# rasd3/TODA

Hardware: NVIDIA B200
Metric: frames/s voxelize+VoxelResBackBone8x fwd+bwd (higher is better)
Workload: dtype bf16

## Files before the change

include/toda_b200.h:

```cpp
#ifndef TODA_B200_H
#define TODA_B200_H

#include <stddef.h>
#include <stdint.h>

#ifdef __cplusplus
extern "C" {
#endif

#define TODA_OK 0
#define TODA_ERR_INVALID (-1)
#define TODA_ERR_CUDA (-2)
#define TODA_ERR_WORKSPACE (-3)
#define TODA_ERR_UNSUPPORTED (-4)

#define TODA_ORDER_FIRST_APPEARANCE 0
#define TODA_ORDER_CANONICAL 1

const char *toda_last_error(void);
int toda_version(void);
long long toda_launch_count(void);
int toda_device_info(int *sm_count_host, int *cc_major_host, int *cc_minor_host);

size_t toda_index_bytes(int batch, int D, int H, int W);
int toda_index_insert(void *index, int batch, int D, int H, int W, const int32_t *coords, int n, void *stream);
int toda_index_insert_strided(void *index_out, int batch, int oD, int oH, int oW, const int32_t *in_coords, int n_in,
                              const int *ksize_host, const int *stride_host, const int *pad_host, void *stream);
int toda_index_build(void *index, int batch, int D, int H, int W, int32_t *out_coords, int cap, int32_t *n_out,
                     void *stream);
int toda_index_rows(const void *index, int batch, int D, int H, int W, const int32_t *coords, int n, int32_t *rows,
                    void *stream);
int toda_index_release(void *index, int batch, int D, int H, int W, const int32_t *coords, int n, void *stream);

#define TODA_SELECT_RANGE_XY 0
#define TODA_SELECT_RECT_XY 1
#define TODA_SELECT_SECTOR 2
#define TODA_SELECT_BOXES 3
size_t toda_points_select_workspace_bytes(int n);
int toda_points_select(const float *points, int n, int stride, int x_col, const int32_t *frame_offsets, int batch, int mode,
                       const double *params_host, int invert, int add_batch_col, float *out, int32_t *out_offsets,
                       void *workspace, size_t workspace_bytes, void *stream);

#define TODA_WORLD_FLIP_X 0
#define TODA_WORLD_FLIP_Y 1
#define TODA_WORLD_ROTATE 2
#define TODA_WORLD_SCALE 3
int toda_points_world_transform(const float *points, int n, int stride, int x_col, const int32_t *frame_offsets, int batch,
                                int n_steps, const int *kinds_host, const float *params_host, float *out, void *stream);

size_t toda_voxelize_workspace_bytes(int64_t n_points, int batch, const int *grid_host, int max_points,
                                     int max_voxels);
int toda_voxelize_hard(const float *points, int64_t n_points, int point_stride, int xyz_col, int feat_col,
                       int num_features, const int32_t *frame_offsets, int batch, const float *range_host,
                       const float *vsize_host, const int *grid_host, int max_points, int max_voxels, int order,
                       float *voxels, int32_t *coords, int32_t *num_points, int32_t *voxel_counts, void *workspace,
                       size_t workspace_bytes, void *stream);

int toda_mean_vfe_fwd(const float *voxels, const void *num_points, int num_is_float, int n_voxels, int max_points,
                      int num_features, float *voxel_features, void *stream);
int toda_mean_vfe_bwd(const float *d_voxel_features, const void *num_points, int num_is_float, int n_voxels,
                      int max_points, int num_features, float *d_voxels, void *stream);

int toda_rulebook_subm(const void *index, int batch, int D, int H, int W, const int32_t *coords, int n,
                       const int *ksize_host, int32_t *nbr, void *stream);
int toda_rulebook_sparse(const void *index_in, int iD, int iH, int iW, const void *index_out, int oD, int oH, int oW,
                         int batch, const int32_t *in_coords, int n_in, const int32_t *out_coords, int n_out,
                         const int *ksize_host, const int *stride_host, const int *pad_host, int32_t *nbr_fwd,
                         int32_t *nbr_bwd, void *stream);

size_t toda_parity_order_workspace_bytes(int n);
int toda_parity_order(const int32_t *coords, int n, const int *stride_host, const int *pad_host, int32_t *order,
                      int32_t *pos_of_row, void *workspace, size_t workspace_bytes, void *stream);

#define TODA_CONV_FP32 0
#define TODA_CONV_BF16 1
#define TODA_CONV_BF16X3 2
int toda_weight_repack(const float *w_param, int kvol, int cin, int cout, int transpose, int mirror_k, float *w_out,
                       void *stream);
size_t toda_spconv_fwd_workspace_bytes(int n_in, int cin, int cout, int kvol, int precision);
int toda_table_tile_masks(const int32_t *nbr, int n_out, int kvol, uint32_t *masks, void *stream);
int toda_spconv_uses_tensor_cores(int cin, int cout, int kvol, int precision);
int toda_spconv_wgrad_uses_tensor_cores(int cin, int cout, int kvol, int precision);
int toda_spconv_fwd(const float *x, const void *x_bf16, int n_in, int cin, const int32_t *nbr, int n_out, int kvol,
                    const float *w, int cout, const float *bias, float *y, const int32_t *out_rows,
                    const uint32_t *tile_masks, double *bn_sums, int precision, void *workspace, size_t workspace_bytes,
                    void *stream);
int toda_tile_plan_capacity(int channels);
int toda_table_tile_plan(const int32_t *nbr, int n_out, int kvol, int ngroups, int cap, uint16_t *lidx, int32_t *rows,
                         int32_t *cnt, void *stream);
int toda_spconv_fwd_plan(const float *x, const void *x_bf16, int n_in, int cin, const int32_t *nbr, int n_out, int kvol,
                         const float *w, int cout, const float *bias, const float *addend, float *y,
                         const int32_t *out_rows, const uint32_t *tile_masks, const uint16_t *plan_lidx,
                         const int32_t *plan_rows, const int32_t *plan_cnt, int plan_groups, int plan_cap, double *bn_sums,
                         const void *w_bf16, int precision, void *workspace, size_t workspace_bytes, void *stream);
int toda_weight_kmajor_bf16(const float *w, int kvol, int cin, int cout, void *w_bf16, void *stream);
size_t toda_spconv_wgrad_workspace_bytes(int n_in, int n_out, int kvol, int cin, int cout, int precision);
int toda_spconv_wgrad(const float *x, const void *x_bf16, int n_in, int cin, const int32_t *nbr, int n_out, int kvol,
                      const float *dy, const void *dy_bf16, int cout, float *dw_param, void *workspace,
                      size_t workspace_bytes, int precision, void *stream);

size_t toda_bn_workspace_bytes(int channels);
int toda_bn_local_sums(const float *y, const double *epilogue_sums, int n, int channels, double *sums, double *count,
                       void *workspace, size_t workspace_bytes, void *stream);
int toda_bn_eval_coeffs(const float *gamma, const float *beta, const float *running_mean, const float *running_var,
                        float eps, int channels, float *scale, float *shift, void *stream);
int toda_bn_apply(const float *y, int n, int channels, const float *scale, const float *shift, const float *residual,
                  int relu, float *a, void *a_bf16, void *stream);
int toda_bn_apply_sums(const float *y, int n, int channels, const double *sums, const double *count, const float *gamma,
                       const float *beta, float eps, float momentum, float *running_mean, float *running_var, float *scale,
                       float *shift, float *save_mean, float *save_rstd, const float *residual, int relu, float *a,
                       void *a_bf16, void *stream);
int toda_bn_bwd_reduce(const float *da, const float *a, const float *y, int n, int channels, const float *save_mean,
                       const float *save_rstd, int relu, double *red, float *dgamma, float *dbeta, void *workspace,
                       size_t workspace_bytes, void *stream);
int toda_bn_bwd_finish(const float *da, const float *a, const float *y, int n, int channels, const float *gamma,
                       const float *save_mean, const float *save_rstd, int relu, int training, const double *red,
                       const double *count, float *dy, void *dy_bf16, float *dresidual, void *stream);
int toda_bn_bwd(const float *da, const float *a, const float *y, int n, int channels, const float *gamma,
                const float *save_mean, const float *save_rstd, int relu, int training, float *dy, void *dy_bf16,
                float *dresidual, float *dgamma, float *dbeta, void *workspace, size_t workspace_bytes, void *stream);
int toda_col_sum(const float *dy, int n, int channels, float *out, void *workspace, size_t workspace_bytes,
                 void *stream);

typedef struct {
    const float *x; const void *x_bf16; int n_in, cin; const int32_t *nbr; int n_out, kvol;
    const float *w; const void *w_bf16 ; int cout; const float *bias ;
    const uint32_t *tile_masks ;
    const uint16_t *plan_lidx ; const int32_t *plan_rows; const int32_t *plan_cnt; int plan_groups, plan_cap;
    int precision; void *conv_ws; size_t conv_ws_bytes;
    const float *gamma; const float *beta; float eps, momentum; float *running_mean; float *running_var; int training;
    const float *residual ; int relu;
    float *y; double *sums; float *stats; float *a; void *a_bf16 ;
    void *bn_ws; size_t bn_ws_bytes;
} toda_layer_fwd_args;
typedef struct {
    const float *da; const float *a_mask; const float *y; int n_out, cout; const float *gamma; const float *mean; const float *rstd;
    int relu, training; float *dy; void *dy_bf16 ; float *dres ; float *dgamma; float *dbeta;
    void *bn_ws; size_t bn_ws_bytes;
    const float *x; const void *x_bf16 ; int n_in, cin, kvol;
    int need_dx; const int32_t *dgrad_nbr; const float *wt; const void *wt_bf16 ;
    const int32_t *dgrad_out_rows ; const uint32_t *dgrad_masks ;
    const uint16_t *dplan_lidx ; const int32_t *dplan_rows; const int32_t *dplan_cnt; int dplan_groups, dplan_cap;
    const float *addend ; float *dx;
    int need_dw; const int32_t *nbr_fwd; float *dw; void *wgrad_ws; size_t wgrad_ws_bytes;
    int need_db; float *db;
    int precision; void *conv_ws; size_t conv_ws_bytes;
} toda_layer_bwd_args;
int toda_layer_fwd(const toda_layer_fwd_args *args, void *stream);
int toda_layer_bwd(const toda_layer_bwd_args *args, void *stream);
int toda_layer_fwd_stats(const toda_layer_fwd_args *args, double *local_sums, void *stream);
int toda_layer_fwd_apply(const toda_layer_fwd_args *args, const double *global_sums, void *stream);
int toda_layer_bwd_reduce(const toda_layer_bwd_args *args, double *local_red, void *stream);
int toda_layer_bwd_finish(const toda_layer_bwd_args *args, const double *global_red, const double *global_count, void *stream);

int toda_bev_scatter_fwd(const float *features, const int32_t *coords, int n, int channels, int batch, int D, int H,
                         int W, float *out, void *stream);
int toda_bev_scatter_bwd(const float *d_out, const int32_t *coords, int n, int channels, int batch, int D, int H,
                         int W, float *d_features, void *stream);

int toda_gather_rows(const float *in, const int32_t *rows, int n, int channels, float *out, void *stream);

#ifdef __cplusplus
}
#endif
#endif
```

toda_b200/_C.py:

```python
import ctypes
import os

_HERE = os.path.dirname(os.path.abspath(__file__))
LIB_PATH = os.path.join(_HERE, "lib", "libtoda_b200.so")

c_int, c_i64, c_f32, c_vp, c_sz = ctypes.c_int, ctypes.c_int64, ctypes.c_float, ctypes.c_void_p, ctypes.c_size_t
_IP = ctypes.POINTER(ctypes.c_int)
_FP = ctypes.POINTER(ctypes.c_float)

SIGNATURES = {
    "toda_last_error": (ctypes.c_char_p, []),
    "toda_version": (c_int, []),
    "toda_launch_count": (ctypes.c_longlong, []),
    "toda_device_info": (c_int, [_IP, _IP, _IP]),
    "toda_index_bytes": (c_sz, [c_int] * 4),
    "toda_index_insert": (c_int, [c_vp, c_int, c_int, c_int, c_int, c_vp, c_int, c_vp]),
    "toda_index_insert_strided": (c_int, [c_vp, c_int, c_int, c_int, c_int, c_vp, c_int, _IP, _IP, _IP, c_vp]),
    "toda_index_build": (c_int, [c_vp, c_int, c_int, c_int, c_int, c_vp, c_int, c_vp, c_vp]),
    "toda_index_rows": (c_int, [c_vp, c_int, c_int, c_int, c_int, c_vp, c_int, c_vp, c_vp]),
    "toda_index_release": (c_int, [c_vp, c_int, c_int, c_int, c_int, c_vp, c_int, c_vp]),
    "toda_points_select_workspace_bytes": (c_sz, [c_int]),
    "toda_points_select": (c_int, [c_vp, c_int, c_int, c_int, c_vp, c_int, c_int, ctypes.POINTER(ctypes.c_double), c_int, c_int,
                                   c_vp, c_vp, c_vp, c_sz, c_vp]),
    "toda_points_world_transform": (c_int, [c_vp, c_int, c_int, c_int, c_vp, c_int, c_int, _IP, _FP, c_vp, c_vp]),
    "toda_voxelize_workspace_bytes": (c_sz, [c_i64, c_int, _IP, c_int, c_int]),
    "toda_voxelize_hard": (c_int, [c_vp, c_i64, c_int, c_int, c_int, c_int, c_vp, c_int, _FP, _FP, _IP, c_int, c_int,
                                   c_int, c_vp, c_vp, c_vp, c_vp, c_vp, c_sz, c_vp]),
    "toda_mean_vfe_fwd": (c_int, [c_vp, c_vp, c_int, c_int, c_int, c_int, c_vp, c_vp]),
    "toda_mean_vfe_bwd": (c_int, [c_vp, c_vp, c_int, c_int, c_int, c_int, c_vp, c_vp]),
    "toda_rulebook_subm": (c_int, [c_vp, c_int, c_int, c_int, c_int, c_vp, c_int, _IP, c_vp, c_vp]),
    "toda_rulebook_sparse": (c_int, [c_vp, c_int, c_int, c_int, c_vp, c_int, c_int, c_int, c_int, c_vp, c_int, c_vp,
                                     c_int, _IP, _IP, _IP, c_vp, c_vp, c_vp]),
    "toda_weight_repack": (c_int, [c_vp, c_int, c_int, c_int, c_int, c_int, c_vp, c_vp]),
    "toda_spconv_fwd_workspace_bytes": (c_sz, [c_int] * 5),
    "toda_spconv_uses_tensor_cores": (c_int, [c_int] * 4),
    "toda_spconv_wgrad_uses_tensor_cores": (c_int, [c_int] * 4),
    "toda_parity_order_workspace_bytes": (c_sz, [c_int]),
    "toda_parity_order": (c_int, [c_vp, c_int, _IP, _IP, c_vp, c_vp, c_vp, c_sz, c_vp]),
    "toda_table_tile_masks": (c_int, [c_vp, c_int, c_int, c_vp, c_vp]),
    "toda_spconv_fwd": (c_int, [c_vp, c_vp, c_int, c_int, c_vp, c_int, c_int, c_vp, c_int, c_vp, c_vp, c_vp, c_vp, c_vp, c_int, c_vp,
                                c_sz, c_vp]),
    "toda_tile_plan_capacity": (c_int, [c_int]),
    "toda_table_tile_plan": (c_int, [c_vp, c_int, c_int, c_int, c_int, c_vp, c_vp, c_vp, c_vp]),
    "toda_spconv_fwd_plan": (c_int, [c_vp, c_vp, c_int, c_int, c_vp, c_int, c_int, c_vp, c_int, c_vp, c_vp, c_vp, c_vp, c_vp, c_vp,
                                     c_vp, c_vp, c_int, c_int, c_vp, c_vp, c_int, c_vp, c_sz, c_vp]),
    "toda_weight_kmajor_bf16": (c_int, [c_vp, c_int, c_int, c_int, c_vp, c_vp]),
    "toda_layer_fwd": (c_int, [c_vp, c_vp]),
    "toda_layer_bwd": (c_int, [c_vp, c_vp]),
    "toda_layer_fwd_stats": (c_int, [c_vp, c_vp, c_vp]),
    "toda_layer_fwd_apply": (c_int, [c_vp, c_vp, c_vp]),
    "toda_layer_bwd_reduce": (c_int, [c_vp, c_vp, c_vp]),
    "toda_layer_bwd_finish": (c_int, [c_vp, c_vp, c_vp, c_vp]),
    "toda_spconv_wgrad_workspace_bytes": (c_sz, [c_int] * 6),
    "toda_spconv_wgrad": (c_int, [c_vp, c_vp, c_int, c_int, c_vp, c_int, c_int, c_vp, c_vp, c_int, c_vp, c_vp, c_sz, c_int, c_vp]),
    "toda_bn_workspace_bytes": (c_sz, [c_int]),
    "toda_bn_local_sums": (c_int, [c_vp, c_vp, c_int, c_int, c_vp, c_vp, c_vp, c_sz, c_vp]),
    "toda_bn_eval_coeffs": (c_int, [c_vp, c_vp, c_vp, c_vp, c_f32, c_int, c_vp, c_vp, c_vp]),
    "toda_bn_apply": (c_int, [c_vp, c_int, c_int, c_vp, c_vp, c_vp, c_int, c_vp, c_vp, c_vp]),
    "toda_bn_apply_sums": (c_int, [c_vp, c_int, c_int, c_vp, c_vp, c_vp, c_vp, c_f32, c_f32, c_vp, c_vp, c_vp, c_vp, c_vp, c_vp,
                                   c_vp, c_int, c_vp, c_vp, c_vp]),
    "toda_bn_bwd": (c_int, [c_vp, c_vp, c_vp, c_int, c_int, c_vp, c_vp, c_vp, c_int, c_int, c_vp, c_vp, c_vp, c_vp, c_vp,
                            c_vp, c_sz, c_vp]),
    "toda_bn_bwd_reduce": (c_int, [c_vp, c_vp, c_vp, c_int, c_int, c_vp, c_vp, c_int, c_vp, c_vp, c_vp, c_vp, c_sz, c_vp]),
    "toda_bn_bwd_finish": (c_int, [c_vp, c_vp, c_vp, c_int, c_int, c_vp, c_vp, c_vp, c_int, c_int, c_vp, c_vp, c_vp, c_vp, c_vp,
                                   c_vp]),
    "toda_col_sum": (c_int, [c_vp, c_int, c_int, c_vp, c_vp, c_sz, c_vp]),
    "toda_bev_scatter_fwd": (c_int, [c_vp, c_vp, c_int, c_int, c_int, c_int, c_int, c_int, c_vp, c_vp]),
    "toda_bev_scatter_bwd": (c_int, [c_vp, c_vp, c_int, c_int, c_int, c_int, c_int, c_int, c_vp, c_vp]),
    "toda_gather_rows": (c_int, [c_vp, c_vp, c_int, c_int, c_vp, c_vp]),
}



class LayerFwdArgs(ctypes.Structure):
    _fields_ = [("x", c_vp), ("x_bf16", c_vp), ("n_in", c_int), ("cin", c_int), ("nbr", c_vp), ("n_out", c_int), ("kvol", c_int),
                ("w", c_vp), ("w_bf16", c_vp), ("cout", c_int), ("bias", c_vp), ("tile_masks", c_vp),
                ("plan_lidx", c_vp), ("plan_rows", c_vp), ("plan_cnt", c_vp), ("plan_groups", c_int), ("plan_cap", c_int),
                ("precision", c_int), ("conv_ws", c_vp), ("conv_ws_bytes", c_sz),
                ("gamma", c_vp), ("beta", c_vp), ("eps", c_f32), ("momentum", c_f32), ("running_mean", c_vp), ("running_var", c_vp),
                ("training", c_int), ("residual", c_vp), ("relu", c_int),
                ("y", c_vp), ("sums", c_vp), ("stats", c_vp), ("a", c_vp), ("a_bf16", c_vp), ("bn_ws", c_vp), ("bn_ws_bytes", c_sz)]


class LayerBwdArgs(ctypes.Structure):
    _fields_ = [("da", c_vp), ("a_mask", c_vp), ("y", c_vp), ("n_out", c_int), ("cout", c_int), ("gamma", c_vp), ("mean", c_vp),
                ("rstd", c_vp), ("relu", c_int), ("training", c_int), ("dy", c_vp), ("dy_bf16", c_vp), ("dres", c_vp), ("dgamma", c_vp),
                ("dbeta", c_vp), ("bn_ws", c_vp), ("bn_ws_bytes", c_sz),
                ("x", c_vp), ("x_bf16", c_vp), ("n_in", c_int), ("cin", c_int), ("kvol", c_int),
                ("need_dx", c_int), ("dgrad_nbr", c_vp), ("wt", c_vp), ("wt_bf16", c_vp), ("dgrad_out_rows", c_vp), ("dgrad_masks", c_vp),
                ("dplan_lidx", c_vp), ("dplan_rows", c_vp), ("dplan_cnt", c_vp), ("dplan_groups", c_int), ("dplan_cap", c_int),
                ("addend", c_vp), ("dx", c_vp),
                ("need_dw", c_int), ("nbr_fwd", c_vp), ("dw", c_vp), ("wgrad_ws", c_vp), ("wgrad_ws_bytes", c_sz),
                ("need_db", c_int), ("db", c_vp),
                ("precision", c_int), ("conv_ws", c_vp), ("conv_ws_bytes", c_sz)]


_lib = None


def lib():
    global _lib
    if _lib is None:
        if not os.path.exists(LIB_PATH):
            raise RuntimeError(
                f"{LIB_PATH} is missing: build it with `python -c 'import __graft_entry__ as g; g.build()'` "
                "(nvcc, sm_100a).  toda_b200 has no CPU fallback.")
        L = ctypes.CDLL(LIB_PATH)
        for name, (res, args) in SIGNATURES.items():
            fn = getattr(L, name)
            fn.restype = res
            fn.argtypes = args
        _lib = L
    return _lib


def check(rc, what=""):
    if rc != 0:
        msg = lib().toda_last_error().decode("utf-8", "replace")
        raise RuntimeError(f"libtoda_b200 {what} failed (code {rc}): {msg}")


def ints(vals):
    return (ctypes.c_int * len(vals))(*[int(v) for v in vals])


def doubles(vals):
    return (ctypes.c_double * len(vals))(*[float(v) for v in vals])


def floats(vals):
    return (ctypes.c_float * len(vals))(*[float(v) for v in vals])
```

toda_b200/csrc/bn.cu:

```cuda
#include <cuda_bf16.h>

#include "common.cuh"

namespace {

constexpr int kThreads = 256;
constexpr int kPartials = 2 * kNumSMs;

template <int MODE>
__global__ void __launch_bounds__(kThreads) col_reduce_vec_kernel(const float *__restrict__ p0, const float *__restrict__ p1,
                                                                  const float *__restrict__ p2, int n, int c,
                                                                  const float *__restrict__ mean, const float *__restrict__ rstd,
                                                                  int relu, double *__restrict__ partial) {
    __shared__ double s0[kThreads * 4], s1[kThreads * 4];
    const int tpr = c >> 2;
    const int rpi = kThreads / tpr;
    const int tx = threadIdx.x % tpr, ty = threadIdx.x / tpr;
    double a0[4] = {0, 0, 0, 0}, a1[4] = {0, 0, 0, 0};
    float4 m4 = make_float4(0, 0, 0, 0), r4 = make_float4(0, 0, 0, 0);
    if (MODE == 1) { m4 = __ldg((const float4 *)mean + tx); r4 = __ldg((const float4 *)rstd + tx); }
    const long long stride = (long long)gridDim.x * rpi;
    const bool active = ty < rpi;
    constexpr int U = 4;
    for (long long r = (long long)blockIdx.x * rpi + ty; active && r < n; r += U * stride) {
        float4 v0[U], v1[U], v2[U];
        bool ok[U];
#pragma unroll
        for (int u = 0; u < U; ++u) {
            long long rr = r + u * stride;
            ok[u] = rr < n;
            size_t e = ok[u] ? (size_t)rr * tpr + tx : 0;
            v0[u] = __ldg((const float4 *)p0 + e);
            if (MODE == 1) { v1[u] = __ldg((const float4 *)p1 + e); v2[u] = __ldg((const float4 *)p2 + e); }
        }
#pragma unroll
        for (int u = 0; u < U; ++u) {
            if (!ok[u]) continue;
            float x[4] = {v0[u].x, v0[u].y, v0[u].z, v0[u].w};
            if (MODE == 0) {
#pragma unroll
                for (int q = 0; q < 4; ++q) { a0[q] += x[q]; a1[q] += (double)x[q] * x[q]; }
            } else if (MODE == 1) {
                float av[4] = {v1[u].x, v1[u].y, v1[u].z, v1[u].w}, yv[4] = {v2[u].x, v2[u].y, v2[u].z, v2[u].w};
                float mm[4] = {m4.x, m4.y, m4.z, m4.w}, rs[4] = {r4.x, r4.y, r4.z, r4.w};
#pragma unroll
                for (int q = 0; q < 4; ++q) {
                    float g = (relu && !(av[q] > 0.f)) ? 0.f : x[q];
                    float xh = (yv[q] - mm[q]) * rs[q];
                    a0[q] += g; a1[q] += (double)g * xh;
                }
            } else {
#pragma unroll
                for (int q = 0; q < 4; ++q) a0[q] += x[q];
            }
        }
    }
#pragma unroll
    for (int q = 0; q < 4; ++q) { s0[threadIdx.x * 4 + q] = a0[q]; s1[threadIdx.x * 4 + q] = a1[q]; }
    __syncthreads();
    if ((int)threadIdx.x < c) {
        int ch = threadIdx.x, txx = ch >> 2, q = ch & 3;
        double t0 = 0.0, t1 = 0.0;
        for (int j = 0; j < rpi; ++j) { t0 += s0[(j * tpr + txx) * 4 + q]; t1 += s1[(j * tpr + txx) * 4 + q]; }
        partial[((size_t)blockIdx.x * 2 + 0) * c + ch] = t0;
        partial[((size_t)blockIdx.x * 2 + 1) * c + ch] = t1;
    }
}

template <int MODE>
__global__ void __launch_bounds__(kThreads) col_reduce_kernel(const float *__restrict__ p0, const float *__restrict__ p1,
                                                              const float *__restrict__ p2, int n, int c,
                                                              const float *__restrict__ mean, const float *__restrict__ rstd,
                                                              int relu, double *__restrict__ partial) {
    __shared__ double s0[kThreads], s1[kThreads];
    const int cpad = c <= 16 ? 16 : (c <= 32 ? 32 : (c <= 64 ? 64 : (c <= 128 ? 128 : 256)));
    const int rows_per_iter = kThreads / cpad;
    const int tx = threadIdx.x % cpad, ty = threadIdx.x / cpad;
    double a0 = 0.0, a1 = 0.0;
    float m = 0.f, rs = 0.f;
    if (MODE == 1 && tx < c) { m = mean[tx]; rs = rstd[tx]; }
    for (long long r = (long long)blockIdx.x * rows_per_iter + ty; r < n; r += (long long)gridDim.x * rows_per_iter) {
        if (tx < c) {
            size_t e = (size_t)r * c + tx;
            if (MODE == 0) {
                float v = __ldg(p0 + e);
                a0 += v; a1 += (double)v * v;
            } else if (MODE == 1) {
                float g = __ldg(p0 + e);
                if (relu && !(__ldg(p1 + e) > 0.f)) g = 0.f;
                float xh = (__ldg(p2 + e) - m) * rs;
                a0 += g; a1 += (double)g * xh;
            } else {
                a0 += __ldg(p0 + e);
            }
        }
    }
    s0[threadIdx.x] = a0; s1[threadIdx.x] = a1;
    __syncthreads();
    if (threadIdx.x < cpad && threadIdx.x < c) {
        double t0 = 0.0, t1 = 0.0;
        for (int j = 0; j < rows_per_iter; ++j) { t0 += s0[j * cpad + threadIdx.x]; t1 += s1[j * cpad + threadIdx.x]; }
        partial[((size_t)blockIdx.x * 2 + 0) * c + threadIdx.x] = t0;
        partial[((size_t)blockIdx.x * 2 + 1) * c + threadIdx.x] = t1;
    }
}

static bool vec_channels(int c) { return c % 4 == 0 && kThreads % (c / 4) == 0; }

template <int MODE>
static void launch_col_reduce(const float *p0, const float *p1, const float *p2, int n, int c, const float *mean,
                              const float *rstd, int relu, double *partial, cudaStream_t st) {
    if (vec_channels(c))
        col_reduce_vec_kernel<MODE><<<kPartials, kThreads, 0, st>>>(p0, p1, p2, n, c, mean, rstd, relu, partial);
    else
        col_reduce_kernel<MODE><<<kPartials, kThreads, 0, st>>>(p0, p1, p2, n, c, mean, rstd, relu, partial);
}

__device__ __forceinline__ void warp_sum_partials(const double *__restrict__ partial, int nblocks, int c, int ch, double &s,
                                                  double &ss) {
    const int lane = threadIdx.x & 31;
    constexpr int kPerLane = (kPartials + 31) / 32;
    double va[kPerLane], vb[kPerLane];
#pragma unroll
    for (int i = 0; i < kPerLane; ++i) {
        const int j = lane + 32 * i;
        const bool ok = j < nblocks;
        va[i] = ok ? partial[((size_t)j * 2) * c + ch] : 0.0;
        vb[i] = ok ? partial[((size_t)j * 2 + 1) * c + ch] : 0.0;
    }
    double a = 0.0, b = 0.0;
#pragma unroll
    for (int i = 0; i < kPerLane; ++i) { a += va[i]; b += vb[i]; }
#pragma unroll
    for (int o = 16; o > 0; o >>= 1) { a += __shfl_xor_sync(0xffffffffu, a, o); b += __shfl_xor_sync(0xffffffffu, b, o); }
    s = a; ss = b;
}

__device__ __forceinline__ void bn_coeffs(double s, double ss, int n, float g, float bt, float eps, float &scale, float &shift,
                                          float &meanf, float &rstd, double &var) {
    const double mean = n > 0 ? s / n : 0.0;
    var = n > 0 ? ss / n - mean * mean : 0.0;
    if (var < 0.0) var = 0.0;
    rstd = (float)(1.0 / sqrt(var + (double)eps));
    meanf = (float)mean;
    scale = __fmul_rn(g, rstd);
    shift = __fsub_rn(bt, __fmul_rn(__fmul_rn(meanf, g), rstd));
}

__device__ __forceinline__ void bn_update_running(float *running_mean, float *running_var, int ch, float momentum, float meanf,
                                                  double var, int n) {
    if (running_mean) running_mean[ch] = __fadd_rn(__fmul_rn(1.f - momentum, running_mean[ch]), __fmul_rn(momentum, meanf));
    if (running_var) {
        const double unbiased = n > 1 ? var * n / (n - 1) : var;
        running_var[ch] = __fadd_rn(__fmul_rn(1.f - momentum, running_var[ch]), __fmul_rn(momentum, (float)unbiased));
    }
}

__global__ void bn_local_sums_kernel(const double *partial, int nblocks, const double *src, int n, int c, double *out,
                                     double *count) {
    if (count && blockIdx.x == 0 && threadIdx.x == 0) *count = (double)n;
    int ch = (blockIdx.x * blockDim.x + threadIdx.x) >> 5;
    if (ch >= c) return;
    double s = 0.0, ss = 0.0;
    if (partial) warp_sum_partials(partial, nblocks, c, ch, s, ss);
    else if (src) { s = src[ch]; ss = src[c + ch]; }
    if ((threadIdx.x & 31) != 0) return;
    out[ch] = s;
    out[c + ch] = ss;
}

__global__ void bn_eval_coeffs_kernel(const float *gamma, const float *beta, const float *rm, const float *rv, float eps,
                                      int c, float *scale, float *shift) {
    int ch = blockIdx.x * blockDim.x + threadIdx.x;
    if (ch >= c) return;
    float rstd = 1.0f / sqrtf(rv[ch] + eps);
    float g = gamma ? gamma[ch] : 1.f, bt = beta ? beta[ch] : 0.f;
    scale[ch] = g * rstd;
    shift[ch] = bt - rm[ch] * g * rstd;
}

__device__ __forceinline__ void store_bf16x4(__nv_bfloat16 *__restrict__ dst, long long e, float4 o) {
    __nv_bfloat162 lo = __floats2bfloat162_rn(o.x, o.y), hi = __floats2bfloat162_rn(o.z, o.w);
    uint2 pk;
    pk.x = *(uint32_t *)&lo;
    pk.y = *(uint32_t *)&hi;
    ((uint2 *)dst)[e] = pk;
}

struct BnCoeffs {
    const double *sums; const double *count; int n;
    const float *gamma, *beta; float eps, momentum;
    float *running_mean, *running_var, *scale, *shift, *save_mean, *save_rstd;
};

template <bool VEC>
__global__ void __launch_bounds__(kThreads) bn_apply_kernel(const float *__restrict__ y, long long total, int c, BnCoeffs k,
                                                            const float *__restrict__ residual, int relu, float *__restrict__ a,
                                                            __nv_bfloat16 *__restrict__ a_bf16) {
    extern __shared__ __align__(16) float s_coef[];
    float *s_sc = s_coef, *s_sh = s_coef + c;
    const int n = k.count ? (int)*k.count : k.n;
    for (int ch = threadIdx.x; ch < c; ch += blockDim.x) {
        if (!k.sums) {
            s_sc[ch] = k.scale[ch];
            s_sh[ch] = k.shift[ch];
            continue;
        }
        float meanf, rstd;
        double var;
        bn_coeffs(k.sums[ch], k.sums[c + ch], n, k.gamma ? k.gamma[ch] : 1.f, k.beta ? k.beta[ch] : 0.f, k.eps, s_sc[ch], s_sh[ch],
                  meanf, rstd, var);
        if (blockIdx.x == 0) {
            k.scale[ch] = s_sc[ch];
            k.shift[ch] = s_sh[ch];
            if (k.save_mean) k.save_mean[ch] = meanf;
            if (k.save_rstd) k.save_rstd[ch] = rstd;
            if (n > 0) bn_update_running(k.running_mean, k.running_var, ch, k.momentum, meanf, var, n);
        }
    }
    __syncthreads();
    const long long stride = (long long)gridDim.x * blockDim.x;
    long long e = blockIdx.x * (long long)blockDim.x + threadIdx.x;
    if (VEC) {
        const long long tv = total >> 2;
        const int ch = (int)((e << 2) % c);
        const float4 sc = *(const float4 *)(s_sc + ch), sh = *(const float4 *)(s_sh + ch);
        for (; e < tv; e += stride) {
            const float4 v = __ldg((const float4 *)y + e);
            float4 o = make_float4(fmaf(v.x, sc.x, sh.x), fmaf(v.y, sc.y, sh.y), fmaf(v.z, sc.z, sh.z), fmaf(v.w, sc.w, sh.w));
            if (residual) {
                const float4 r = __ldg((const float4 *)residual + e);
                o.x += r.x; o.y += r.y; o.z += r.z; o.w += r.w;
            }
            if (relu) { o.x = fmaxf(o.x, 0.f); o.y = fmaxf(o.y, 0.f); o.z = fmaxf(o.z, 0.f); o.w = fmaxf(o.w, 0.f); }
            ((float4 *)a)[e] = o;
            if (a_bf16) store_bf16x4(a_bf16, e, o);
        }
    } else {
        for (; e < total; e += stride) {
            const int ch = (int)(e % c);
            float o = fmaf(__ldg(y + e), s_sc[ch], s_sh[ch]);
            if (residual) o += __ldg(residual + e);
            if (relu) o = fmaxf(o, 0.f);
            a[e] = o;
            if (a_bf16) a_bf16[e] = __float2bfloat16_rn(o);
        }
    }
}

__global__ void bn_bwd_finalize_kernel(const double *__restrict__ partial, int nblocks, int c, float *dgamma, float *dbeta,
                                       double *sums) {
    int ch = (blockIdx.x * blockDim.x + threadIdx.x) >> 5;
    if (ch >= c) return;
    double s, sx;
    warp_sum_partials(partial, nblocks, c, ch, s, sx);
    if ((threadIdx.x & 31) != 0) return;
    if (dbeta) dbeta[ch] = (float)s;
    if (dgamma) dgamma[ch] = (float)sx;
    sums[ch] = s;
    sums[c + ch] = sx;
}

template <bool VEC>
__global__ void __launch_bounds__(kThreads) bn_bwd_apply_kernel(const float *__restrict__ da, const float *__restrict__ a,
                                                                const float *__restrict__ y, long long total, int c, int n,
                                                                const double *__restrict__ count, const float *__restrict__ gamma,
                                                                const float *__restrict__ mean, const float *__restrict__ rstd,
                                                                const double *__restrict__ sums, int relu, int training,
                                                                float *__restrict__ dy, float *__restrict__ dres,
                                                                __nv_bfloat16 *__restrict__ dy_bf16) {
    if (count) n = (int)*count;
    auto sum = [&](int i) -> float { return (float)sums[i]; };
    const float inv_n = n > 0 ? 1.0f / (float)n : 0.f;
    const long long stride = (long long)gridDim.x * blockDim.x;
    long long e = blockIdx.x * (long long)blockDim.x + threadIdx.x;
    if (VEC) {
        const long long tv = total >> 2;
        const int ch = (int)((e << 2) % c);
        float A[4], B[4], C[4];
#pragma unroll
        for (int q = 0; q < 4; ++q) {
            float gm = gamma ? gamma[ch + q] : 1.f, rs = rstd[ch + q];
            A[q] = gm * rs;
            B[q] = training ? -gm * rs * rs * sum(c + ch + q) * inv_n : 0.f;
            C[q] = training ? -A[q] * sum(ch + q) * inv_n - B[q] * mean[ch + q] : 0.f;
        }
        for (; e < tv; e += stride) {
            float4 g4 = __ldg((const float4 *)da + e);
            float4 y4 = training ? __ldg((const float4 *)y + e) : make_float4(0.f, 0.f, 0.f, 0.f);
            if (relu) {
                float4 a4 = __ldg((const float4 *)a + e);
                g4.x = a4.x > 0.f ? g4.x : 0.f; g4.y = a4.y > 0.f ? g4.y : 0.f;
                g4.z = a4.z > 0.f ? g4.z : 0.f; g4.w = a4.w > 0.f ? g4.w : 0.f;
            }
            if (dres) ((float4 *)dres)[e] = g4;
            float4 o;
            o.x = fmaf(A[0], g4.x, fmaf(B[0], y4.x, C[0]));
            o.y = fmaf(A[1], g4.y, fmaf(B[1], y4.y, C[1]));
            o.z = fmaf(A[2], g4.z, fmaf(B[2], y4.z, C[2]));
            o.w = fmaf(A[3], g4.w, fmaf(B[3], y4.w, C[3]));
            if (dy) ((float4 *)dy)[e] = o;
            if (dy_bf16) store_bf16x4(dy_bf16, e, o);
        }
    } else {
        for (; e < total; e += stride) {
            int ch = (int)(e % c);
            float g = __ldg(da + e);
            if (relu && !(__ldg(a + e) > 0.f)) g = 0.f;
            if (dres) dres[e] = g;
            float gm = gamma ? gamma[ch] : 1.f;
            float rs = rstd[ch];
            float o;
            if (training) {
                float xh = (__ldg(y + e) - mean[ch]) * rs;
                o = gm * rs * (g - sum(ch) * inv_n - xh * sum(c + ch) * inv_n);
            } else {
                o = gm * rs * g;
            }
            if (dy) dy[e] = o;
            if (dy_bf16) dy_bf16[e] = __float2bfloat16_rn(o);
        }
    }
}

__global__ void col_sum_finalize_kernel(const double *__restrict__ partial, int nblocks, int c, float *out) {
    int ch = (blockIdx.x * blockDim.x + threadIdx.x) >> 5;
    if (ch >= c) return;
    double s, unused;
    warp_sum_partials(partial, nblocks, c, ch, s, unused);
    if ((threadIdx.x & 31) == 0) out[ch] = (float)s;
}

size_t partials_bytes(int c) { return (size_t)kPartials * 2 * c * sizeof(double); }
size_t bn_ws_bytes(int c) { return align_up(partials_bytes(c) + 2 * c * sizeof(double), 256); }

template <auto Kernel> int resident_grid(int64_t items) {
    static const int64_t cap = [] {
        int per_sm = 0;
        if (cudaOccupancyMaxActiveBlocksPerMultiprocessor(&per_sm, Kernel, kThreads, 0) != cudaSuccess || per_sm < 1) per_sm = 4;
        return (int64_t)per_sm * kNumSMs;
    }();
    const int64_t need = (items + kThreads - 1) / kThreads;
    return (int)(need < 1 ? 1 : (need < cap ? need : cap));
}

int launch_bn_apply(const float *y, int n, int c, const BnCoeffs &k, const float *residual, int relu, float *a, void *a_bf16,
                    cudaStream_t st) {
    const long long total = (long long)n * c;
    const size_t smem = 2 * (size_t)c * sizeof(float);
    if (vec_channels(c))
        bn_apply_kernel<true><<<resident_grid<bn_apply_kernel<true>>(total / 4), kThreads, smem, st>>>(
            y, total, c, k, residual, relu, a, (__nv_bfloat16 *)a_bf16);
    else
        bn_apply_kernel<false><<<resident_grid<bn_apply_kernel<false>>(total), kThreads, smem, st>>>(
            y, total, c, k, residual, relu, a, (__nv_bfloat16 *)a_bf16);
    TODA_LAUNCH_OK();
    return TODA_OK;
}

}

extern "C" size_t toda_bn_workspace_bytes(int channels) { return channels > 0 ? bn_ws_bytes(channels) : 0; }

double *bn_workspace_red(void *workspace, int c) { return (double *)((char *)workspace + partials_bytes(c)); }

extern "C" int toda_bn_local_sums(const float *y, const double *epilogue_sums, int n, int c, double *sums, double *count,
                                  void *workspace, size_t workspace_bytes, void *stream) {
    TODA_CHECK_ARG(n >= 0 && c > 0 && c <= 256 && sums, "bn_local_sums: bad args n=%d c=%d", n, c);
    if (n > 0 && epilogue_sums == sums && !count) return TODA_OK;
    cudaStream_t st = (cudaStream_t)stream;
    const double *partial = nullptr;
    if (n > 0 && !epilogue_sums) {
        TODA_CHECK_ARG(y && workspace, "bn_local_sums: null pointer");
        if (workspace_bytes < bn_ws_bytes(c)) { toda_set_error("bn_local_sums: workspace too small"); return TODA_ERR_WORKSPACE; }
        launch_col_reduce<0>(y, nullptr, nullptr, n, c, nullptr, nullptr, 0, (double *)workspace, st);
        TODA_LAUNCH_OK();
        partial = (const double *)workspace;
    }
    bn_local_sums_kernel<<<ceil_div(c * 32, 128), 128, 0, st>>>(partial, kPartials, n > 0 ? epilogue_sums : nullptr, n, c, sums,
                                                              count);
    TODA_LAUNCH_OK();
    return TODA_OK;
}

extern "C" int toda_bn_eval_coeffs(const float *gamma, const float *beta, const float *running_mean, const float *running_var,
                                   float eps, int c, float *scale, float *shift, void *stream) {
    TODA_CHECK_ARG(c > 0 && running_mean && running_var && scale && shift, "bn_eval_coeffs: bad args");
    bn_eval_coeffs_kernel<<<ceil_div(c, 128), 128, 0, (cudaStream_t)stream>>>(gamma, beta, running_mean, running_var, eps, c,
                                                                             scale, shift);
    TODA_LAUNCH_OK();
    return TODA_OK;
}

extern "C" int toda_bn_apply(const float *y, int n, int c, const float *scale, const float *shift, const float *residual,
                             int relu, float *a, void *a_bf16, void *stream) {
    TODA_CHECK_ARG(n >= 0 && c > 0, "bn_apply: bad sizes");
    if (n == 0) return TODA_OK;
    TODA_CHECK_ARG(y && scale && shift && a, "bn_apply: null pointer");
    BnCoeffs k{};
    k.scale = (float *)scale;
    k.shift = (float *)shift;
    return launch_bn_apply(y, n, c, k, residual, relu, a, a_bf16, (cudaStream_t)stream);
}

extern "C" int toda_bn_apply_sums(const float *y, int n, int c, const double *sums, const double *count, const float *gamma,
                                  const float *beta, float eps, float momentum, float *running_mean, float *running_var,
                                  float *scale, float *shift, float *save_mean, float *save_rstd, const float *residual, int relu,
                                  float *a, void *a_bf16, void *stream) {
    TODA_CHECK_ARG(n >= 0 && c > 0 && sums && scale && shift, "bn_apply_sums: bad args");
    TODA_CHECK_ARG(n == 0 || (y && a), "bn_apply_sums: null pointer");
    const BnCoeffs k{sums, count, n, gamma, beta, eps, momentum, running_mean, running_var, scale, shift, save_mean, save_rstd};
    return launch_bn_apply(y, n, c, k, residual, relu, a, a_bf16, (cudaStream_t)stream);
}

extern "C" int toda_bn_bwd_reduce(const float *da, const float *a, const float *y, int n, int c, const float *save_mean,
                                  const float *save_rstd, int relu, double *local_red, float *dgamma, float *dbeta, void *workspace,
                                  size_t workspace_bytes, void *stream) {
    TODA_CHECK_ARG(n >= 0 && c > 0 && c <= 256, "bn_bwd_reduce: unsupported sizes n=%d c=%d", n, c);
    TODA_CHECK_ARG(save_mean && save_rstd && workspace && local_red && (n == 0 || (da && y)) && (!relu || a || n == 0),
                   "bn_bwd_reduce: null pointer");
    if (workspace_bytes < bn_ws_bytes(c)) { toda_set_error("bn_bwd_reduce: workspace too small"); return TODA_ERR_WORKSPACE; }
    cudaStream_t st = (cudaStream_t)stream;
    double *partial = (double *)workspace;
    launch_col_reduce<1>(da, a, y, n, c, save_mean, save_rstd, relu, partial, st);
    TODA_LAUNCH_OK();
    bn_bwd_finalize_kernel<<<ceil_div(c * 32, 128), 128, 0, st>>>(partial, kPartials, c, dgamma, dbeta, local_red);
    TODA_LAUNCH_OK();
    return TODA_OK;
}

extern "C" int toda_bn_bwd_finish(const float *da, const float *a, const float *y, int n, int c, const float *gamma,
                                  const float *save_mean, const float *save_rstd, int relu, int training, const double *red,
                                  const double *count, float *dy, void *dy_bf16, float *dresidual, void *stream) {
    TODA_CHECK_ARG(n >= 0 && c > 0 && c <= 256, "bn_bwd_finish: unsupported sizes n=%d c=%d", n, c);
    TODA_CHECK_ARG(save_mean && save_rstd && (red || !training) && (n == 0 || (da && y && (dy || dy_bf16))) &&
                   (!relu || a || n == 0), "bn_bwd_finish: null pointer");
    if (n == 0) return TODA_OK;
    const long long total = (long long)n * c;
    cudaStream_t st = (cudaStream_t)stream;
    if (vec_channels(c))
        bn_bwd_apply_kernel<true><<<resident_grid<bn_bwd_apply_kernel<true>>(total / 4), kThreads, 0, st>>>(
            da, a, y, total, c, n, count, gamma, save_mean, save_rstd, red, relu, training, dy, dresidual, (__nv_bfloat16 *)dy_bf16);
    else
        bn_bwd_apply_kernel<false><<<resident_grid<bn_bwd_apply_kernel<false>>(total), kThreads, 0, st>>>(
            da, a, y, total, c, n, count, gamma, save_mean, save_rstd, red, relu, training, dy, dresidual, (__nv_bfloat16 *)dy_bf16);
    TODA_LAUNCH_OK();
    return TODA_OK;
}

extern "C" int toda_bn_bwd(const float *da, const float *a, const float *y, int n, int c, const float *gamma,
                           const float *save_mean, const float *save_rstd, int relu, int training, float *dy, void *dy_bf16,
                           float *dresidual, float *dgamma, float *dbeta, void *workspace, size_t workspace_bytes, void *stream) {
    TODA_CHECK_ARG(workspace, "bn_bwd: null workspace");
    double *red = bn_workspace_red(workspace, c);
    int rc = toda_bn_bwd_reduce(da, a, y, n, c, save_mean, save_rstd, relu, red, dgamma, dbeta, workspace, workspace_bytes, stream);
    if (rc) return rc;
    return toda_bn_bwd_finish(da, a, y, n, c, gamma, save_mean, save_rstd, relu, training, red, nullptr, dy, dy_bf16, dresidual,
                              stream);
}

extern "C" int toda_col_sum(const float *dy, int n, int c, float *out, void *workspace, size_t workspace_bytes, void *stream) {
    TODA_CHECK_ARG(n >= 0 && c > 0 && c <= 256 && out && workspace, "col_sum: bad args");
    if (workspace_bytes < bn_ws_bytes(c)) { toda_set_error("col_sum: workspace too small"); return TODA_ERR_WORKSPACE; }
    cudaStream_t st = (cudaStream_t)stream;
    double *partial = (double *)workspace;
    launch_col_reduce<2>(dy, nullptr, nullptr, n, c, nullptr, nullptr, 0, partial, st);
    TODA_LAUNCH_OK();
    col_sum_finalize_kernel<<<ceil_div(c * 32, 128), 128, 0, st>>>(partial, kPartials, c, out);
    TODA_LAUNCH_OK();
    return TODA_OK;
}
```

toda_b200/csrc/conv_simt.cu:

```cuda
#include "common.cuh"
#include "conv_ts.cuh"

int conv_tc_fwd(const float *x, const void *x_bf16, int n_in, int cin, const int32_t *nbr, int n_out, int kvol, const float *w,
                int cout, const float *bias, float *y, const int32_t *out_rows, const uint32_t *tile_masks, double *bn_sums,
                void *workspace, size_t workspace_bytes,
                cudaStream_t st, const TilePlan *plan, const float *addend, const void *w_bf16);
size_t conv_tc_fwd_workspace_bytes(int n_in, int cin, int cout, int kvol);
int conv_tc_wgrad(const float *x, const void *x_bf16, int n_in, int cin, const int32_t *nbr, int n_out, int kvol,
                  const float *dy, const void *dy_bf16, int cout, float *dw_param, void *workspace, size_t workspace_bytes,
                  cudaStream_t st);
bool conv_tc_supported(int cin, int cout, int kvol);
size_t conv_x3_fwd_workspace_bytes(int n_in, int cin, int cout, int kvol);
int conv_x3_fwd(const float *x, int n_in, int cin, const int32_t *nbr, int n_out, int kvol, const float *w, int cout, const float *bias,
                float *y, const int32_t *out_rows, const uint32_t *tile_masks, double *bn_sums, void *workspace, size_t workspace_bytes,
                cudaStream_t st, const TilePlan *plan, const float *addend);
size_t conv_x3_wgrad_workspace_bytes(int n_in, int n_out, int kvol, int cin, int cout);
int conv_x3_wgrad(const float *x, int n_in, int cin, const int32_t *nbr, int n_out, int kvol, const float *dy, int cout, float *dw_param,
                  void *workspace, size_t workspace_bytes, cudaStream_t st);
bool conv_tc_wgrad_supported(int cin, int cout, int kvol);
size_t conv_tc_wgrad_workspace_bytes(int n_in, int n_out, int kvol, int cin, int cout);

namespace {

constexpr int kThreads = 256;
constexpr int BK = 16;

template <int BM, int BN>
__global__ void __launch_bounds__(kThreads) conv_fwd_f32_kernel(const float *__restrict__ x, int cin,
                                                                const int *__restrict__ nbr, int n_out, int kvol,
                                                                const float *__restrict__ w, int cout,
                                                                const float *__restrict__ bias, float *__restrict__ y,
                                                                const int *__restrict__ out_rows ,
                                                                const float *__restrict__ addend ) {
    static_assert((BM / 4) * (BN / 4) == kThreads, "4x4 micro-tiles must cover the CTA tile");
    __shared__ __align__(16) float As[BK][BM + 4];
    __shared__ __align__(16) float Bs[BK][BN + 4];
    __shared__ int rows[BM];
    const int tid = threadIdx.x;
    const int tx = tid % (BN / 4), ty = tid / (BN / 4);
    const int row0 = blockIdx.x * BM, col0 = blockIdx.y * BN;
    const bool vec = (cin % 4) == 0;
    float acc[4][4];
#pragma unroll
    for (int i = 0; i < 4; ++i)
#pragma unroll
        for (int j = 0; j < 4; ++j) acc[i][j] = 0.f;

    for (int k = 0; k < kvol; ++k) {
        int any = 0;
        for (int m = tid; m < BM; m += kThreads) {
            int r = row0 + m;
            int src = (r < n_out) ? __ldg(nbr + (size_t)k * n_out + r) : -1;
            rows[m] = src;
            any |= (src >= 0);
        }
        any = __syncthreads_or(any);
        if (!any) continue;
        for (int c0 = 0; c0 < cin; c0 += BK) {
            if (vec) {
                for (int e = tid; e < BM * (BK / 4); e += kThreads) {
                    int m = e / (BK / 4), q = e % (BK / 4);
                    int src = rows[m];
                    float4 v = make_float4(0.f, 0.f, 0.f, 0.f);
                    if (src >= 0 && c0 + q * 4 < cin) v = __ldg((const float4 *)(x + (size_t)src * cin + c0 + q * 4));
                    As[q * 4 + 0][m] = v.x; As[q * 4 + 1][m] = v.y; As[q * 4 + 2][m] = v.z; As[q * 4 + 3][m] = v.w;
                }
            } else {
                for (int e = tid; e < BM * BK; e += kThreads) {
                    int m = e / BK, kk = e % BK;
                    int src = rows[m];
                    As[kk][m] = (src >= 0 && c0 + kk < cin) ? __ldg(x + (size_t)src * cin + c0 + kk) : 0.f;
                }
            }
            for (int e = tid; e < BK * BN; e += kThreads) {
                int kk = e / BN, nn = e % BN;
                Bs[kk][nn] = (c0 + kk < cin && col0 + nn < cout) ? __ldg(w + ((size_t)k * cin + c0 + kk) * cout + col0 + nn) : 0.f;
            }
            __syncthreads();
#pragma unroll
            for (int kk = 0; kk < BK; ++kk) {
                float4 a = *(const float4 *)&As[kk][ty * 4];
                float4 b = *(const float4 *)&Bs[kk][tx * 4];
                float av[4] = {a.x, a.y, a.z, a.w}, bv[4] = {b.x, b.y, b.z, b.w};
#pragma unroll
                for (int i = 0; i < 4; ++i)
#pragma unroll
                    for (int j = 0; j < 4; ++j) acc[i][j] = fmaf(av[i], bv[j], acc[i][j]);
            }
            __syncthreads();
        }
    }
#pragma unroll
    for (int i = 0; i < 4; ++i) {
        int r = row0 + ty * 4 + i;
        if (r >= n_out) continue;
        const int orow = out_rows ? __ldg(out_rows + r) : r;
#pragma unroll
        for (int j = 0; j < 4; ++j) {
            int c = col0 + tx * 4 + j;
            if (c < cout) y[(size_t)orow * cout + c] = acc[i][j] + (bias ? __ldg(bias + c) : 0.f) + (addend ? __ldg(addend + (size_t)orow * cout + c) : 0.f);
        }
    }
}

constexpr int WT = 64;
__global__ void __launch_bounds__(kThreads) conv_wgrad_f32_kernel(const float *__restrict__ x, int cin,
                                                                  const int *__restrict__ nbr, int n_out, int kvol,
                                                                  const float *__restrict__ dy, int cout, int rows_per_split,
                                                                  float *__restrict__ partial) {
    __shared__ __align__(16) float As[BK][WT + 4];
    __shared__ __align__(16) float Bs[BK][WT + 4];
    __shared__ int pin[kThreads], pout[kThreads];
    __shared__ int warp_cnt[kThreads / 32];
    const int tid = threadIdx.x, lane = tid & 31, warp = tid >> 5;
    const int tx = tid % (WT / 4), ty = tid / (WT / 4);
    const int ci_tiles = (cin + WT - 1) / WT, co_tiles = (cout + WT - 1) / WT;
    int bx = blockIdx.x;
    const int co_t = bx % co_tiles; bx /= co_tiles;
    const int ci_t = bx % ci_tiles; bx /= ci_tiles;
    const int k = bx;
    const int split = blockIdx.y;
    const int ci0 = ci_t * WT, co0 = co_t * WT;
    const int r_begin = split * rows_per_split;
    const int r_end = min(n_out, r_begin + rows_per_split);
    float acc[4][4];
#pragma unroll
    for (int i = 0; i < 4; ++i)
#pragma unroll
        for (int j = 0; j < 4; ++j) acc[i][j] = 0.f;

    for (int r0 = r_begin; r0 < r_end; r0 += kThreads) {
        int r = r0 + tid;
        int src = (r < r_end) ? __ldg(nbr + (size_t)k * n_out + r) : -1;
        unsigned bal = __ballot_sync(0xffffffffu, src >= 0);
        if (lane == 0) warp_cnt[warp] = __popc(bal);
        __syncthreads();
        int woff = 0, total = 0;
#pragma unroll
        for (int wi = 0; wi < kThreads / 32; ++wi) {
            int c = warp_cnt[wi];
            if (wi < warp) woff += c;
            total += c;
        }
        if (src >= 0) {
            int pos = woff + __popc(bal & ((1u << lane) - 1u));
            pin[pos] = src;
            pout[pos] = r;
        }
        __syncthreads();
        for (int g0 = 0; g0 < total; g0 += BK) {
            for (int e = tid; e < BK * WT; e += kThreads) {
                int kk = e / WT, c = e % WT;
                bool ok = g0 + kk < total;
                As[kk][c] = (ok && ci0 + c < cin) ? __ldg(x + (size_t)pin[ok ? g0 + kk : 0] * cin + ci0 + c) : 0.f;
                Bs[kk][c] = (ok && co0 + c < cout) ? __ldg(dy + (size_t)pout[ok ? g0 + kk : 0] * cout + co0 + c) : 0.f;
            }
            __syncthreads();
#pragma unroll
            for (int kk = 0; kk < BK; ++kk) {
                float4 a = *(const float4 *)&As[kk][ty * 4];
                float4 b = *(const float4 *)&Bs[kk][tx * 4];
                float av[4] = {a.x, a.y, a.z, a.w}, bv[4] = {b.x, b.y, b.z, b.w};
#pragma unroll
                for (int i = 0; i < 4; ++i)
#pragma unroll
                    for (int j = 0; j < 4; ++j) acc[i][j] = fmaf(av[i], bv[j], acc[i][j]);
            }
            __syncthreads();
        }
    }
    float *dst = partial + ((size_t)split * kvol + k) * cin * cout;
#pragma unroll
    for (int i = 0; i < 4; ++i) {
        int ci = ci0 + ty * 4 + i;
        if (ci >= cin) continue;
#pragma unroll
        for (int j = 0; j < 4; ++j) {
            int co = co0 + tx * 4 + j;
            if (co < cout) dst[(size_t)ci * cout + co] = acc[i][j];
        }
    }
}

__global__ void wgrad_reduce_kernel(const float *__restrict__ partial, int splits, int kvol, int cin, int cout,
                                    float *__restrict__ dw_param) {
    size_t per = (size_t)kvol * cin * cout;
    const int sub = threadIdx.x & 7;
    for (size_t e = (blockIdx.x * (size_t)blockDim.x + threadIdx.x) >> 3; e < ((per + 31) & ~(size_t)31);
         e += ((size_t)gridDim.x * blockDim.x) >> 3) {
        float s = 0.f;
        if (e < per) {
            int ci = (int)(e % cin);
            size_t t = e / cin;
            int k = (int)(t % kvol);
            int co = (int)(t / kvol);
            size_t src = ((size_t)k * cin + ci) * cout + co;
            for (int sp = sub; sp < splits; sp += 8) s += partial[sp * per + src];
        }
        s += __shfl_xor_sync(0xffffffffu, s, 1);
        s += __shfl_xor_sync(0xffffffffu, s, 2);
        s += __shfl_xor_sync(0xffffffffu, s, 4);
        if (e < per && sub == 0) dw_param[e] = s;
    }
}

__global__ void weight_repack_kernel(const float *__restrict__ w_param, int kvol, int cin, int cout, int transpose,
                                     int mirror, float *__restrict__ w_out) {
    size_t per = (size_t)kvol * cin * cout;
    for (size_t e = blockIdx.x * (size_t)blockDim.x + threadIdx.x; e < per; e += (size_t)gridDim.x * blockDim.x) {
        int inner = (int)(e % (transpose ? cin : cout));
        size_t t = e / (transpose ? cin : cout);
        int mid = (int)(t % (transpose ? cout : cin));
        int k = (int)(t / (transpose ? cout : cin));
        int ci = transpose ? inner : mid, co = transpose ? mid : inner;
        int ks = mirror ? kvol - 1 - k : k;
        w_out[e] = __ldg(w_param + ((size_t)co * kvol + ks) * cin + ci);
    }
}

__global__ void gather_rows_kernel(const float *__restrict__ in, const int *__restrict__ rows, long long total, int c,
                                   float *__restrict__ out) {
    for (long long e = blockIdx.x * (long long)blockDim.x + threadIdx.x; e < total; e += (long long)gridDim.x * blockDim.x) {
        long long i = e / c;
        int r = __ldg(rows + i);
        out[e] = r >= 0 ? __ldg(in + (long long)r * c + (e - i * c)) : 0.f;
    }
}

int wgrad_splits(int n_out, int kvol, int cin, int cout) {
    int tiles = kvol * ((cin + WT - 1) / WT) * ((cout + WT - 1) / WT);
    int want = (4 * kNumSMs + tiles - 1) / tiles;
    int max_by_rows = (n_out + 4 * kThreads - 1) / (4 * kThreads);
    int s = want < max_by_rows ? want : max_by_rows;
    return s < 1 ? 1 : s;
}

}

extern "C" int toda_weight_repack(const float *w_param, int kvol, int cin, int cout, int transpose, int mirror_k,
                                  float *w_out, void *stream) {
    TODA_CHECK_ARG(w_param && w_out && kvol > 0 && cin > 0 && cout > 0, "weight_repack: bad args");
    size_t per = (size_t)kvol * cin * cout;
    weight_repack_kernel<<<wave_grid(per, 256), 256, 0, (cudaStream_t)stream>>>(w_param, kvol, cin, cout, transpose,
                                                                              mirror_k, w_out);
    TODA_LAUNCH_OK();
    return TODA_OK;
}

extern "C" int toda_spconv_uses_tensor_cores(int cin, int cout, int kvol, int precision) {
    return (precision == TODA_CONV_BF16 || precision == TODA_CONV_BF16X3) && conv_tc_supported(cin, cout, kvol) ? 1 : 0;
}

extern "C" int toda_spconv_wgrad_uses_tensor_cores(int cin, int cout, int kvol, int precision) {
    return (precision == TODA_CONV_BF16 || precision == TODA_CONV_BF16X3) && conv_tc_wgrad_supported(cin, cout, kvol) ? 1 : 0;
}

extern "C" size_t toda_spconv_fwd_workspace_bytes(int n_in, int cin, int cout, int kvol, int precision) {
    if (precision == TODA_CONV_BF16 && n_in >= 0 && cin > 0 && cout > 0 && kvol > 0 && conv_tc_supported(cin, cout, kvol))
        return conv_tc_fwd_workspace_bytes(n_in, cin, cout, kvol);
    if (precision == TODA_CONV_BF16X3 && n_in >= 0 && cin > 0 && cout > 0 && kvol > 0 && conv_tc_supported(cin, cout, kvol))
        return conv_x3_fwd_workspace_bytes(n_in, cin, cout, kvol);
    return 0;
}

static int spconv_fwd_impl(const float *x, const void *x_bf16, int n_in, int cin, const int32_t *nbr, int n_out, int kvol,
                           const float *w, int cout, const float *bias, float *y, const int32_t *out_rows,
                           const uint32_t *tile_masks, double *bn_sums, int precision, void *workspace, size_t workspace_bytes,
                           void *stream, const TilePlan *plan, const float *addend, const void *w_bf16);

extern "C" int toda_spconv_fwd(const float *x, const void *x_bf16, int n_in, int cin, const int32_t *nbr, int n_out, int kvol,
                               const float *w, int cout, const float *bias, float *y, const int32_t *out_rows,
                               const uint32_t *tile_masks, double *bn_sums, int precision,
                               void *workspace, size_t workspace_bytes, void *stream) {
    return spconv_fwd_impl(x, x_bf16, n_in, cin, nbr, n_out, kvol, w, cout, bias, y, out_rows, tile_masks, bn_sums, precision, workspace,
                           workspace_bytes, stream, nullptr, nullptr, nullptr);
}

extern "C" int toda_spconv_fwd_plan(const float *x, const void *x_bf16, int n_in, int cin, const int32_t *nbr, int n_out, int kvol,
                                    const float *w, int cout, const float *bias, const float *addend, float *y,
                                    const int32_t *out_rows, const uint32_t *tile_masks, const uint16_t *plan_lidx,
                                    const int32_t *plan_rows, const int32_t *plan_cnt, int plan_groups, int plan_cap, double *bn_sums,
                                    const void *w_bf16, int precision, void *workspace, size_t workspace_bytes, void *stream) {
    TilePlan plan{plan_lidx, plan_rows, plan_cnt, plan_groups, plan_cap};
    return spconv_fwd_impl(x, x_bf16, n_in, cin, nbr, n_out, kvol, w, cout, bias, y, out_rows, tile_masks, bn_sums, precision, workspace,
                           workspace_bytes, stream, plan_lidx ? &plan : nullptr, addend, w_bf16);
}

static int spconv_fwd_impl(const float *x, const void *x_bf16, int n_in, int cin, const int32_t *nbr, int n_out, int kvol,
                           const float *w, int cout, const float *bias, float *y, const int32_t *out_rows,
                           const uint32_t *tile_masks, double *bn_sums, int precision, void *workspace, size_t workspace_bytes,
                           void *stream, const TilePlan *plan, const float *addend, const void *w_bf16) {
    TODA_CHECK_ARG(n_in >= 0 && n_out >= 0 && cin > 0 && cout > 0 && kvol > 0, "spconv_fwd: bad sizes");
    if (n_out == 0) return TODA_OK;
    TODA_CHECK_ARG(x && nbr && w && y, "spconv_fwd: null pointer");
    cudaStream_t st = (cudaStream_t)stream;
    TODA_CHECK_ARG(precision == TODA_CONV_FP32 || precision == TODA_CONV_BF16 || precision == TODA_CONV_BF16X3,
                   "spconv_fwd: unknown precision %d", precision);
    if (precision == TODA_CONV_BF16X3 && conv_tc_supported(cin, cout, kvol))
        return conv_x3_fwd(x, n_in, cin, nbr, n_out, kvol, w, cout, bias, y, out_rows, tile_masks, bn_sums, workspace, workspace_bytes, st,
                           plan, addend);
    if (precision == TODA_CONV_BF16 && conv_tc_supported(cin, cout, kvol))
        return conv_tc_fwd(x, x_bf16, n_in, cin, nbr, n_out, kvol, w, cout, bias, y, out_rows, tile_masks, bn_sums, workspace,
                           workspace_bytes, st, plan, addend, w_bf16);
    TODA_CHECK_ARG(!bn_sums, "spconv_fwd: fused BatchNorm statistics need the tensor-core kernel for this shape");
    if (cout <= 16) {
        dim3 grid(ceil_div(n_out, 256), ceil_div(cout, 16));
        conv_fwd_f32_kernel<256, 16><<<grid, kThreads, 0, st>>>(x, cin, nbr, n_out, kvol, w, cout, bias, y, out_rows, addend);
    } else if (cout <= 32) {
        dim3 grid(ceil_div(n_out, 128), ceil_div(cout, 32));
        conv_fwd_f32_kernel<128, 32><<<grid, kThreads, 0, st>>>(x, cin, nbr, n_out, kvol, w, cout, bias, y, out_rows, addend);
    } else {
        dim3 grid(ceil_div(n_out, 64), ceil_div(cout, 64));
        conv_fwd_f32_kernel<64, 64><<<grid, kThreads, 0, st>>>(x, cin, nbr, n_out, kvol, w, cout, bias, y, out_rows, addend);
    }
    TODA_LAUNCH_OK();
    return TODA_OK;
}

extern "C" size_t toda_spconv_wgrad_workspace_bytes(int n_in, int n_out, int kvol, int cin, int cout, int precision) {
    if (n_in < 0 || n_out < 0 || kvol <= 0 || cin <= 0 || cout <= 0) return 0;
    if (precision == TODA_CONV_BF16 && conv_tc_wgrad_supported(cin, cout, kvol))
        return conv_tc_wgrad_workspace_bytes(n_in, n_out, kvol, cin, cout);
    if (precision == TODA_CONV_BF16X3 && conv_tc_wgrad_supported(cin, cout, kvol))
        return conv_x3_wgrad_workspace_bytes(n_in, n_out, kvol, cin, cout);
    int splits = wgrad_splits(n_out, kvol, cin, cout);
    return align_up((size_t)splits * kvol * cin * cout * sizeof(float), 256);
}

extern "C" int toda_spconv_wgrad(const float *x, const void *x_bf16, int n_in, int cin, const int32_t *nbr, int n_out,
                                 int kvol, const float *dy, const void *dy_bf16, int cout, float *dw_param, void *workspace,
                                 size_t workspace_bytes, int precision, void *stream) {
    TODA_CHECK_ARG(n_in >= 0 && n_out >= 0 && cin > 0 && cout > 0 && kvol > 0, "spconv_wgrad: bad sizes");
    TODA_CHECK_ARG(dw_param, "spconv_wgrad: null dw");
    cudaStream_t st = (cudaStream_t)stream;
    if (n_out == 0) {
        TODA_CUDA_OK(cudaMemsetAsync(dw_param, 0, (size_t)kvol * cin * cout * sizeof(float), st));
        return TODA_OK;
    }
    TODA_CHECK_ARG(x && nbr && dy && workspace, "spconv_wgrad: null pointer");
    TODA_CHECK_ARG(precision == TODA_CONV_FP32 || precision == TODA_CONV_BF16 || precision == TODA_CONV_BF16X3,
                   "spconv_wgrad: unknown precision %d", precision);
    if (precision == TODA_CONV_BF16X3 && conv_tc_wgrad_supported(cin, cout, kvol))
        return conv_x3_wgrad(x, n_in, cin, nbr, n_out, kvol, dy, cout, dw_param, workspace, workspace_bytes, st);
    if (precision == TODA_CONV_BF16 && conv_tc_wgrad_supported(cin, cout, kvol))
        return conv_tc_wgrad(x, x_bf16, n_in, cin, nbr, n_out, kvol, dy, dy_bf16, cout, dw_param, workspace, workspace_bytes, st);
    int splits = wgrad_splits(n_out, kvol, cin, cout);
    size_t need = (size_t)splits * kvol * cin * cout * sizeof(float);
    if (workspace_bytes < need) {
        toda_set_error("spconv_wgrad: workspace %zu < required %zu bytes", workspace_bytes, need);
        return TODA_ERR_WORKSPACE;
    }
    int rows_per_split = ceil_div(n_out, splits);
    rows_per_split = ceil_div(rows_per_split, kThreads) * kThreads;
    int tiles = kvol * ((cin + WT - 1) / WT) * ((cout + WT - 1) / WT);
    dim3 grid(tiles, splits);
    conv_wgrad_f32_kernel<<<grid, kThreads, 0, st>>>(x, cin, nbr, n_out, kvol, dy, cout, rows_per_split, (float *)workspace);
    TODA_LAUNCH_OK();
    size_t per = (size_t)kvol * cin * cout;
    wgrad_reduce_kernel<<<wave_grid(per * 8, 256), 256, 0, st>>>((const float *)workspace, splits, kvol, cin, cout, dw_param);
    TODA_LAUNCH_OK();
    return TODA_OK;
}

extern "C" int toda_gather_rows(const float *in, const int32_t *rows, int n, int channels, float *out, void *stream) {
    TODA_CHECK_ARG(n >= 0 && channels > 0, "gather_rows: bad sizes");
    if (n == 0) return TODA_OK;
    TODA_CHECK_ARG(in && rows && out, "gather_rows: null pointer");
    long long total = (long long)n * channels;
    gather_rows_kernel<<<wave_grid(total, 256), 256, 0, (cudaStream_t)stream>>>(in, rows, total, channels, out);
    TODA_LAUNCH_OK();
    return TODA_OK;
}
```

toda_b200/csrc/conv_tc.cu:

```cuda
#include <cuda.h>
#include <cuda_bf16.h>
#include <stdlib.h>

#include "common.cuh"
#include "conv_ts.cuh"
#include "epilogue.cuh"
#include "table_slice.cuh"

namespace {

constexpr int kTileM = 128;
constexpr int kChunkK = 64;
constexpr int kStages = 3;
constexpr int kProducers = 128;
constexpr int kThreadsTC = kProducers + 32;
constexpr int kABytes = kTileM * kChunkK * 2;
constexpr int kBBytesMax = 128 * kChunkK * 2;
constexpr int kStageBytes = kABytes + kBBytesMax;
constexpr int kMaxKvol = 27;
constexpr int kIdxBytes = kMaxKvol * kTileM * 4;

__device__ __forceinline__ uint32_t smem_u32(const void *p) { return (uint32_t)__cvta_generic_to_shared(p); }

__device__ __forceinline__ void mbar_init(uint32_t bar, uint32_t count) {
// ... 245 lines not shown
                const uint32_t d_tmem = tmem_base + ab * COUT;
                uint32_t accumulate = 0;
                for (unsigned long long cm = chunk_mask_of(t); cm; cm &= cm - 1, ++g) {
                    const int c = __ffsll((long long)cm) - 1;
                    const int s = g % S, use = g / S;
                    if (dbg && blockIdx.x == 0 && lane == 0 && g < 256) dbg[4 * 256 + g] = clock64();
                    if (!ready) mbar_wait(full_bar + 8 * s, use & 1);
                    if (dbg && blockIdx.x == 0 && lane == 0 && g < 256) dbg[5 * 256 + g] = clock64();
                    const int sn = (g + 1) % S, usen = (g + 1) / S;
                    ready = mbar_test(full_bar + 8 * sn, usen & 1);
                    asm volatile("tcgen05.fence::after_thread_sync;" ::: "memory");
                    const uint32_t a_tile = base + s * C::kStage, b_tile = a_tile + C::kATile;
                    const int ksteps = min(kChunkElems, ktot - c * kChunkElems) / 16;
                    if (elect_one()) {
                        const uint64_t ad0 = make_desc_k_sw128(a_tile), bd0 = make_desc_k_sw128(b_tile);
                        umma_bf16(d_tmem, ad0, bd0, idesc, accumulate);
                        for (int j = 1; j < ksteps; ++j) {
                            const uint32_t blk = j >> 2, st = j & 3;
                            umma_bf16(d_tmem, ad0 + blk * (C::kABlock >> 4) + 2 * st, bd0 + blk * (C::kBBlock >> 4) + 2 * st, idesc, 1u);
                        }
                        umma_commit(empty_bar + 8 * s);
                    }
                    accumulate = 1u;
                    __syncwarp();
                    if (dbg && blockIdx.x == 0 && lane == 0 && g < 256) dbg[6 * 256 + g] = clock64();
                }
                if (elect_one()) umma_commit(acc_full + 8 * ab);
                __syncwarp();
            }
        }
    } else if (warp < 13) {
        const int q = warp & 3;
        float acc_s[COUT / 16], acc_q[COUT / 16];
#pragma unroll
        for (int i = 0; i < COUT / 16; ++i) acc_s[i] = acc_q[i] = 0.f;
        int it = 0;
        for (int t = blockIdx.x; t < num_tiles; t += gridDim.x, ++it) {
            const int ab = it & 1;
            mbar_wait(acc_full + 8 * ab, (it >> 1) & 1);
            asm volatile("tcgen05.fence::after_thread_sync;" ::: "memory");
            const int row = t * kTileM + q * 32 + lane;
            const int orow = (out_rows && row < n_out) ? __ldg(out_rows + row) : row;
            const uint32_t taddr = tmem_base + ((uint32_t)(q * 32) << 16) + ab * COUT;
#pragma unroll
            for (int n0 = 0; n0 < COUT; n0 += 16) {
                uint32_t v[16];
                asm volatile(
                    "tcgen05.ld.sync.aligned.32x32b.x16.b32 {%0,%1,%2,%3,%4,%5,%6,%7,%8,%9,%10,%11,%12,%13,%14,%15}, [%16];"
                    : "=r"(v[0]), "=r"(v[1]), "=r"(v[2]), "=r"(v[3]), "=r"(v[4]), "=r"(v[5]), "=r"(v[6]), "=r"(v[7]), "=r"(v[8]),
                      "=r"(v[9]), "=r"(v[10]), "=r"(v[11]), "=r"(v[12]), "=r"(v[13]), "=r"(v[14]), "=r"(v[15])
                    : "r"(taddr + n0));
                asm volatile("tcgen05.wait::ld.sync.aligned;" ::: "memory");
                float o[16];
#pragma unroll
                for (int j = 0; j < 16; ++j) o[j] = __uint_as_float(v[j]) + (bias ? __ldg(bias + n0 + j) : 0.f);
                if (row < n_out) {
                    if (addend) {
                        const float4 *ad = (const float4 *)(addend + (size_t)orow * COUT + n0);
#pragma unroll
                        for (int qq = 0; qq < 4; ++qq) {
                            const float4 a4 = __ldg(ad + qq);
                            o[4 * qq] += a4.x; o[4 * qq + 1] += a4.y; o[4 * qq + 2] += a4.z; o[4 * qq + 3] += a4.w;
                        }
                    }
                    float4 *dst = (float4 *)(y + (size_t)orow * COUT + n0);
#pragma unroll
                    for (int qq = 0; qq < 4; ++qq) dst[qq] = make_float4(o[4 * qq], o[4 * qq + 1], o[4 * qq + 2], o[4 * qq + 3]);
                }
                if (bn_sums) {
                    float sq[16];
#pragma unroll
                    for (int j = 0; j < 16; ++j) {
                        o[j] = row < n_out ? o[j] : 0.f;
                        sq[j] = o[j] * o[j];
                    }
                    acc_s[n0 / 16] += warp_colsum16(o, lane);
                    acc_q[n0 / 16] += warp_colsum16(sq, lane);
                }
            }
            asm volatile("tcgen05.fence::before_thread_sync;" ::: "memory");
            mbar_arrive(acc_empty + 8 * ab);
            if (dbg && blockIdx.x == 0 && q == 1 && lane == 0 && it < 256) dbg[2 * 256 + it] = clock64();
        }
        if (bn_sums && !(lane & 1)) {
            const int col = (lane >> 1) & 15;
#pragma unroll
            for (int i = 0; i < COUT / 16; ++i) {
                atomicAdd(bn_sums + i * 16 + col, (double)acc_s[i]);
                atomicAdd(bn_sums + COUT + i * 16 + col, (double)acc_q[i]);
            }
        }
    } else {
        int it = 0;
        for (int t = blockIdx.x; t < num_tiles; t += gridDim.x, ++it) {
            const int ib = it & 1, use = it >> 1;
            if (use > 0) mbar_wait(idx_empty + 8 * ib, (use - 1) & 1);
            const uint32_t dst0 = idx_base + ib * kIdxBytes;
            const int row0 = t * kTileM;
            load_table_slice<kTileM>(dst0, nbr, n_out, row0, n_out, kvol, lane);
            cp_async_arrive_noinc(idx_full + 8 * ib);
            mbar_arrive(idx_full + 8 * ib);
        }
    }
    __syncthreads();
    if (warp == 8) {
        asm volatile("tcgen05.fence::after_thread_sync;" ::: "memory");
        asm volatile("tcgen05.dealloc.cta_group::1.sync.aligned.b32 %0, %1;" ::"r"(tmem_base), "n"(C::kTmemCols) : "memory");
    }
}

__global__ void f32_to_bf16_kernel(const float *__restrict__ in, long long n4, __nv_bfloat16 *__restrict__ out) {
    for (long long i = blockIdx.x * (long long)blockDim.x + threadIdx.x; i < n4; i += (long long)gridDim.x * blockDim.x) {
        float4 v = __ldg((const float4 *)in + i);
        __nv_bfloat162 lo = __floats2bfloat162_rn(v.x, v.y), hi = __floats2bfloat162_rn(v.z, v.w);
        uint2 o;
        o.x = *(uint32_t *)&lo;
        o.y = *(uint32_t *)&hi;
        ((uint2 *)out)[i] = o;
    }
}

__global__ void f32_to_bf16_pad_kernel(const float *__restrict__ in, long long n, int cin, int cpad,
                                       __nv_bfloat16 *__restrict__ out) {
    long long total = n * cpad;
    for (long long e = blockIdx.x * (long long)blockDim.x + threadIdx.x; e < total; e += (long long)gridDim.x * blockDim.x) {
        long long r = e / cpad;
        int c = (int)(e - r * cpad);
        out[e] = __float2bfloat16_rn(c < cin ? __ldg(in + r * cin + c) : 0.f);
    }
}

__global__ void weight_to_kmajor_bf16_kernel(const float *__restrict__ w, int kvol, int cin, int cpad, int cout,
                                             __nv_bfloat16 *__restrict__ wb) {
    size_t per = (size_t)kvol * cpad * cout;
    for (size_t e = blockIdx.x * (size_t)blockDim.x + threadIdx.x; e < per; e += (size_t)gridDim.x * blockDim.x) {
        size_t kc = e % ((size_t)kvol * cpad);
        int co = (int)(e / ((size_t)kvol * cpad));
        int k = (int)(kc / cpad), ci = (int)(kc % cpad);
        wb[e] = __float2bfloat16_rn(ci < cin ? __ldg(w + ((size_t)k * cin + ci) * cout + co) : 0.f);
    }
}

__global__ void table_tile_masks_kernel(const int *__restrict__ nbr, int n_out, int kvol, int num_tiles, uint32_t *__restrict__ masks) {
    const int t = (blockIdx.x * blockDim.x + threadIdx.x) >> 5, lane = threadIdx.x & 31;
    if (t >= num_tiles) return;
    const int row0 = t * kTileM;
    uint32_t m = 0;
    for (int k = 0; k < kvol; ++k) {
        const int *src = nbr + (size_t)k * n_out + row0;
        int any = 0;
#pragma unroll
        for (int j = 0; j < kTileM / 32; ++j) {
            const int r = lane + 32 * j;
            if (row0 + r < n_out) any |= (__ldg(src + r) >= 0);
        }
        if (__any_sync(0xffffffffu, any)) m |= 1u << k;
    }
    if (lane == 0) masks[t] = m;
}

}

extern "C" int toda_table_tile_masks(const int32_t *nbr, int n_out, int kvol, uint32_t *masks, void *stream) {
    TODA_CHECK_ARG(n_out >= 0 && kvol > 0 && kvol <= 32, "table_tile_masks: bad sizes n_out=%d kvol=%d", n_out, kvol);
    if (n_out == 0) return TODA_OK;
    TODA_CHECK_ARG(nbr && masks, "table_tile_masks: null pointer");
    const int num_tiles = ceil_div(n_out, kTileM);
    table_tile_masks_kernel<<<ceil_div(num_tiles * 32, 256), 256, 0, (cudaStream_t)stream>>>(nbr, n_out, kvol, num_tiles, masks);
    TODA_LAUNCH_OK();
    return TODA_OK;
}

static inline int pad16(int c) { return c < 16 ? 16 : c; }

int conv_tma_fwd(const void *xb, int n_in, int cin, const int32_t *nbr, int n_out, int kvol, const void *wb, int cout,
                 const float *bias, const float *addend, float *y, const int32_t *out_rows, const uint32_t *tile_masks, double *bn_sums,
                 cudaStream_t st);

static long long *g_dbg_timeline = nullptr;
extern "C" void toda_debug_set_timeline(long long *buf) { g_dbg_timeline = buf; }
long long *conv_tc_debug_timeline() { return g_dbg_timeline; }
static int g_dbg_mode = 0;
extern "C" void toda_debug_set_mode(int m) { g_dbg_mode = m; }
int conv_tc_debug_mode() { return g_dbg_mode; }

extern "C" int toda_weight_kmajor_bf16(const float *w, int kvol, int cin, int cout, void *w_bf16, void *stream) {
    TODA_CHECK_ARG(w && w_bf16 && kvol > 0 && cin > 0 && cout > 0, "weight_kmajor_bf16: bad args");
    const int cp = cin < 16 ? 16 : cin;
    weight_to_kmajor_bf16_kernel<<<wave_grid((int64_t)kvol * cp * cout, 256), 256, 0, (cudaStream_t)stream>>>(w, kvol, cin, cp, cout,
                                                                                                            (__nv_bfloat16 *)w_bf16);
    TODA_LAUNCH_OK();
    return TODA_OK;
}

bool conv_tc_supported(int cin, int cout, int kvol) {
    bool cin_ok = (cin >= 1 && cin < 16) || cin == 16 || cin == 32 || cin == 64 || cin == 128;
    return cin_ok && kvol <= kMaxKvol && (cout == 16 || cout == 32 || cout == 64 || cout == 128);
}

size_t conv_tc_fwd_workspace_bytes(int n_in, int cin, int cout, int kvol) {
    int cp = pad16(cin);
    return align_up((size_t)n_in * cp * 2 + 16, 256) + align_up((size_t)kvol * cp * cout * 2, 256) + 256;
}

int conv_tc_fwd(const float *x, const void *x_bf16, int n_in, int cin, const int32_t *nbr, int n_out, int kvol, const float *w,
                int cout, const float *bias, float *y, const int32_t *out_rows, const uint32_t *tile_masks, double *bn_sums,
                void *workspace, size_t workspace_bytes,
                cudaStream_t st, const TilePlan *plan, const float *addend, const void *w_bf16) {
    size_t need = conv_tc_fwd_workspace_bytes(n_in, cin, cout, kvol);
    if (!workspace || workspace_bytes < need) {
        toda_set_error("spconv_fwd(bf16): workspace %zu < required %zu bytes", workspace_bytes, need);
        return TODA_ERR_WORKSPACE;
    }
    const int cp = pad16(cin);
    __nv_bfloat16 *xb = (__nv_bfloat16 *)workspace;
    __nv_bfloat16 *wb = (__nv_bfloat16 *)((char *)workspace + align_up((size_t)n_in * cp * 2 + 16, 256));
    if (cp == cin && x_bf16) {
        xb = (__nv_bfloat16 *)x_bf16;
    } else if (cp == cin) {
        long long n4 = (long long)n_in * cin / 4;
        if (n4 > 0) {
            f32_to_bf16_kernel<<<wave_grid(n4, 256), 256, 0, st>>>(x, n4, xb);
            TODA_LAUNCH_OK();
        }
    } else if (n_in > 0) {
        f32_to_bf16_pad_kernel<<<wave_grid((int64_t)n_in * cp, 256), 256, 0, st>>>(x, n_in, cin, cp, xb);
        TODA_LAUNCH_OK();
    }
    if (w_bf16) {
        wb = (__nv_bfloat16 *)w_bf16;
    } else {
        weight_to_kmajor_bf16_kernel<<<wave_grid((int64_t)kvol * cp * cout, 256), 256, 0, st>>>(w, kvol, cin, cp, cout, wb);
        TODA_LAUNCH_OK();
    }
    cin = cp;
    if (bn_sums) TODA_CUDA_OK(cudaMemsetAsync(bn_sums, 0, 2 * (size_t)cout * sizeof(double), st));
    static int feed = -1;
    if (feed < 0) { const char *e = getenv("TODA_TC_FEED"); feed = !e ? 2 : (e[0] == 'c' ? 0 : (e[0] == 't' && e[1] == 'm' ? 1 : 2)); }
    if (feed == 2 && conv_ts_supported(cin, cout, kvol, plan))
        return conv_ts_fwd(xb, n_in, cin, nbr, n_out, kvol, *plan, wb, cout, bias, addend, y, out_rows, tile_masks, bn_sums, st);
    if (feed == 1 || (feed == 2 && cin == 128 && cout == 128))
        {
        return conv_tma_fwd(xb, n_in, cin, nbr, n_out, kvol, wb, cout, bias, addend, y, out_rows, out_rows ? tile_masks : nullptr, bn_sums, st);
    }
    int num_tiles = ceil_div(n_out, kTileM);
    int grid = num_tiles < kNumSMs ? num_tiles : kNumSMs;
    CUtensorMap map_w;
    if (int rc = conv_tma_make_map(&map_w, wb, (uint64_t)cout, (uint64_t)kvol * cin, (uint32_t)cout, kChunkK)) return rc;
#define LAUNCH_TC(CI, CO)                                                                                                    \
    do {                                                                                                                     \
        constexpr int KB_ = (CO) <= 64 ? 2 : 1;                                                                              \
        constexpr int smem = FwdCfg<CO, KB_>::kSmem;                                                                         \
        static bool attr_set = false;                                                                                        \
        if (!attr_set) {                                                                                                     \
            TODA_CUDA_OK(cudaFuncSetAttribute(conv_tc_fwd_kernel<CI, CO, KB_>, cudaFuncAttributeMaxDynamicSharedMemorySize, smem)); \
            attr_set = true;                                                                                                 \
        }                                                                                                                    \
        conv_tc_fwd_kernel<CI, CO, KB_><<<grid, kFwdThreads, smem, st>>>(xb, nbr, n_out, kvol, map_w, bias, addend, y, out_rows, tile_masks, bn_sums, num_tiles, g_dbg_timeline); \
    } while (0)
#define LAUNCH_TC_CO(CI)                                                                                 \
    switch (cout) {                                                                                      \
        case 16: LAUNCH_TC(CI, 16); break;                                                               \
        case 32: LAUNCH_TC(CI, 32); break;                                                               \
        case 64: LAUNCH_TC(CI, 64); break;                                                               \
        case 128: LAUNCH_TC(CI, 128); break;                                                             \
        default: toda_set_error("conv_tc_fwd: unsupported cout %d", cout); return TODA_ERR_UNSUPPORTED;  \
    }
    switch (cin) {
        case 16: LAUNCH_TC_CO(16); break;
        case 32: LAUNCH_TC_CO(32); break;
        case 64: LAUNCH_TC_CO(64); break;
        case 128: LAUNCH_TC_CO(128); break;
        default: toda_set_error("conv_tc_fwd: unsupported cin %d", cin); return TODA_ERR_UNSUPPORTED;
    }
#undef LAUNCH_TC_CO
#undef LAUNCH_TC
    TODA_LAUNCH_OK();
    return TODA_OK;
}

namespace {

template <int NPAD, int ROWS> struct WCfg {
    static constexpr int kATile = 2 * ROWS * 128;
    static constexpr int kBTile = (NPAD / 64) * ROWS * 128;
    static constexpr int kIdx = 32 * ROWS * 4;
    static constexpr int kBBufs = ROWS == 128 ? 2 : 3;
    static constexpr int kStages = ROWS == 128 ? 4 : 8;
    static constexpr int kLag = ROWS == 128 ? 2 : 3;
    static constexpr int kSmem = kStages * kATile + kBBufs * kBTile + 2 * kIdx + 1024 + 256;
};
constexpr int kWgradThreads = kProdThreads + 32 + 128 + 32;

__device__ __forceinline__ uint64_t make_desc_mn_sw128(uint32_t smem_addr, uint32_t lbo_bytes) {
    uint64_t d = 0;
    d |= (uint64_t)((smem_addr >> 4) & 0x3fff);
    d |= (uint64_t)((lbo_bytes >> 4) & 0x3fff) << 16;
    d |= (uint64_t)(1024 >> 4) << 32;
    d |= (uint64_t)1 << 46;
    d |= (uint64_t)2 << 61;
    return d;
}

template <int CIN, int NPAD, int ROWS>
__global__ void __launch_bounds__(kWgradThreads, 1) conv_tc_wgrad_kernel(const __nv_bfloat16 *__restrict__ xb,
                                                                         const int *__restrict__ nbr, int n_out, int kvol,
                                                                         const __nv_bfloat16 *__restrict__ dyb, int cout,
                                                                         int rows_per_split, int passes_per_cta,
                                                                         float *__restrict__ partial) {
    using W = WCfg<NPAD, ROWS>;
    constexpr int kOffsPerPass = 128 / CIN;
    constexpr int S = W::kStages;
    constexpr int kRowsW = ROWS, kATileW = W::kATile, kBTileW = W::kBTile, kIdxW = W::kIdx, kBBufsW = W::kBBufs;
    constexpr int kRowIters = ROWS / 32;
    extern __shared__ uint8_t smem_raw[];
    const uint32_t raw = smem_u32(smem_raw);
    const uint32_t base = (raw + 1023u) & ~1023u;
    const uint32_t b_base = base + S * kATileW;
    const uint32_t idx_base = b_base + kBBufsW * kBTileW;
    const uint32_t bar_base = idx_base + 2 * kIdxW;
    const uint32_t a_full = bar_base, a_empty = bar_base + 8 * S;
    const uint32_t b_full = bar_base + 16 * S, b_empty = b_full + 32;
    const uint32_t idx_full = b_full + 64, idx_empty = b_full + 80;
    const uint32_t accum_bar = b_full + 96, tmem_slot = b_full + 104;
    volatile uint32_t *tmem_slot_ptr = (volatile uint32_t *)(smem_raw + (tmem_slot - raw));

    const int tid = threadIdx.x, warp = tid >> 5, lane = tid & 31;
    const int split = blockIdx.x, group = blockIdx.y;
    const int total_passes = (kvol + kOffsPerPass - 1) / kOffsPerPass;
    const int pass0 = group * passes_per_cta;
    const int npass = min(passes_per_cta, total_passes - pass0);
    const int k0 = pass0 * kOffsPerPass;
    const int noffs = min(npass * kOffsPerPass, kvol - k0);
    const int r_begin = split * rows_per_split;
    const int r_end = min(n_out, r_begin + rows_per_split);
    const int nchunks = r_end > r_begin ? (r_end - r_begin + kRowsW - 1) / kRowsW : 0;

    if (tid == 0) {
        for (int s = 0; s < S; ++s) {
            mbar_init(a_full + 8 * s, kProdThreads / 32);
            mbar_init(a_empty + 8 * s, 1);
        }
        for (int b = 0; b < kBBufsW; ++b) {
            mbar_init(b_full + 8 * b, kProdThreads / 32);
            mbar_init(b_empty + 8 * b, 1);
        }
        for (int b = 0; b < 2; ++b) {
            mbar_init(idx_full + 8 * b, 64);
            mbar_init(idx_empty + 8 * b, kProdThreads);
        }
        mbar_init(accum_bar, 1);
        asm volatile("fence.mbarrier_init.release.cluster;" ::: "memory");
    }
    uint32_t tmem_cols = 32;
    while ((int)tmem_cols < passes_per_cta * NPAD) tmem_cols <<= 1;
    if (warp == 8) {
        asm volatile("tcgen05.alloc.cta_group::1.sync.aligned.shared::cta.b32 [%0], %1;" ::"r"(tmem_slot), "r"(tmem_cols) : "memory");
        asm volatile("tcgen05.relinquish_alloc_permit.cta_group::1.sync.aligned;" ::: "memory");
    }
    asm volatile("tcgen05.fence::before_thread_sync;" ::: "memory");
    __syncthreads();
    asm volatile("tcgen05.fence::after_thread_sync;" ::: "memory");
    const uint32_t tmem_base = *tmem_slot_ptr;

    if (warp < 8) {
        const int p = tid & 7, rbase = tid >> 3;
        const uint32_t piece_off = (uint32_t)(rbase * 128 + ((p ^ (rbase & 7)) << 4));
        const int off_lo = CIN >= 64 ? 0 : p / (CIN / 8);
        const int ci_lo = CIN >= 64 ? p * 8 : (p % (CIN / 8)) * 8;
        constexpr int kLagW = W::kLag;
        int g = 0, signalled = 0;
        for (int rc = 0; rc < nchunks; ++rc) {
            const int ib = rc & 1, use_i = rc >> 1;
            const int bb = rc % kBBufsW, use_b = rc / kBBufsW;
            const int row_base = r_begin + rc * kRowsW;
            if (npass < kLagW) {
                asm volatile("cp.async.wait_group 0;" ::: "memory");
                asm volatile("fence.proxy.async.shared::cta;" ::: "memory");
                __syncwarp();
                if (lane == 0)
                    for (; signalled < g; ++signalled) {
                        if (signalled % npass == 0) mbar_arrive(b_full + 8 * ((signalled / npass) % kBBufsW));
                        mbar_arrive(a_full + 8 * (signalled % S));
                    }
                signalled = g;
            }
            if (use_b > 0) mbar_wait(b_empty + 8 * bb, (use_b - 1) & 1);
            {
                const uint32_t b_dst = b_base + bb * kBTileW + piece_off;
#pragma unroll
                for (int nb = 0; nb < NPAD / 64; ++nb) {
                    const int co = nb * 64 + p * 8;
#pragma unroll
                    for (int i = 0; i < kRowIters; ++i) {
                        const int row = row_base + rbase + 32 * i;
                        const uint32_t dst = b_dst + nb * (kRowsW * 128) + i * 4096;
                        if (row < r_end && co < cout) cp_async_16(dst, dyb + (size_t)row * cout + co, 16u);
                        else st_shared_zero16(dst);
                    }
                }
            }
            mbar_wait(idx_full + 8 * ib, use_i & 1);
            const uint32_t idx_tile = idx_base + ib * kIdxW + 4 * rbase;
            for (int ps = 0; ps < npass; ++ps, ++g) {
                const int s = g % S, use = g / S;
                if (use > 0) mbar_wait(a_empty + 8 * s, (use - 1) & 1);
                const uint32_t a_dst = base + s * kATileW + piece_off;
#pragma unroll
                for (int mb = 0; mb < 2; ++mb) {
                    const int koff = ps * kOffsPerPass + (CIN == 128 ? 0 : (CIN == 64 ? mb : mb * (kOffsPerPass / 2) + off_lo));
                    const int ci = CIN == 128 ? mb * 64 + ci_lo : ci_lo;
                    const bool k_ok = koff < noffs;
                    int src[kRowIters];
#pragma unroll
                    for (int i = 0; i < kRowIters; ++i) {
                        src[i] = -1;
                        if (k_ok) asm volatile("ld.shared.b32 %0, [%1];" : "=r"(src[i]) : "r"(idx_tile + 4 * (koff * kRowsW + 32 * i)));
                    }
#pragma unroll
                    for (int i = 0; i < kRowIters; ++i) {
                        const uint32_t dst = a_dst + mb * (kRowsW * 128) + i * 4096;
                        if (src[i] >= 0) cp_async_16(dst, xb + (size_t)(unsigned)src[i] * CIN + ci, 16u);
                        else st_shared_zero16(dst);
                    }
                }
                asm volatile("cp.async.commit_group;" ::: "memory");
                if (g - signalled >= kLagW) {
                    asm volatile("cp.async.wait_group %0;" ::"n"(kLagW) : "memory");
                    asm volatile("fence.proxy.async.shared::cta;" ::: "memory");
                    __syncwarp();
                    const int j = signalled;
                    if (lane == 0) {
                        if (j % npass == 0) mbar_arrive(b_full + 8 * ((j / npass) % kBBufsW));
                        mbar_arrive(a_full + 8 * (j % S));
                    }
                    ++signalled;
                }
            }
            mbar_arrive(idx_empty + 8 * ib);
        }
        asm volatile("cp.async.wait_group 0;" ::: "memory");
        asm volatile("fence.proxy.async.shared::cta;" ::: "memory");
        __syncwarp();
        if (lane == 0)
            for (int j = signalled; j < g; ++j) {
                if (j % npass == 0) mbar_arrive(b_full + 8 * ((j / npass) % kBBufsW));
                mbar_arrive(a_full + 8 * (j % S));
            }
    } else if (warp == 8) {
        if (nchunks > 0) {
            constexpr uint32_t idesc = make_idesc_bf16(128, NPAD) | (1u << 15) | (1u << 16);
            int g = 0;
            uint32_t ready = 0;
            for (int rc = 0; rc < nchunks; ++rc) {
                const int ib = rc % kBBufsW;
                mbar_wait(b_full + 8 * ib, (rc / kBBufsW) & 1);
                const uint32_t b_tile = b_base + ib * kBTileW;
                for (int ps = 0; ps < npass; ++ps, ++g) {
                    const int s = g % S, use = g / S;
                    if (!ready) mbar_wait(a_full + 8 * s, use & 1);
                    ready = mbar_test(a_full + 8 * ((g + 1) % S), ((g + 1) / S) & 1);
                    asm volatile("tcgen05.fence::after_thread_sync;" ::: "memory");
                    const uint32_t a_tile = base + s * kATileW;
                    if (elect_one()) {
#pragma unroll
                        const uint64_t ad0 = make_desc_mn_sw128(a_tile, kRowsW * 128), bd0 = make_desc_mn_sw128(b_tile, kRowsW * 128);
                        umma_bf16(tmem_base + ps * NPAD, ad0, bd0, idesc, rc != 0);
                        for (int j = 1; j < kRowsW / 16; ++j)
                            umma_bf16(tmem_base + ps * NPAD, ad0 + 128 * j, bd0 + 128 * j, idesc, 1u);
                        umma_commit(a_empty + 8 * s);
                    }
                    __syncwarp();
                }
                if (elect_one()) umma_commit(b_empty + 8 * ib);
                __syncwarp();
            }
            if (elect_one()) umma_commit(accum_bar);
            __syncwarp();
        }
    } else if (warp < 13) {
        const int q = warp & 3;
        if (nchunks > 0) {
            mbar_wait(accum_bar, 0);
            asm volatile("tcgen05.fence::after_thread_sync;" ::: "memory");
        }
        const int m = q * 32 + lane;
        for (int ps = 0; ps < npass; ++ps) {
            const int k = (pass0 + ps) * kOffsPerPass + m / CIN, ci = m % CIN;
            float *dst = partial + (((size_t)split * kvol + k) * CIN + ci) * cout;
            const uint32_t taddr = tmem_base + ((uint32_t)(q * 32) << 16) + ps * NPAD;
            for (int n0 = 0; n0 < cout; n0 += 16) {
                uint32_t v[16];
                if (nchunks > 0) {
                    asm volatile(
                        "tcgen05.ld.sync.aligned.32x32b.x16.b32 {%0,%1,%2,%3,%4,%5,%6,%7,%8,%9,%10,%11,%12,%13,%14,%15}, [%16];"
                        : "=r"(v[0]), "=r"(v[1]), "=r"(v[2]), "=r"(v[3]), "=r"(v[4]), "=r"(v[5]), "=r"(v[6]), "=r"(v[7]),
                          "=r"(v[8]), "=r"(v[9]), "=r"(v[10]), "=r"(v[11]), "=r"(v[12]), "=r"(v[13]), "=r"(v[14]), "=r"(v[15])
                        : "r"(taddr + n0));
                    asm volatile("tcgen05.wait::ld.sync.aligned;" ::: "memory");
                } else {
#pragma unroll
                    for (int qq = 0; qq < 16; ++qq) v[qq] = 0u;
                }
                if (k < kvol) {
#pragma unroll
                    for (int qq = 0; qq < 4; ++qq)
                        *(float4 *)(dst + n0 + 4 * qq) = make_float4(__uint_as_float(v[4 * qq]), __uint_as_float(v[4 * qq + 1]),
                                                                     __uint_as_float(v[4 * qq + 2]), __uint_as_float(v[4 * qq + 3]));
                }
            }
        }
        asm volatile("tcgen05.fence::before_thread_sync;" ::: "memory");
    } else {
        for (int rc = 0; rc < nchunks; ++rc) {
            const int ib = rc & 1, use = rc >> 1;
            if (use > 0) mbar_wait(idx_empty + 8 * ib, (use - 1) & 1);
            const uint32_t dst0 = idx_base + ib * kIdxW;
            const int row_base = r_begin + rc * kRowsW;
            load_table_slice<ROWS>(dst0, nbr + (size_t)k0 * n_out, n_out, row_base, r_end, noffs, lane);
            cp_async_arrive_noinc(idx_full + 8 * ib);
            mbar_arrive(idx_full + 8 * ib);
        }
    }
    __syncthreads();
    if (warp == 8) {
        asm volatile("tcgen05.fence::after_thread_sync;" ::: "memory");
        asm volatile("tcgen05.dealloc.cta_group::1.sync.aligned.b32 %0, %1;" ::"r"(tmem_base), "r"(tmem_cols) : "memory");
    }
}

__global__ void __launch_bounds__(256) wgrad_tc_reduce_kernel(const float *__restrict__ partial, int splits, int kvol, int cin,
                                                              int cpad, int cout, float *__restrict__ dw_param) {
    __shared__ float red[8][33];
    const size_t per_pad = (size_t)kvol * cpad * cout;
    const int x = threadIdx.x & 31, y = threadIdx.x >> 5;
    for (size_t e0 = (size_t)blockIdx.x * 32; e0 < per_pad; e0 += (size_t)gridDim.x * 32) {
        const size_t e = e0 + x;
        float s = 0.f;
        if (e < per_pad) {
#pragma unroll 4
            for (int sp = y; sp < splits; sp += 8) s += __ldg(partial + sp * per_pad + e);
        }
        red[y][x] = s;
        __syncthreads();
        if (y == 0 && e < per_pad) {
            s = ((red[0][x] + red[1][x]) + (red[2][x] + red[3][x])) + ((red[4][x] + red[5][x]) + (red[6][x] + red[7][x]));
            const int co = (int)(e % cout);
            const size_t t = e / cout;
            const int ci = (int)(t % cpad), k = (int)(t / cpad);
            if (ci < cin) dw_param[((size_t)co * kvol + k) * cin + ci] = s;
        }
        __syncthreads();
    }
}

struct WgradPlan {
    int passes_per_cta, groups, splits, rows_per_split;
    size_t xb_bytes, dyb_bytes, partial_bytes;
};

WgradPlan wgrad_plan(int n_in, int n_out, int kvol, int cin, int cout) {
    WgradPlan p;
    int npad = cout <= 64 ? 64 : 128;
    const int kRowsW = npad == 64 ? 128 : 64;
    int offs = 128 / cin;
    int total_passes = (kvol + offs - 1) / offs;
    p.passes_per_cta = total_passes < 512 / npad ? total_passes : 512 / npad;
    p.groups = (total_passes + p.passes_per_cta - 1) / p.passes_per_cta;
    int want = kNumSMs / p.groups;
    if (want < 1) want = 1;
    int max_by_rows = (n_out + 4 * kRowsW - 1) / (4 * kRowsW);
    p.splits = want < max_by_rows ? want : max_by_rows;
    if (p.splits < 1) p.splits = 1;
    int rps = (n_out + p.splits - 1) / p.splits;
    p.rows_per_split = (rps + kRowsW - 1) / kRowsW * kRowsW;
    if (p.rows_per_split < kRowsW) p.rows_per_split = kRowsW;
    p.xb_bytes = align_up((size_t)n_in * cin * 2 + 16, 256);
    p.dyb_bytes = align_up((size_t)n_out * cout * 2 + 16, 256);
    p.partial_bytes = align_up((size_t)p.splits * kvol * cin * cout * 4, 256);
    return p;
}

}

bool conv_tc_wgrad_supported(int cin, int cout, int kvol) {
    return kvol <= kMaxKvol && ((cin >= 1 && cin <= 16) || cin == 32 || cin == 64 || cin == 128) && (cout == 16 || cout == 32 || cout == 64 || cout == 128);
}

size_t conv_tc_wgrad_workspace_bytes(int n_in, int n_out, int kvol, int cin, int cout) {
    WgradPlan p = wgrad_plan(n_in, n_out, kvol, pad16(cin), cout);
    return p.xb_bytes + p.dyb_bytes + p.partial_bytes + 256;
}

int conv_tc_wgrad(const float *x, const void *x_bf16, int n_in, int cin, const int32_t *nbr, int n_out, int kvol,
                  const float *dy, const void *dy_bf16, int cout, float *dw_param, void *workspace, size_t workspace_bytes,
                  cudaStream_t st) {
    const int cin_real = cin;
    cin = pad16(cin);
    WgradPlan p = wgrad_plan(n_in, n_out, kvol, cin, cout);
    size_t need = p.xb_bytes + p.dyb_bytes + p.partial_bytes;
    if (!workspace || workspace_bytes < need) {
        toda_set_error("spconv_wgrad(bf16): workspace %zu < required %zu bytes", workspace_bytes, need);
        return TODA_ERR_WORKSPACE;
    }
    __nv_bfloat16 *xb = (__nv_bfloat16 *)workspace;
    __nv_bfloat16 *dyb = (__nv_bfloat16 *)((char *)workspace + p.xb_bytes);
    float *partial = (float *)((char *)workspace + p.xb_bytes + p.dyb_bytes);
    long long n4 = (long long)n_in * cin / 4;
    if (cin_real != cin) {
        if (n_in > 0) {
            f32_to_bf16_pad_kernel<<<wave_grid((int64_t)n_in * cin, 256), 256, 0, st>>>(x, n_in, cin_real, cin, xb);
            TODA_LAUNCH_OK();
        }
    } else if (x_bf16) {
        xb = (__nv_bfloat16 *)x_bf16;
    } else if (n4 > 0) {
        f32_to_bf16_kernel<<<wave_grid(n4, 256), 256, 0, st>>>(x, n4, xb);
        TODA_LAUNCH_OK();
    }
    if (dy_bf16) {
        dyb = (__nv_bfloat16 *)dy_bf16;
    } else {
        n4 = (long long)n_out * cout / 4;
        f32_to_bf16_kernel<<<wave_grid(n4, 256), 256, 0, st>>>(dy, n4, dyb);
        TODA_LAUNCH_OK();
    }
    dim3 grid(p.splits, p.groups);
#define LAUNCH_W(CI, NP, RW)                                                                                              \
    do {                                                                                                                   \
        constexpr int smem = WCfg<NP, RW>::kSmem;                                                                          \
        static bool attr_set = false;                                                                                      \
        if (!attr_set) {                                                                                                   \
            TODA_CUDA_OK(cudaFuncSetAttribute(conv_tc_wgrad_kernel<CI, NP, RW>, cudaFuncAttributeMaxDynamicSharedMemorySize, smem)); \
            attr_set = true;                                                                                               \
        }                                                                                                                  \
        conv_tc_wgrad_kernel<CI, NP, RW><<<grid, kWgradThreads, smem, st>>>(xb, nbr, n_out, kvol, dyb, cout, p.rows_per_split,  \
                                                                           p.passes_per_cta, partial);                      \
    } while (0)
    const bool wide = cout > 64;
    switch (cin) {
        case 16: if (wide) LAUNCH_W(16, 128, 64); else LAUNCH_W(16, 64, 128); break;
        case 32: if (wide) LAUNCH_W(32, 128, 64); else LAUNCH_W(32, 64, 128); break;
        case 64: if (wide) LAUNCH_W(64, 128, 64); else LAUNCH_W(64, 64, 128); break;
        case 128: if (wide) LAUNCH_W(128, 128, 64); else LAUNCH_W(128, 64, 128); break;
        default: toda_set_error("conv_tc_wgrad: unsupported cin %d", cin); return TODA_ERR_UNSUPPORTED;
    }
#undef LAUNCH_W
    TODA_LAUNCH_OK();
    size_t per_pad = (size_t)kvol * cin * cout;
    wgrad_tc_reduce_kernel<<<wave_grid(per_pad * 8, 256), 256, 0, st>>>(partial, p.splits, kvol, cin_real, cin, cout, dw_param);
    TODA_LAUNCH_OK();
    return TODA_OK;
}
```

toda_b200/csrc/conv_x3.cu:

```cuda
#include <cuda_bf16.h>

#include "common.cuh"
#include "conv_ts.cuh"

int conv_tc_fwd(const float *x, const void *x_bf16, int n_in, int cin, const int32_t *nbr, int n_out, int kvol, const float *w,
                int cout, const float *bias, float *y, const int32_t *out_rows, const uint32_t *tile_masks, double *bn_sums,
                void *workspace, size_t workspace_bytes,
                cudaStream_t st, const TilePlan *plan, const float *addend, const void *w_bf16);
size_t conv_tc_fwd_workspace_bytes(int n_in, int cin, int cout, int kvol);
int conv_tc_wgrad(const float *x, const void *x_bf16, int n_in, int cin, const int32_t *nbr, int n_out, int kvol,
                  const float *dy, const void *dy_bf16, int cout, float *dw_param, void *workspace, size_t workspace_bytes,
                  cudaStream_t st);
size_t conv_tc_wgrad_workspace_bytes(int n_in, int n_out, int kvol, int cin, int cout);

namespace {

static inline int pad16(int c) { return c < 16 ? 16 : c; }

__device__ __forceinline__ void split_bf16(float v, __nv_bfloat16 &hi, __nv_bfloat16 &lo) {
    hi = __float2bfloat16_rn(v);
    lo = __float2bfloat16_rn(v - __bfloat162float(hi));
}

__global__ void split_rows_kernel(const float *__restrict__ in, long long n, int cin, int cpad, __nv_bfloat16 *__restrict__ hi,
                                  __nv_bfloat16 *__restrict__ lo) {
    const long long total = n * cpad;
    for (long long e = blockIdx.x * (long long)blockDim.x + threadIdx.x; e < total; e += (long long)gridDim.x * blockDim.x) {
        const long long r = e / cpad;
        const int c = (int)(e - r * cpad);
        __nv_bfloat16 h, l;
        split_bf16(c < cin ? __ldg(in + r * cin + c) : 0.f, h, l);
        hi[e] = h;
        lo[e] = l;
    }
}

__global__ void split_weights_kernel(const float *__restrict__ w, int kvol, int cin, int cpad, int cout, __nv_bfloat16 *__restrict__ hi,
                                     __nv_bfloat16 *__restrict__ lo) {
    const size_t per = (size_t)kvol * cpad * cout;
    for (size_t e = blockIdx.x * (size_t)blockDim.x + threadIdx.x; e < per; e += (size_t)gridDim.x * blockDim.x) {
        const size_t kc = e % ((size_t)kvol * cpad);
        const int co = (int)(e / ((size_t)kvol * cpad));
        const int k = (int)(kc / cpad), ci = (int)(kc % cpad);
        __nv_bfloat16 h, l;
        split_bf16(ci < cin ? __ldg(w + ((size_t)k * cin + ci) * cout + co) : 0.f, h, l);
        hi[e] = h;
        lo[e] = l;
    }
}

__global__ void sum3_unpad_kernel(const float *__restrict__ t1, const float *__restrict__ t2, const float *__restrict__ t3, size_t rows,
                                  int cpad, int cin, float *__restrict__ dw) {
    const size_t total = rows * cin;
    for (size_t e = blockIdx.x * (size_t)blockDim.x + threadIdx.x; e < total; e += (size_t)gridDim.x * blockDim.x) {
        const size_t r = e / cin;
        const int c = (int)(e - r * cin);
        const size_t s = r * cpad + c;
        dw[e] = (t1[s] + t2[s]) + t3[s];
    }
}

struct X3Fwd { size_t x_bytes, w_bytes, inner; };
X3Fwd x3_fwd_layout(int n_in, int cin, int cout, int kvol) {
    const int cp = pad16(cin);
    X3Fwd l;
    l.x_bytes = align_up((size_t)(n_in > 0 ? n_in : 1) * cp * 2 + 16, 256);
    l.w_bytes = align_up((size_t)kvol * cp * cout * 2, 256);
    l.inner = conv_tc_fwd_workspace_bytes(n_in, cp, cout, kvol);
    return l;
}

struct X3Wgrad { size_t x_bytes, dy_bytes, t_bytes, inner; };
X3Wgrad x3_wgrad_layout(int n_in, int n_out, int kvol, int cin, int cout) {
    const int cp = pad16(cin);
    X3Wgrad l;
    l.x_bytes = align_up((size_t)(n_in > 0 ? n_in : 1) * cp * 2 + 16, 256);
    l.dy_bytes = align_up((size_t)(n_out > 0 ? n_out : 1) * cout * 2 + 16, 256);
    l.t_bytes = align_up((size_t)kvol * cp * cout * 4, 256);
    l.inner = conv_tc_wgrad_workspace_bytes(n_in, n_out, kvol, cp, cout);
    return l;
}

}

size_t conv_x3_fwd_workspace_bytes(int n_in, int cin, int cout, int kvol) {
    X3Fwd l = x3_fwd_layout(n_in, cin, cout, kvol);
    return 2 * l.x_bytes + 2 * l.w_bytes + l.inner + 256;
}

int conv_x3_fwd(const float *x, int n_in, int cin, const int32_t *nbr, int n_out, int kvol, const float *w, int cout, const float *bias,
                float *y, const int32_t *out_rows, const uint32_t *tile_masks, double *bn_sums, void *workspace, size_t workspace_bytes,
                cudaStream_t st, const TilePlan *plan, const float *addend) {
    const size_t need = conv_x3_fwd_workspace_bytes(n_in, cin, cout, kvol);
    if (!workspace || workspace_bytes < need) {
        toda_set_error("spconv_fwd(bf16x3): workspace %zu < required %zu bytes", workspace_bytes, need);
        return TODA_ERR_WORKSPACE;
    }
    const int cp = pad16(cin);
    X3Fwd l = x3_fwd_layout(n_in, cin, cout, kvol);
    char *p = (char *)workspace;
    __nv_bfloat16 *xh = (__nv_bfloat16 *)p, *xl = (__nv_bfloat16 *)(p + l.x_bytes);
    __nv_bfloat16 *wh = (__nv_bfloat16 *)(p + 2 * l.x_bytes), *wl = (__nv_bfloat16 *)(p + 2 * l.x_bytes + l.w_bytes);
    void *inner = p + 2 * l.x_bytes + 2 * l.w_bytes;
    if (n_in > 0) {
        split_rows_kernel<<<wave_grid((int64_t)n_in * cp, 256), 256, 0, st>>>(x, n_in, cin, cp, xh, xl);
        TODA_LAUNCH_OK();
    }
    split_weights_kernel<<<wave_grid((int64_t)kvol * cp * cout, 256), 256, 0, st>>>(w, kvol, cin, cp, cout, wh, wl);
    TODA_LAUNCH_OK();
    int rc = conv_tc_fwd(x, xh, n_in, cp, nbr, n_out, kvol, w, cout, bias, y, out_rows, tile_masks, nullptr, inner, l.inner, st, plan, addend, wh);
    if (rc) return rc;
    rc = conv_tc_fwd(x, xh, n_in, cp, nbr, n_out, kvol, w, cout, nullptr, y, out_rows, tile_masks, nullptr, inner, l.inner, st, plan, y, wl);
    if (rc) return rc;
    return conv_tc_fwd(x, xl, n_in, cp, nbr, n_out, kvol, w, cout, nullptr, y, out_rows, tile_masks, bn_sums, inner, l.inner, st, plan, y, wh);
}

size_t conv_x3_wgrad_workspace_bytes(int n_in, int n_out, int kvol, int cin, int cout) {
    X3Wgrad l = x3_wgrad_layout(n_in, n_out, kvol, cin, cout);
    return 2 * l.x_bytes + 2 * l.dy_bytes + 3 * l.t_bytes + l.inner + 256;
}

int conv_x3_wgrad(const float *x, int n_in, int cin, const int32_t *nbr, int n_out, int kvol, const float *dy, int cout, float *dw_param,
                  void *workspace, size_t workspace_bytes, cudaStream_t st) {
    const size_t need = conv_x3_wgrad_workspace_bytes(n_in, n_out, kvol, cin, cout);
    if (!workspace || workspace_bytes < need) {
        toda_set_error("spconv_wgrad(bf16x3): workspace %zu < required %zu bytes", workspace_bytes, need);
        return TODA_ERR_WORKSPACE;
    }
    const int cp = pad16(cin);
    X3Wgrad l = x3_wgrad_layout(n_in, n_out, kvol, cin, cout);
    char *p = (char *)workspace;
    __nv_bfloat16 *xh = (__nv_bfloat16 *)p, *xl = (__nv_bfloat16 *)(p + l.x_bytes);
    __nv_bfloat16 *dh = (__nv_bfloat16 *)(p + 2 * l.x_bytes), *dl = (__nv_bfloat16 *)(p + 2 * l.x_bytes + l.dy_bytes);
    float *t1 = (float *)(p + 2 * l.x_bytes + 2 * l.dy_bytes), *t2 = (float *)((char *)t1 + l.t_bytes), *t3 = (float *)((char *)t2 + l.t_bytes);
    void *inner = (char *)t3 + l.t_bytes;
    split_rows_kernel<<<wave_grid((int64_t)n_in * cp, 256), 256, 0, st>>>(x, n_in, cin, cp, xh, xl);
    TODA_LAUNCH_OK();
    split_rows_kernel<<<wave_grid((int64_t)n_out * cout, 256), 256, 0, st>>>(dy, n_out, cout, cout, dh, dl);
    TODA_LAUNCH_OK();
    int rc = conv_tc_wgrad(x, xh, n_in, cp, nbr, n_out, kvol, dy, dh, cout, t1, inner, l.inner, st);
    if (rc) return rc;
    rc = conv_tc_wgrad(x, xh, n_in, cp, nbr, n_out, kvol, dy, dl, cout, t2, inner, l.inner, st);
    if (rc) return rc;
    rc = conv_tc_wgrad(x, xl, n_in, cp, nbr, n_out, kvol, dy, dh, cout, t3, inner, l.inner, st);
    if (rc) return rc;
    const size_t rows = (size_t)cout * kvol;
    sum3_unpad_kernel<<<wave_grid((int64_t)rows * cin, 256), 256, 0, st>>>(t1, t2, t3, rows, cp, cin, dw_param);
    TODA_LAUNCH_OK();
    return TODA_OK;
}
```

toda_b200/csrc/layer.cu:

```cuda
#include "common.cuh"

static int layer_conv(const toda_layer_fwd_args *p, double *bn_sums, void *stream) {
    return toda_spconv_fwd_plan(p->x, p->x_bf16, p->n_in, p->cin, p->nbr, p->n_out, p->kvol, p->w, p->cout, p->bias, nullptr, p->y,
                                nullptr, p->tile_masks, p->plan_lidx, p->plan_rows, p->plan_cnt, p->plan_groups, p->plan_cap,
                                bn_sums, p->w_bf16, p->precision, p->conv_ws, p->conv_ws_bytes, stream);
}

static int layer_fwd_stats(const toda_layer_fwd_args *p, double *sums, double *count, void *stream) {
    const int c = p->cout, n = p->n_out;
    const bool tc = n > 0 && toda_spconv_uses_tensor_cores(p->cin, c, p->kvol, p->precision);
    int rc = layer_conv(p, tc ? sums : nullptr, stream);
    if (rc) return rc;
    return toda_bn_local_sums(p->y, tc ? sums : nullptr, n, c, sums, count, p->bn_ws, p->bn_ws_bytes, stream);
}

static int layer_fwd_apply(const toda_layer_fwd_args *p, const double *sums, const double *count, void *stream) {
    const int c = p->cout;
    float *scale = p->stats, *shift = p->stats + c, *mean = p->stats + 2 * c, *rstd = p->stats + 3 * c;
    return toda_bn_apply_sums(p->y, p->n_out, c, sums, count, p->gamma, p->beta, p->eps, p->momentum, p->running_mean,
                              p->running_var, scale, shift, mean, rstd, p->residual, p->relu, p->a, p->a_bf16, stream);
}

extern "C" int toda_layer_fwd(const toda_layer_fwd_args *p, void *stream) {
    TODA_CHECK_ARG(p, "layer_fwd: null args");
    const int c = p->cout, n = p->n_out;
    TODA_CHECK_ARG(c > 0 && n >= 0 && p->stats && (n == 0 || (p->y && p->a)) && (!p->training || p->sums),
                   "layer_fwd: bad sizes / null outputs");
    if (n == 0) return layer_conv(p, nullptr, stream);
    int rc;
    if (p->training) {
        rc = layer_fwd_stats(p, p->sums, nullptr, stream);
        return rc ? rc : layer_fwd_apply(p, p->sums, nullptr, stream);
    }
    float *scale = p->stats, *shift = p->stats + c;
    if ((rc = layer_conv(p, nullptr, stream))) return rc;
    if ((rc = toda_bn_eval_coeffs(p->gamma, p->beta, p->running_mean, p->running_var, p->eps, c, scale, shift, stream))) return rc;
    return toda_bn_apply(p->y, n, c, scale, shift, p->residual, p->relu, p->a, p->a_bf16, stream);
}

static int layer_bwd_empty(const toda_layer_bwd_args *p, bool bn_grads, cudaStream_t st) {
    const int c = p->cout;
    if (bn_grads && p->dgamma) TODA_CUDA_OK(cudaMemsetAsync(p->dgamma, 0, sizeof(float) * c, st));
    if (bn_grads && p->dbeta) TODA_CUDA_OK(cudaMemsetAsync(p->dbeta, 0, sizeof(float) * c, st));
    if (p->need_db && p->db) TODA_CUDA_OK(cudaMemsetAsync(p->db, 0, sizeof(float) * c, st));
    if (p->need_dw && p->dw) TODA_CUDA_OK(cudaMemsetAsync(p->dw, 0, sizeof(float) * (size_t)p->kvol * p->cin * c, st));
    if (p->need_dx && p->dx && p->n_in > 0) {
        if (p->addend) TODA_CUDA_OK(cudaMemcpyAsync(p->dx, p->addend, sizeof(float) * (size_t)p->n_in * p->cin, cudaMemcpyDeviceToDevice, st));
        else TODA_CUDA_OK(cudaMemsetAsync(p->dx, 0, sizeof(float) * (size_t)p->n_in * p->cin, st));
    }
    return TODA_OK;
}

static bool layer_bwd_reads_dy_f32(const toda_layer_bwd_args *p) {
    const int c = p->cout;
    return p->need_db || !p->dy_bf16 || p->precision != TODA_CONV_BF16 ||
           (p->need_dx && !toda_spconv_uses_tensor_cores(c, p->cin, p->kvol, p->precision)) ||
           (p->need_dw && !toda_spconv_wgrad_uses_tensor_cores(p->cin, c, p->kvol, p->precision));
}

static int layer_bwd_conv(const toda_layer_bwd_args *p, void *stream) {
    const int c = p->cout, n = p->n_out;
    int rc;
    if (p->need_dx) {
        rc = toda_spconv_fwd_plan(p->dy, p->dy_bf16, n, c, p->dgrad_nbr, p->n_in, p->kvol, p->wt, p->cin, nullptr, p->addend, p->dx,
                                  p->dgrad_out_rows, p->dgrad_masks, p->dplan_lidx, p->dplan_rows, p->dplan_cnt, p->dplan_groups,
                                  p->dplan_cap, nullptr, p->wt_bf16, p->precision, p->conv_ws, p->conv_ws_bytes, stream);
        if (rc) return rc;
    }
    if (p->need_dw) {
        rc = toda_spconv_wgrad(p->x, p->x_bf16, p->n_in, p->cin, p->nbr_fwd, n, p->kvol, p->dy, p->dy_bf16, c, p->dw, p->wgrad_ws,
                               p->wgrad_ws_bytes, p->precision, stream);
        if (rc) return rc;
    }
    if (p->need_db) {
        rc = toda_col_sum(p->dy, n, c, p->db, p->bn_ws, p->bn_ws_bytes, stream);
        if (rc) return rc;
    }
    return TODA_OK;
}

static int layer_bwd_reduce(const toda_layer_bwd_args *p, double *red, void *stream) {
    return toda_bn_bwd_reduce(p->da, p->a_mask, p->y, p->n_out, p->cout, p->mean, p->rstd, p->relu, red, p->dgamma, p->dbeta,
                              p->bn_ws, p->bn_ws_bytes, stream);
}

static int layer_bwd_finish(const toda_layer_bwd_args *p, const double *red, const double *count, void *stream) {
    const int c = p->cout, n = p->n_out;
    if (n == 0) return layer_bwd_empty(p, false, (cudaStream_t)stream);
    int rc = toda_bn_bwd_finish(p->da, p->a_mask, p->y, n, c, p->gamma, p->mean, p->rstd, p->relu, p->training, red, count,
                                layer_bwd_reads_dy_f32(p) ? p->dy : nullptr, p->dy_bf16, p->dres, stream);
    return rc ? rc : layer_bwd_conv(p, stream);
}

extern "C" int toda_layer_bwd(const toda_layer_bwd_args *p, void *stream) {
    TODA_CHECK_ARG(p, "layer_bwd: null args");
    TODA_CHECK_ARG(p->cout > 0 && p->n_out >= 0, "layer_bwd: bad sizes");
    if (p->n_out == 0) return layer_bwd_empty(p, true, (cudaStream_t)stream);
    TODA_CHECK_ARG(p->bn_ws, "layer_bwd: null workspace");
    double *red = bn_workspace_red(p->bn_ws, p->cout);
    int rc = layer_bwd_reduce(p, red, stream);
    return rc ? rc : layer_bwd_finish(p, red, nullptr, stream);
}


extern "C" int toda_layer_fwd_stats(const toda_layer_fwd_args *p, double *local_sums, void *stream) {
    TODA_CHECK_ARG(p && local_sums, "layer_fwd_stats: null args");
    const int c = p->cout, n = p->n_out;
    TODA_CHECK_ARG(c > 0 && n >= 0 && p->training && (n == 0 || p->y), "layer_fwd_stats: bad sizes / not training / null y");
    return layer_fwd_stats(p, local_sums, local_sums + 2 * c, stream);
}

extern "C" int toda_layer_fwd_apply(const toda_layer_fwd_args *p, const double *global_sums, void *stream) {
    TODA_CHECK_ARG(p && global_sums, "layer_fwd_apply: null args");
    const int c = p->cout, n = p->n_out;
    TODA_CHECK_ARG(c > 0 && n >= 0 && p->training && p->stats && (n == 0 || (p->y && p->a)),
                   "layer_fwd_apply: bad sizes / not training / null outputs");
    return layer_fwd_apply(p, global_sums, global_sums + 2 * c, stream);
}

extern "C" int toda_layer_bwd_reduce(const toda_layer_bwd_args *p, double *local_red, void *stream) {
    TODA_CHECK_ARG(p && local_red, "layer_bwd_reduce: null args");
    TODA_CHECK_ARG(p->cout > 0 && p->n_out >= 0 && p->training, "layer_bwd_reduce: bad sizes / not training");
    return layer_bwd_reduce(p, local_red, stream);
}

extern "C" int toda_layer_bwd_finish(const toda_layer_bwd_args *p, const double *global_red, const double *global_count,
                                     void *stream) {
    TODA_CHECK_ARG(p && global_red && global_count, "layer_bwd_finish: null args");
    TODA_CHECK_ARG(p->cout > 0 && p->n_out >= 0 && p->training, "layer_bwd_finish: bad sizes / not training");
    return layer_bwd_finish(p, global_red, global_count, stream);
}
```

toda_b200/ops.py:

```python
import ctypes
import weakref
from dataclasses import dataclass
from typing import List, Optional

import numpy as np
import torch
import torch.distributed as dist

from . import _C

ORDER_FIRST_APPEARANCE = 0
ORDER_CANONICAL = 1
CONV_FP32 = 0
CONV_BF16 = 1
CONV_BF16X3 = 2
_TC_PRECISIONS = (CONV_BF16, CONV_BF16X3)

_launch_base = 0


def launches():
    return int(_C.lib().toda_launch_count()) - _launch_base


# ... 273 lines not shown
        _C.check(_C.lib().toda_index_insert(_p(self.buf), *self._dims(), _p(coords), coords.shape[0], _stream()),
                 "toda_index_insert")

    def insert_strided(self, in_coords, ksize, stride, padding):
        self._acquire()
        in_coords = _need(in_coords, torch.int32, "in_coords")
        _C.check(_C.lib().toda_index_insert_strided(_p(self.buf), *self._dims(), _p(in_coords), in_coords.shape[0],
                                                    _C.ints(ksize), _C.ints(stride), _C.ints(padding), _stream()),
                 "toda_index_insert_strided")

    def build(self, cap, known_n=None):
        dev = self.buf.device
        coords = torch.empty((max(cap, 1), 4), dtype=torch.int32, device=dev)
        n_out = torch.empty((self.batch + 1,), dtype=torch.int32, device=dev)
        with _timed("index_build", cells=self.batch * self.shape[0] * self.shape[1] * self.shape[2]):
            _C.check(_C.lib().toda_index_build(_p(self.buf), *self._dims(), _p(coords), cap, _p(n_out), _stream()),
                     "toda_index_build")
        self.n = int(n_out[0].item()) if known_n is None else int(known_n)
        self.coords = coords[:self.n]
        self.frame_counts = n_out
        return self.coords

    def ensure_live(self):
        if _index_occupant.get(self.key) is self:
            return
        if self.coords is None:
            raise RuntimeError("occupancy index was released")
        coords, n = self.coords, self.n
        self.insert(coords)
        self.build(n, known_n=n)

    def rows(self, coords):
        self.ensure_live()
        coords = _need(coords, torch.int32, "coords")
        rows = torch.empty((coords.shape[0],), dtype=torch.int32, device=coords.device)
        _C.check(_C.lib().toda_index_rows(_p(self.buf), *self._dims(), _p(coords), coords.shape[0], _p(rows), _stream()),
                 "toda_index_rows")
        return rows

    def release(self):
        if _index_occupant.get(self.key) is self:
            self._unmark()
        self.coords = None
        self.n = 0


@dataclass
class Rulebook:
    subm: bool
    ksize: List[int]
    stride: List[int]
    padding: List[int]
    in_shape: List[int]
    out_shape: List[int]
    n_in: int
    n_out: int
    out_coords: torch.Tensor
    nbr_fwd: torch.Tensor
    nbr_bwd: Optional[torch.Tensor]
    dgrad_order: Optional[torch.Tensor] = None
    nbr_bwd_sorted: Optional[torch.Tensor] = None
    dgrad_tile_masks: Optional[torch.Tensor] = None
    tile_masks: Optional[torch.Tensor] = None
    plan: Optional["TilePlan"] = None
    dgrad_plan: Optional["TilePlan"] = None

    @property
    def kvol(self):
        return self.ksize[0] * self.ksize[1] * self.ksize[2]


@dataclass
class TilePlan:
    lidx: torch.Tensor
    rows: torch.Tensor
    cnt: torch.Tensor
    ngroups: int
    cap: int

    def tensors(self):
        return [self.lidx, self.rows, self.cnt]


def table_tile_plan(nbr, ksize, channels):
    kvol, n = nbr.shape
    ngroups = int(ksize[0])
    if n == 0 or kvol > 27 or ngroups > 3 or kvol % ngroups or kvol // ngroups > 9 or not channels:
        return None
    L = _C.lib()
    cap = L.toda_tile_plan_capacity(int(channels))
    if cap <= 0:
        return None
    tiles = (n + 127) // 128
    dev = nbr.device
    lidx = torch.empty((tiles, kvol, 128), dtype=torch.int16, device=dev)
    rows = torch.empty((tiles, ngroups, cap), dtype=torch.int32, device=dev)
    cnt = torch.empty((tiles, ngroups), dtype=torch.int32, device=dev)
    with _timed("tile_plan", n=n, kvol=kvol):
        _C.check(L.toda_table_tile_plan(_p(nbr), n, kvol, ngroups, cap, _p(lidx), _p(rows), _p(cnt), _stream()),
                 "toda_table_tile_plan")
    return TilePlan(lidx, rows, cnt, ngroups, cap)


def conv_out_size(in_size, k, s, p):
    return (in_size + 2 * p - (k - 1) - 1) // s + 1


def rulebook_subm(index: OccupancyIndex, ksize, channels=None):
    index.ensure_live()
    n = index.n
    kvol = ksize[0] * ksize[1] * ksize[2]
    nbr = torch.empty((kvol, n), dtype=torch.int32, device=index.buf.device)
    with _timed("rulebook_subm", n=n, kvol=kvol):
        _C.check(_C.lib().toda_rulebook_subm(_p(index.buf), index.batch, *index.shape, _p(index.coords), n, _C.ints(ksize),
                                             _p(nbr), _stream()), "toda_rulebook_subm")
    rb = Rulebook(True, list(ksize), [1, 1, 1], [k // 2 for k in ksize], index.shape, index.shape, n, n, index.coords,
                  nbr, None)
    rb.tile_masks = table_tile_masks(nbr) if (n > 0 and kvol <= 32) else None
    rb.plan = table_tile_plan(nbr, ksize, channels) if _TILE_PLANS else None
    return rb


def rulebook_sparse(index_in: OccupancyIndex, ksize, stride, padding, tag, cin=None, cout=None):
    index_in.ensure_live()
    out_shape = [conv_out_size(index_in.shape[a], ksize[a], stride[a], padding[a]) for a in range(3)]
    index_out = OccupancyIndex(index_in.batch, out_shape, index_in.buf.device, tag)
    if index_out.buf.data_ptr() == index_in.buf.data_ptr():
        index_out = OccupancyIndex(index_in.batch, out_shape, index_in.buf.device, (tag, "alt"))
    assert index_out.buf.data_ptr() != index_in.buf.data_ptr()
    index_out.insert_strided(index_in.coords, ksize, stride, padding)
    per_in = 1
    for a in range(3):
        per_in *= min(ksize[a], (ksize[a] + stride[a] - 1) // stride[a])
    cells = index_in.batch * out_shape[0] * out_shape[1] * out_shape[2]
    cap = int(min(index_in.n * per_in, cells))
    out_coords = index_out.build(cap)
    n_in, n_out = index_in.n, index_out.n
    kvol = ksize[0] * ksize[1] * ksize[2]
    dev = index_in.buf.device
    nbr_fwd = torch.empty((kvol, n_out), dtype=torch.int32, device=dev)
    nbr_bwd = torch.empty((kvol, n_in), dtype=torch.int32, device=dev)
    with _timed("rulebook_sparse", n_in=n_in, n_out=n_out, kvol=kvol):
        _C.check(_C.lib().toda_rulebook_sparse(_p(index_in.buf), *index_in.shape, _p(index_out.buf), *out_shape,
                                               index_in.batch, _p(index_in.coords), n_in, _p(out_coords), n_out,
                                               _C.ints(ksize), _C.ints(stride), _C.ints(padding), _p(nbr_fwd), _p(nbr_bwd),
                                               _stream()), "toda_rulebook_sparse")
    rb = Rulebook(False, list(ksize), list(stride), list(padding), index_in.shape, out_shape, n_in, n_out, out_coords,
                  nbr_fwd, nbr_bwd)
    rb.tile_masks = table_tile_masks(nbr_fwd) if (n_out > 0 and kvol <= 32) else None
    rb.dgrad_order, rb.nbr_bwd_sorted = (_dgrad_parity_order(index_in.coords, nbr_bwd, stride, padding) if kvol <= 32
                                         else (None, None))
    if rb.dgrad_order is not None:
        rb.dgrad_tile_masks = table_tile_masks(rb.nbr_bwd_sorted)
    if _TILE_PLANS:
        rb.plan = table_tile_plan(nbr_fwd, ksize, cin)
        rb.dgrad_plan = table_tile_plan(rb.nbr_bwd_sorted if rb.dgrad_order is not None else nbr_bwd, ksize, cout)
    return rb, index_out


import os as _os
_TILE_PLANS = _os.environ.get("TODA_TILE_PLANS", "0") == "1"


def set_tile_plans(on):
    global _TILE_PLANS
    _TILE_PLANS = bool(on)


def tile_plans_enabled():
    return _TILE_PLANS


def table_tile_masks(nbr):
    kvol, n = nbr.shape
    masks = torch.empty(((n + 127) // 128,), dtype=torch.int32, device=nbr.device)
    _C.check(_C.lib().toda_table_tile_masks(_p(nbr), n, kvol, _p(masks), _stream()), "toda_table_tile_masks")
    return masks


def _dgrad_parity_order(in_coords, nbr_bwd, stride, padding):
    if all(s == 1 for s in stride) or in_coords.shape[0] == 0:
        return None, None
    if stride[0] * stride[1] * stride[2] > 8:
        return None, None
    n = in_coords.shape[0]
    L = _C.lib()
    ws = _workspace("parity", L.toda_parity_order_workspace_bytes(n), in_coords.device)
    order = torch.empty((n,), dtype=torch.int32, device=in_coords.device)
    _C.check(L.toda_parity_order(_p(in_coords), n, _C.ints(stride), _C.ints(padding), _p(order), None, _p(ws), ws.numel(),
                                 _stream()), "toda_parity_order")
    return order, nbr_bwd.index_select(1, order).contiguous()


_repack_cache = {}


def invalidate_weight_cache():
    _repack_cache.clear()


def _repack(weight, transpose, mirror, want_bf16=False):
    key = (id(weight), bool(transpose), bool(mirror))
    hit = _repack_cache.get(key)
    if hit is not None and hit[2]() is weight and hit[0] == weight._version and hit[3] == weight.data_ptr():
        out = hit[1]
    else:
        cout, kvol, cin = weight.shape[0], weight.shape[1] * weight.shape[2] * weight.shape[3], weight.shape[4]
        out = torch.empty((kvol, cout, cin) if transpose else (kvol, cin, cout), dtype=torch.float32, device=weight.device)
        _C.check(_C.lib().toda_weight_repack(_p(weight), kvol, cin, cout, int(transpose), int(mirror), _p(out), _stream()),
                 "toda_weight_repack")
        if len(_repack_cache) > 512:
            _repack_cache.clear()
        hit = [weight._version, out, weakref.ref(weight), weight.data_ptr(), None]
        _repack_cache[key] = hit
    if not want_bf16:
        return out
    if hit[4] is None:
        kvol, ci, co = out.shape
        wb = torch.empty((co, kvol * max(ci, 16)), dtype=torch.bfloat16, device=out.device)
        _C.check(_C.lib().toda_weight_kmajor_bf16(_p(out), kvol, ci, co, _p(wb), _stream()), "toda_weight_kmajor_bf16")
        hit[4] = wb
    return out, hit[4]


def _bf16_shadow_of(t):
    tag = getattr(t, "_toda_bf16", None)
    if tag is not None and tag[1] == t._version and tag[0].shape == t.shape:
        return tag[0]
    return None


def _conv_call(x, xb, cin, nbr, n_out, kvol, w, cout, bias, precision, what="conv_fwd", rb=None, bn_sums=None, y=None,
               out_rows=None, tile_masks=None, plan=None, addend=None, w_bf16=None):
    if y is None:
        y = torch.empty((n_out, cout), dtype=torch.float32, device=x.device)
    L = _C.lib()
    ws_bytes = L.toda_spconv_fwd_workspace_bytes(x.shape[0], cin, cout, kvol, precision)
    ws = _workspace("conv", ws_bytes, x.device) if ws_bytes else None
    if precision not in _TC_PRECISIONS:
        plan = None
    with _timed(what, n_in=x.shape[0], n_out=n_out, cin=cin, cout=cout, kvol=kvol, precision=precision, rb=id(rb)):
        if plan is None and addend is None and w_bf16 is None:
            _C.check(L.toda_spconv_fwd(_p(x), _p(xb), x.shape[0], cin, _p(nbr), n_out, kvol, _p(w), cout, _p(bias), _p(y),
                                       _p(out_rows), _p(tile_masks), _p(bn_sums), precision, _p(ws), ws.numel() if ws is not None else 0,
                                       _stream()), "toda_spconv_fwd")
        else:
            pl = plan
            _C.check(L.toda_spconv_fwd_plan(_p(x), _p(xb), x.shape[0], cin, _p(nbr), n_out, kvol, _p(w), cout, _p(bias),
                                            _p(addend), _p(y), _p(out_rows), _p(tile_masks), _p(pl.lidx) if pl else None,
                                            _p(pl.rows) if pl else None, _p(pl.cnt) if pl else None, pl.ngroups if pl else 0,
                                            pl.cap if pl else 0, _p(bn_sums), _p(w_bf16), precision, _p(ws),
                                            ws.numel() if ws is not None else 0, _stream()), "toda_spconv_fwd_plan")
    return y


def conv_plan_usable(plan, cin, cout, kvol, precision):
    if plan is None or precision not in _TC_PRECISIONS or _os.environ.get("TODA_TC_FEED", "ts")[:1] in ("c",) or \
            _os.environ.get("TODA_TC_FEED", "ts")[:2] == "tm":
        return False
    cp = max(16, cin)
    return (cp in (16, 32, 64, 128) and cout in (16, 32, 64, 128) and kvol <= 27
            and plan.cap <= _C.lib().toda_tile_plan_capacity(cp))


def _conv_forward_impl(x, x_bf16, weight, bias, rb, precision, want_stats):
    x = _need(x.contiguous(), torch.float32, "features")
    weight = _need(weight.contiguous(), torch.float32, "weight")
    cout, cin = weight.shape[0], weight.shape[4]
    assert x.shape == (rb.n_in, cin), (x.shape, rb.n_in, cin)
    if x_bf16 is not None and (precision != CONV_BF16 or x_bf16.shape != x.shape or x_bf16.dtype != torch.bfloat16
                               or not x_bf16.is_contiguous()):
        x_bf16 = None
    w = _repack(weight, False, False)
    b = bias.contiguous() if bias is not None else None
    sums = None
    if want_stats and rb.n_out > 0 and _C.lib().toda_spconv_uses_tensor_cores(cin, cout, rb.kvol, precision):
        sums = torch.empty((2 * cout,), dtype=torch.float64, device=x.device)
    y = _conv_call(x, x_bf16, cin, rb.nbr_fwd, rb.n_out, rb.kvol, w, cout, b, precision, "conv_fwd", rb, sums,
                   tile_masks=rb.tile_masks, plan=rb.plan)
    return y, sums, x, weight, x_bf16


def _conv_backward_impl(dy, dyb, x, weight, xb, rb, precision, need_dx, need_dw, need_db):
    cout, cin = weight.shape[0], weight.shape[4]
    L = _C.lib()
    dx = dw = db = None
    if need_dx:
        wt = _repack(weight, True, rb.subm)
        if rb.subm:
            dx = _conv_call(dy, dyb, cout, rb.nbr_fwd, rb.n_in, rb.kvol, wt, cin, None, precision, "conv_dgrad", rb,
                            tile_masks=rb.tile_masks, plan=rb.plan)
        elif rb.dgrad_order is None:
            dx = _conv_call(dy, dyb, cout, rb.nbr_bwd, rb.n_in, rb.kvol, wt, cin, None, precision, "conv_dgrad", rb,
                            plan=rb.dgrad_plan)
        else:
            dx = _conv_call(dy, dyb, cout, rb.nbr_bwd_sorted, rb.n_in, rb.kvol, wt, cin, None, precision, "conv_dgrad",
                            rb, out_rows=rb.dgrad_order, tile_masks=rb.dgrad_tile_masks, plan=rb.dgrad_plan)
    if need_dw:
        dw = torch.empty_like(weight)
        ws_bytes = L.toda_spconv_wgrad_workspace_bytes(rb.n_in, rb.n_out, rb.kvol, cin, cout, precision)
        ws = _workspace("wgrad", ws_bytes, dy.device)
        with _timed("conv_wgrad", n_in=rb.n_in, n_out=rb.n_out, cin=cin, cout=cout, kvol=rb.kvol, precision=precision,
                    rb=id(rb)):
            _C.check(L.toda_spconv_wgrad(_p(x), _p(xb), rb.n_in, cin, _p(rb.nbr_fwd), rb.n_out, rb.kvol, _p(dy), _p(dyb),
                                         cout, _p(dw), _p(ws), ws.numel(), precision, _stream()), "toda_spconv_wgrad")
    if need_db:
        db = col_sum(dy)
    return dx, dw, db


class _SparseConv(torch.autograd.Function):
    @staticmethod
    def forward(ctx, x, x_bf16, weight, bias, rb: Rulebook, precision, want_stats):
        y, sums, x, weight, x_bf16 = _conv_forward_impl(x, x_bf16, weight, bias, rb, precision, want_stats)
        ctx.save_for_backward(x, weight, x_bf16)
        ctx.set_materialize_grads(False)
        ctx.rb, ctx.precision, ctx.has_bias = rb, precision, bias is not None
        if sums is not None:
            ctx.mark_non_differentiable(sums)
        return y, sums

    @staticmethod
    def backward(ctx, dy, _dsums=None):
        if dy is None:
            return (None,) * 7
        x, weight, xb = ctx.saved_tensors
        dyb = _bf16_shadow_of(dy) if (ctx.precision == CONV_BF16 and dy.is_contiguous()) else None
        dx, dw, db = _conv_backward_impl(dy.contiguous(), dyb, x, weight, xb, ctx.rb, ctx.precision, ctx.needs_input_grad[0],
                                         ctx.needs_input_grad[2], ctx.has_bias and ctx.needs_input_grad[3])
        return dx, None, dw, db, None, None, None


def sparse_conv(x, weight, bias, rb, precision=CONV_FP32, x_bf16=None, want_stats=False):
    y, sums = _SparseConv.apply(x, x_bf16, weight, bias, rb, precision, want_stats)
    return (y, sums) if want_stats else y


def col_sum(t):
    n, c = t.shape
    out = torch.empty((c,), dtype=torch.float32, device=t.device)
    L = _C.lib()
    ws = _workspace("bn", L.toda_bn_workspace_bytes(c), t.device)
    _C.check(L.toda_col_sum(_p(t), n, c, _p(out), _p(ws), ws.numel(), _stream()), "toda_col_sum")
    return out


class ReluMaskTape:

    def __init__(self, mode):
        assert mode in ("record", "replay")
        self.mode, self.masks, self.i = mode, [], 0

    def replay(self):
        self.mode, self.i = "replay", 0
        return self


_relu_tape = None


def set_relu_mask_tape(tape):
    global _relu_tape
    _relu_tape = tape


def sync_group(bn):
    if not isinstance(bn, torch.nn.SyncBatchNorm) or not bn.training:
        return None
    if bn.momentum is None:
        raise NotImplementedError("toda_b200: SyncBatchNorm with momentum=None (cumulative moving average) is not supported; "
                                  "set a momentum (these backbones use 0.01)")
    if not (dist.is_available() and dist.is_initialized()):
        return None
    group = bn.process_group if bn.process_group is not None else dist.group.WORLD
    return group if dist.get_world_size(group) > 1 else None


def _run_phases(phases, group):
    try:
        buf = next(phases)
        while True:
            dist.all_reduce(buf, op=dist.ReduceOp.SUM, group=group)
            buf = phases.send(None)
    except StopIteration as stop:
        return stop.value


def _tape_mask(a, want_bf16):
    if _relu_tape.mode == "record":
        mask = a > 0
        _relu_tape.masks.append(mask)
    else:
        mask = _relu_tape.masks[_relu_tape.i]
        _relu_tape.i += 1
    a = a * mask
    return a, (a.to(torch.bfloat16) if want_bf16 else None), mask.to(torch.float32)


def _bn_forward_phases(y, gamma, beta, running_mean, running_var, eps, momentum, training, residual, relu, want_bf16, sums,
                       need_grad, sync=False):
    y = _need(y.contiguous(), torch.float32, "bn input")
    n, c = y.shape
    dev = y.device
    L = _C.lib()
    scale, shift, mean, rstd = torch.empty((4, c), dtype=torch.float32, device=dev).unbind(0)
    gsums = count = None
    if training:
        if sync or sums is None:
            buf = torch.empty((2 * c + 1 if sync else 2 * c,), dtype=torch.float64, device=dev)
            count = buf.data_ptr() + 16 * c if sync else None
            ws = _workspace("bn", L.toda_bn_workspace_bytes(c), dev)
            with _timed("bn_stats", n=n, c=c):
                _C.check(L.toda_bn_local_sums(_p(y), _p(sums), n, c, _p(buf), count, _p(ws), ws.numel(), _stream()),
                         "toda_bn_local_sums")
            sums = buf
        if sync:
            yield sums
            gsums = sums
    else:
        _C.check(L.toda_bn_eval_coeffs(_p(gamma), _p(beta), _p(running_mean), _p(running_var), float(eps), c, _p(scale),
                                       _p(shift), _stream()), "toda_bn_eval_coeffs")
        mean = running_mean
        rstd = torch.rsqrt(running_var + eps) if need_grad else None
    res = residual.contiguous() if residual is not None else None
    a = torch.empty_like(y)
    tape = _relu_tape is not None and relu
    ab = torch.empty(y.shape, dtype=torch.bfloat16, device=dev) if (want_bf16 and not tape) else None
    act = 0 if tape else int(relu)
    with _timed("bn_apply", n=n, c=c, residual=res is not None):
        if training:
            _C.check(L.toda_bn_apply_sums(_p(y), n, c, _p(sums), count, _p(gamma), _p(beta), float(eps), float(momentum),
                                          _p(running_mean), _p(running_var), _p(scale), _p(shift), _p(mean), _p(rstd), _p(res),
                                          act, _p(a), _p(ab), _stream()), "toda_bn_apply_sums")
        else:
            _C.check(L.toda_bn_apply(_p(y), n, c, _p(scale), _p(shift), _p(res), act, _p(a), _p(ab), _stream()), "toda_bn_apply")
    if tape:
        a, ab, mask = _tape_mask(a, want_bf16)
        return a, ab, y, mean, rstd, mask, gsums
    return a, ab, y, mean, rstd, a, gsums


def _bn_backward_phases(da, y, a, gamma, mean, rstd, training, relu, has_res, want_bf16, gsums=None):
    n, c = y.shape
    da = da.contiguous() if da is not None else torch.zeros_like(y)
    L = _C.lib()
    dy = torch.empty_like(y)
    dyb = torch.empty(y.shape, dtype=torch.bfloat16, device=y.device) if want_bf16 else None
    dres = torch.empty_like(y) if has_res else None
    dgamma, dbeta = torch.empty((2, c), dtype=torch.float32, device=y.device).unbind(0)
    ws = _workspace("bn", L.toda_bn_workspace_bytes(c), y.device)
    if gsums is None:
        with _timed("bn_bwd", n=n, c=c, residual=has_res):
            _C.check(L.toda_bn_bwd(_p(da), _p(a), _p(y), n, c, _p(gamma), _p(mean), _p(rstd), int(relu), int(training),
                                   _p(dy), _p(dyb), _p(dres), _p(dgamma), _p(dbeta), _p(ws), ws.numel(), _stream()), "toda_bn_bwd")
        return dy, dyb, dres, dgamma, dbeta
    red = torch.empty((2 * c,), dtype=torch.float64, device=y.device)
    _C.check(L.toda_bn_bwd_reduce(_p(da), _p(a), _p(y), n, c, _p(mean), _p(rstd), int(relu), _p(red), _p(dgamma), _p(dbeta),
                                  _p(ws), ws.numel(), _stream()), "toda_bn_bwd_reduce")
    yield red
    _C.check(L.toda_bn_bwd_finish(_p(da), _p(a), _p(y), n, c, _p(gamma), _p(mean), _p(rstd), int(relu), 1, _p(red),
                                  gsums.data_ptr() + 16 * c, _p(dy), _p(dyb), _p(dres), _stream()), "toda_bn_bwd_finish")
    return dy, dyb, dres, dgamma, dbeta


class _BNAct(torch.autograd.Function):
    @staticmethod
    def forward(ctx, y, gamma, beta, running_mean, running_var, eps, momentum, training, residual, relu, want_bf16, sums, group):
        a, ab, y, mean, rstd, a_mask, gsums = _run_phases(
            _bn_forward_phases(y, gamma, beta, running_mean, running_var, eps, momentum, training, residual, relu, want_bf16, sums,
                        y.requires_grad or gamma.requires_grad, group is not None), group)
        ctx.save_for_backward(y, a_mask, gamma, mean, rstd, gsums)
        ctx.set_materialize_grads(False)
        ctx.cfg = (bool(training), bool(relu), residual is not None, bool(want_bf16))
        ctx.group = group
        if ab is not None:
            ctx.mark_non_differentiable(ab)
        return a, ab

    @staticmethod
    def backward(ctx, da, _dab=None):
        if da is None and ctx.group is None:
            return (None,) * 13
        y, a, gamma, mean, rstd, gsums = ctx.saved_tensors
        training, relu, has_res, want_bf16 = ctx.cfg
        dy, dyb, dres, dgamma, dbeta = _run_phases(_bn_backward_phases(da, y, a, gamma, mean, rstd, training, relu, has_res,
                                                                       want_bf16, gsums), ctx.group)
        if dyb is not None:
            dy._toda_bf16 = (dyb, dy._version)
        return dy, dgamma, dbeta, None, None, None, None, None, dres, None, None, None, None


def _vp(t):
    return t.data_ptr() if t is not None else None


def _fused_ok(training, need_grad):
    return _prof is None and _relu_tape is None and (training or not need_grad)


def _layer_forward(x, x_bf16, weight, bias, rb, precision, gamma, beta, running_mean, running_var, eps, momentum, training,
                   residual, relu, want_bf16, need_grad=True, group=None):
    return _run_phases(_layer_forward_phases(x, x_bf16, weight, bias, rb, precision, gamma, beta, running_mean, running_var, eps,
                                             momentum, residual, relu, want_bf16, need_grad, training, group is not None), group)


def _layer_forward_phases(x, x_bf16, weight, bias, rb, precision, gamma, beta, running_mean, running_var, eps, momentum,
                          residual, relu, want_bf16, need_grad=True, training=True, sync=True):
    if not _fused_ok(training, need_grad):
        y, sums, x, weight, x_bf16 = _conv_forward_impl(x, x_bf16, weight, bias, rb, precision, bool(training))
        a, ab, y, mean, rstd, a_mask, gsums = yield from _bn_forward_phases(y, gamma, beta, running_mean, running_var, eps,
                                                                            momentum, training, residual, relu, want_bf16, sums,
                                                                            need_grad, sync)
        return a, ab, (x, x_bf16, weight, y, a_mask, gamma, mean, rstd, gsums)
    args, x, x_bf16, weight, y, a, ab, small, _keep = _layer_fwd_args(
        x, x_bf16, weight, bias, rb, precision, gamma, beta, running_mean, running_var, eps, momentum, training, residual, relu,
        want_bf16)
    cout = y.shape[1]
    L = _C.lib()
    gsums = None
    if sync:
        gsums = torch.empty((2 * cout + 1,), dtype=torch.float64, device=y.device)
        _C.check(L.toda_layer_fwd_stats(ctypes.byref(args), _p(gsums), _stream()), "toda_layer_fwd_stats")
        yield gsums
        _C.check(L.toda_layer_fwd_apply(ctypes.byref(args), _p(gsums), _stream()), "toda_layer_fwd_apply")
    else:
        _C.check(L.toda_layer_fwd(ctypes.byref(args), _stream()), "toda_layer_fwd")
    mean = small[2 * cout:3 * cout] if training else running_mean
    rstd = small[3 * cout:4 * cout] if training else None
    return a, ab, (x, x_bf16, weight, y, a, gamma, mean, rstd, gsums)


def _layer_fwd_args(x, x_bf16, weight, bias, rb, precision, gamma, beta, running_mean, running_var, eps, momentum, training,
                    residual, relu, want_bf16):
    x = _need(x.contiguous(), torch.float32, "features")
    weight = _need(weight.contiguous(), torch.float32, "weight")
    cout, cin = weight.shape[0], weight.shape[4]
    assert x.shape == (rb.n_in, cin), (x.shape, rb.n_in, cin)
    if x_bf16 is not None and (precision != CONV_BF16 or x_bf16.shape != x.shape or x_bf16.dtype != torch.bfloat16
                               or not x_bf16.is_contiguous()):
        x_bf16 = None
    L = _C.lib()
    kvol, n_out, dev = rb.kvol, rb.n_out, x.device
    tc = bool(L.toda_spconv_uses_tensor_cores(cin, cout, kvol, precision))
    if tc and precision == CONV_BF16:
        w, wb = _repack(weight, False, False, True)
    else:
        w, wb = _repack(weight, False, False), None
    y = torch.empty((n_out, cout), dtype=torch.float32, device=dev)
    a = torch.empty_like(y)
    ab = torch.empty((n_out, cout), dtype=torch.bfloat16, device=dev) if want_bf16 else None
    small = torch.empty((8 * cout,), dtype=torch.float32, device=dev)
    ws_bytes = L.toda_spconv_fwd_workspace_bytes(x.shape[0], cin, cout, kvol, precision)
    ws = _workspace("conv", ws_bytes, dev) if ws_bytes else None
    bws = _workspace("bn", L.toda_bn_workspace_bytes(cout), dev)
    res = residual.contiguous() if residual is not None else None
    b = bias.contiguous() if bias is not None else None
    pl = rb.plan if precision in _TC_PRECISIONS else None
    sp = small.data_ptr()
    args = _C.LayerFwdArgs(
        x.data_ptr(), _vp(x_bf16), x.shape[0], cin, rb.nbr_fwd.data_ptr(), n_out, kvol, w.data_ptr(), _vp(wb), cout, _vp(b),
        _vp(rb.tile_masks), _vp(pl.lidx) if pl else None, _vp(pl.rows) if pl else None, _vp(pl.cnt) if pl else None,
        pl.ngroups if pl else 0, pl.cap if pl else 0, precision, _vp(ws), ws.numel() if ws is not None else 0,
        gamma.data_ptr(), beta.data_ptr(), float(eps), float(momentum), _vp(running_mean), _vp(running_var), int(bool(training)),
        _vp(res), int(bool(relu)), y.data_ptr(), sp + 16 * cout, sp, a.data_ptr(), _vp(ab), bws.data_ptr(), bws.numel())
    return args, x, x_bf16, weight, y, a, ab, small, (w, wb, ws, bws, res, b)


def _layer_backward(da, saved, rb, precision, training, relu, has_res, has_bias, need_dx, need_dw, addend=None, group=None):
    return _run_phases(_layer_backward_phases(da, saved, rb, precision, relu, has_res, has_bias, need_dx, need_dw, addend,
                                              training), group)


def _layer_backward_phases(da, saved, rb, precision, relu, has_res, has_bias, need_dx, need_dw, addend=None, training=True):
    x, xb, weight, y, a_mask, gamma, mean, rstd, gsums = saved
    if da is None:
        da = torch.zeros_like(y)
    if not _fused_ok(training, True):
        dy, dyb, dres, dgamma, dbeta = yield from _bn_backward_phases(da, y, a_mask, gamma, mean, rstd, training, relu, has_res,
                                                                      precision == CONV_BF16, gsums)
        dx, dw, db = _conv_backward_impl(dy, dyb, x, weight, xb, rb, precision, need_dx, need_dw, has_bias)
        if addend is not None and dx is not None:
            dx = dx + addend
        return dx, dw, db, dgamma, dbeta, dres
    args, dx, dw, dres, small, _keep = _layer_bwd_args(da, saved, rb, precision, training, relu, has_res, has_bias, need_dx,
                                                       need_dw, addend)
    cout = y.shape[1]
    L = _C.lib()
    if gsums is None:
        _C.check(L.toda_layer_bwd(ctypes.byref(args), _stream()), "toda_layer_bwd")
    else:
        red = torch.empty((2 * cout,), dtype=torch.float64, device=y.device)
        _C.check(L.toda_layer_bwd_reduce(ctypes.byref(args), _p(red), _stream()), "toda_layer_bwd_reduce")
        yield red
        _C.check(L.toda_layer_bwd_finish(ctypes.byref(args), _p(red), gsums.data_ptr() + 16 * cout, _stream()),
                 "toda_layer_bwd_finish")
    return dx, dw, (small[2 * cout:] if has_bias else None), small[:cout], small[cout:2 * cout], dres


def _layer_bwd_args(da, saved, rb, precision, training, relu, has_res, has_bias, need_dx, need_dw, addend):
    x, xb, weight, y, a_mask, gamma, mean, rstd, _ = saved
    L = _C.lib()
    da = da.contiguous()
    n_out, cout = y.shape
    cin, kvol, dev = weight.shape[4], rb.kvol, y.device
    bf16 = precision == CONV_BF16
    dy = torch.empty_like(y)
    dyb = torch.empty(y.shape, dtype=torch.bfloat16, device=dev) if bf16 else None
    dres = torch.empty_like(y) if has_res else None
    small = torch.empty((3 * cout,), dtype=torch.float32, device=dev)
    bws = _workspace("bn", L.toda_bn_workspace_bytes(cout), dev)
    dx = dw = None
    wt = wtb = None
    nbr = out_rows = masks = pl = None
    if need_dx:
        tc = bool(L.toda_spconv_uses_tensor_cores(cout, cin, kvol, precision))
        if tc and precision == CONV_BF16:
            wt, wtb = _repack(weight, True, rb.subm, True)
        else:
            wt = _repack(weight, True, rb.subm)
        if rb.subm:
            nbr, masks, pl = rb.nbr_fwd, rb.tile_masks, rb.plan
        elif rb.dgrad_order is None:
            nbr, pl = rb.nbr_bwd, rb.dgrad_plan
        else:
            nbr, out_rows, masks, pl = rb.nbr_bwd_sorted, rb.dgrad_order, rb.dgrad_tile_masks, rb.dgrad_plan
        if precision not in _TC_PRECISIONS:
            pl = None
        dx = torch.empty((rb.n_in, cin), dtype=torch.float32, device=dev)
        if addend is not None:
            addend = addend.contiguous()
    ws_bytes = L.toda_spconv_fwd_workspace_bytes(n_out, cout, cin, kvol, precision) if need_dx else 0
    ws = _workspace("conv", ws_bytes, dev) if ws_bytes else None
    wws = None
    if need_dw:
        dw = torch.empty_like(weight)
        wws = _workspace("wgrad", L.toda_spconv_wgrad_workspace_bytes(rb.n_in, n_out, kvol, cin, cout, precision), dev)
    sp = small.data_ptr()
    args = _C.LayerBwdArgs(
        da.data_ptr(), a_mask.data_ptr(), y.data_ptr(), n_out, cout, gamma.data_ptr(), _vp(mean), _vp(rstd), int(relu), int(training),
        dy.data_ptr(), _vp(dyb), _vp(dres), sp, sp + 4 * cout, bws.data_ptr(), bws.numel(),
        x.data_ptr(), _vp(xb), rb.n_in, cin, kvol,
        int(bool(need_dx)), _vp(nbr), _vp(wt), _vp(wtb), _vp(out_rows), _vp(masks),
        _vp(pl.lidx) if pl else None, _vp(pl.rows) if pl else None, _vp(pl.cnt) if pl else None, pl.ngroups if pl else 0,
        pl.cap if pl else 0, _vp(addend) if need_dx else None, _vp(dx),
        int(bool(need_dw)), rb.nbr_fwd.data_ptr(), _vp(dw), _vp(wws), wws.numel() if wws is not None else 0,
        int(bool(has_bias)), sp + 8 * cout, precision, _vp(ws), ws.numel() if ws is not None else 0)
    return args, dx, dw, dres, small, (da, dy, dyb, addend, wt, wtb, ws, wws, bws)


class _ConvBNAct(torch.autograd.Function):

    @staticmethod
    def forward(ctx, x, x_bf16, weight, bias, rb, precision, gamma, beta, running_mean, running_var, eps, momentum, training,
                residual, relu, want_bf16, group):
        need_grad = any(ctx.needs_input_grad)
        a, ab, saved = _layer_forward(x, x_bf16, weight, bias, rb, precision, gamma, beta, running_mean, running_var, eps, momentum,
                                      training, residual, relu, want_bf16, need_grad, group)
        if need_grad:
            ctx.save_for_backward(*saved)
        ctx.set_materialize_grads(False)
        ctx.rb, ctx.precision, ctx.has_bias, ctx.group = rb, precision, bias is not None, group
        ctx.cfg = (bool(training), bool(relu), residual is not None, bool(want_bf16))
        if ab is not None:
            ctx.mark_non_differentiable(ab)
        return a, ab

    @staticmethod
    def backward(ctx, da, _dab=None):
        if da is None and ctx.group is None:
            return (None,) * 17
        training, relu, has_res, want_bf16 = ctx.cfg
        dx, dw, db, dgamma, dbeta, dres = _layer_backward(da, ctx.saved_tensors, ctx.rb, ctx.precision, training, relu, has_res,
                                                          ctx.has_bias and ctx.needs_input_grad[3], ctx.needs_input_grad[0],
                                                          ctx.needs_input_grad[2], group=ctx.group)
        return dx, None, dw, db, None, None, dgamma, dbeta, None, None, None, None, None, dres, None, None, None


class _ResBlock(torch.autograd.Function):

    @staticmethod
    def forward(ctx, x, x_bf16, w1, b1, g1, be1, rm1, rv1, w2, b2, g2, be2, rm2, rv2, rb, precision, eps, momentum, training, want_bf16,
                group1, group2):
        need_grad = any(ctx.needs_input_grad)
        h, hb, s1 = _layer_forward(x, x_bf16, w1, b1, rb, precision, g1, be1, rm1, rv1, eps, momentum, training, None, True,
                                   want_bf16, need_grad, group1)
        out, outb, s2 = _layer_forward(h, hb, w2, b2, rb, precision, g2, be2, rm2, rv2, eps, momentum, training, s1[0], True,
                                       want_bf16, need_grad, group2)
        if need_grad:
            ctx.save_for_backward(*s1, *s2)
        ctx.set_materialize_grads(False)
        ctx.rb, ctx.precision, ctx.training = rb, precision, bool(training)
        ctx.groups = (group1, group2)
        ctx.has_bias = (b1 is not None, b2 is not None)
        if outb is not None:
            ctx.mark_non_differentiable(outb)
        return out, outb

    @staticmethod
    def backward(ctx, dout, _db=None):
        if dout is None and ctx.groups == (None, None):
            return (None,) * 22
        sv = ctx.saved_tensors
        s1, s2 = sv[:9], sv[9:]
        ng = ctx.needs_input_grad
        dh, dw2, db2, dg2, dbe2, dres = _layer_backward(dout, s2, ctx.rb, ctx.precision, ctx.training, True, True,
                                                        ctx.has_bias[1] and ng[9], True, ng[8], group=ctx.groups[1])
        dx, dw1, db1, dg1, dbe1, _ = _layer_backward(dh, s1, ctx.rb, ctx.precision, ctx.training, True, False,
                                                     ctx.has_bias[0] and ng[3], ng[0], ng[2], addend=dres if ng[0] else None,
                                                     group=ctx.groups[0])
        return (dx, None, dw1, db1, dg1, dbe1, None, None, dw2, db2, dg2, dbe2, None, None, None, None, None, None, None, None,
                None, None)


def _bn_call(bn):
    group = sync_group(bn)
    training = bn.training or bn.running_mean is None
    if training and bn.running_mean is not None and bn.num_batches_tracked is not None:
        bn.num_batches_tracked += 1
    return training, group


def res_block(x, x_bf16, conv1_w, conv1_b, bn1, conv2_w, conv2_b, bn2, rb, precision, want_bf16=False):
    (training, group1), (training2, group2) = _bn_call(bn1), _bn_call(bn2)
    assert bn1.eps == bn2.eps and bn1.momentum == bn2.momentum and training == training2
    return _ResBlock.apply(x, x_bf16, conv1_w, conv1_b, bn1.weight, bn1.bias, bn1.running_mean, bn1.running_var, conv2_w, conv2_b,
                           bn2.weight, bn2.bias, bn2.running_mean, bn2.running_var, rb, precision, bn1.eps, bn1.momentum, training,
                           want_bf16, group1, group2)


def conv_bn_act(x, weight, bias, rb, precision, bn: torch.nn.BatchNorm1d, residual=None, relu=True, x_bf16=None, want_bf16=False):
    training, group = _bn_call(bn)
    return _ConvBNAct.apply(x, x_bf16, weight, bias, rb, precision, bn.weight, bn.bias, bn.running_mean, bn.running_var, bn.eps,
                            bn.momentum, training, residual, relu, want_bf16, group)


def bn_act(y, bn: torch.nn.BatchNorm1d, residual=None, relu=True, want_bf16=False, sums=None):
    training, group = _bn_call(bn)
    a, ab = _BNAct.apply(y, bn.weight, bn.bias, bn.running_mean, bn.running_var, bn.eps, bn.momentum, training, residual,
                         relu, want_bf16, sums if training else None, group)
    return (a, ab) if want_bf16 else a


class _BEVScatter(torch.autograd.Function):
    @staticmethod
    def forward(ctx, features, coords, batch, d, h, w):
        features = _need(features.contiguous(), torch.float32, "features")
        coords = _need(coords, torch.int32, "indices")
        n, c = features.shape
        out = torch.empty((batch, c * d, h, w), dtype=torch.float32, device=features.device)
        with _timed("bev_scatter_fwd", n=n, c=c, out_elems=out.numel()):
            _C.check(_C.lib().toda_bev_scatter_fwd(_p(features), _p(coords), n, c, batch, d, h, w, _p(out), _stream()),
                     "toda_bev_scatter_fwd")
        ctx.save_for_backward(coords)
        ctx.dims = (n, c, batch, d, h, w)
        return out

    @staticmethod
    def backward(ctx, dout):
        (coords,) = ctx.saved_tensors
        n, c, batch, d, h, w = ctx.dims
        dout = dout.contiguous()
        df = torch.empty((n, c), dtype=torch.float32, device=dout.device)
        with _timed("bev_scatter_bwd", n=n, c=c):
            _C.check(_C.lib().toda_bev_scatter_bwd(_p(dout), _p(coords), n, c, batch, d, h, w, _p(df), _stream()),
                     "toda_bev_scatter_bwd")
        return df, None, None, None, None, None


def bev_scatter(features, coords, batch, d, h, w):
    return _BEVScatter.apply(features, coords, batch, d, h, w)


class _GatherRows(torch.autograd.Function):
    @staticmethod
    def forward(ctx, x, rows, inverse_rows):
        x = _need(x.contiguous(), torch.float32, "features")
        n, c = rows.shape[0], x.shape[1]
        out = torch.empty((n, c), dtype=torch.float32, device=x.device)
        _C.check(_C.lib().toda_gather_rows(_p(x), _p(rows), n, c, _p(out), _stream()), "toda_gather_rows")
        ctx.save_for_backward(inverse_rows)
        return out

    @staticmethod
    def backward(ctx, dout):
        (inv,) = ctx.saved_tensors
        dout = dout.contiguous()
        n, c = inv.shape[0], dout.shape[1]
        dx = torch.empty((n, c), dtype=torch.float32, device=dout.device)
        _C.check(_C.lib().toda_gather_rows(_p(dout), _p(inv), n, c, _p(dx), _stream()), "toda_gather_rows")
        return dx, None, None


def permute_rows(x, rows, inverse_rows):
    return _GatherRows.apply(x, rows, inverse_rows)
```

Baseline: 399.6.

## Fuse conv bias gradient into BN backward apply and pass tile masks to wgrad

The bias gradient (column sum of dy) is now accumulated inside the BN backward apply kernel. Each block writes per-channel partials, and a small finalize kernel reduces them, replacing a separate col_sum pass over dy. This also lets the layer skip writing the fp32 dy when only bf16 is needed. Forward tile masks are threaded into the tensor-core wgrad path (with a new row-splits API), apparently so empty tiles can be skipped, but the cost is an extra shared-memory reduction and a capped grid in the apply kernel.

Result: faster. 420.5 (median of 6 runs) (+5.2%).

```diff
diff --git a/include/toda_b200.h b/include/toda_b200.h
--- a/include/toda_b200.h
+++ b/include/toda_b200.h
@@ -96,8 +96,10 @@
 int toda_weight_kmajor_bf16(const float *w, int kvol, int cin, int cout, void *w_bf16, void *stream);
 size_t toda_spconv_wgrad_workspace_bytes(int n_in, int n_out, int kvol, int cin, int cout, int precision);
 int toda_spconv_wgrad(const float *x, const void *x_bf16, int n_in, int cin, const int32_t *nbr, int n_out, int kvol,
-                      const float *dy, const void *dy_bf16, int cout, float *dw_param, void *workspace,
-                      size_t workspace_bytes, int precision, void *stream);
+                      const uint32_t *tile_masks, const float *dy, const void *dy_bf16, int cout, float *dw_param,
+                      void *workspace, size_t workspace_bytes, int precision, void *stream);
+int toda_spconv_wgrad_row_splits(const uint32_t *tile_masks, int n_out, int kvol, int cin, int cout, int *groups,
+                                 int *splits, int32_t *row_begin, void *stream);
 
 size_t toda_bn_workspace_bytes(int channels);
 int toda_bn_local_sums(const float *y, const double *epilogue_sums, int n, int channels, double *sums, double *count,
@@ -115,10 +117,12 @@
                        size_t workspace_bytes, void *stream);
 int toda_bn_bwd_finish(const float *da, const float *a, const float *y, int n, int channels, const float *gamma,
                        const float *save_mean, const float *save_rstd, int relu, int training, const double *red,
-                       const double *count, float *dy, void *dy_bf16, float *dresidual, void *stream);
+                       const double *count, float *dy, void *dy_bf16, float *dresidual, float *dbias, void *workspace,
+                       size_t workspace_bytes, void *stream);
 int toda_bn_bwd(const float *da, const float *a, const float *y, int n, int channels, const float *gamma,
                 const float *save_mean, const float *save_rstd, int relu, int training, float *dy, void *dy_bf16,
-                float *dresidual, float *dgamma, float *dbeta, void *workspace, size_t workspace_bytes, void *stream);
+                float *dresidual, float *dgamma, float *dbeta, float *dbias, void *workspace, size_t workspace_bytes,
+                void *stream);
 int toda_col_sum(const float *dy, int n, int channels, float *out, void *workspace, size_t workspace_bytes,
                  void *stream);
 
@@ -142,7 +146,8 @@
     const int32_t *dgrad_out_rows ; const uint32_t *dgrad_masks ;
     const uint16_t *dplan_lidx ; const int32_t *dplan_rows; const int32_t *dplan_cnt; int dplan_groups, dplan_cap;
     const float *addend ; float *dx;
-    int need_dw; const int32_t *nbr_fwd; float *dw; void *wgrad_ws; size_t wgrad_ws_bytes;
+    int need_dw; const int32_t *nbr_fwd; const uint32_t *fwd_masks ; float *dw;
+    void *wgrad_ws; size_t wgrad_ws_bytes;
     int need_db; float *db;
     int precision; void *conv_ws; size_t conv_ws_bytes;
 } toda_layer_bwd_args;
diff --git a/toda_b200/_C.py b/toda_b200/_C.py
--- a/toda_b200/_C.py
+++ b/toda_b200/_C.py
@@ -52,7 +52,9 @@
     "toda_layer_bwd_reduce": (c_int, [c_vp, c_vp, c_vp]),
     "toda_layer_bwd_finish": (c_int, [c_vp, c_vp, c_vp, c_vp]),
     "toda_spconv_wgrad_workspace_bytes": (c_sz, [c_int] * 6),
-    "toda_spconv_wgrad": (c_int, [c_vp, c_vp, c_int, c_int, c_vp, c_int, c_int, c_vp, c_vp, c_int, c_vp, c_vp, c_sz, c_int, c_vp]),
+    "toda_spconv_wgrad": (c_int, [c_vp, c_vp, c_int, c_int, c_vp, c_int, c_int, c_vp, c_vp, c_vp, c_int, c_vp, c_vp, c_sz, c_int,
+                                  c_vp]),
+    "toda_spconv_wgrad_row_splits": (c_int, [c_vp, c_int, c_int, c_int, c_int, _IP, _IP, c_vp, c_vp]),
     "toda_bn_workspace_bytes": (c_sz, [c_int]),
     "toda_bn_local_sums": (c_int, [c_vp, c_vp, c_int, c_int, c_vp, c_vp, c_vp, c_sz, c_vp]),
     "toda_bn_eval_coeffs": (c_int, [c_vp, c_vp, c_vp, c_vp, c_f32, c_int, c_vp, c_vp, c_vp]),
@@ -60,10 +62,10 @@
     "toda_bn_apply_sums": (c_int, [c_vp, c_int, c_int, c_vp, c_vp, c_vp, c_vp, c_f32, c_f32, c_vp, c_vp, c_vp, c_vp, c_vp, c_vp,
                                    c_vp, c_int, c_vp, c_vp, c_vp]),
     "toda_bn_bwd": (c_int, [c_vp, c_vp, c_vp, c_int, c_int, c_vp, c_vp, c_vp, c_int, c_int, c_vp, c_vp, c_vp, c_vp, c_vp,
-                            c_vp, c_sz, c_vp]),
+                            c_vp, c_vp, c_sz, c_vp]),
     "toda_bn_bwd_reduce": (c_int, [c_vp, c_vp, c_vp, c_int, c_int, c_vp, c_vp, c_int, c_vp, c_vp, c_vp, c_vp, c_sz, c_vp]),
     "toda_bn_bwd_finish": (c_int, [c_vp, c_vp, c_vp, c_int, c_int, c_vp, c_vp, c_vp, c_int, c_int, c_vp, c_vp, c_vp, c_vp, c_vp,
-                                   c_vp]),
+                                   c_vp, c_vp, c_sz, c_vp]),
     "toda_col_sum": (c_int, [c_vp, c_int, c_int, c_vp, c_vp, c_sz, c_vp]),
     "toda_bev_scatter_fwd": (c_int, [c_vp, c_vp, c_int, c_int, c_int, c_int, c_int, c_int, c_vp, c_vp]),
     "toda_bev_scatter_bwd": (c_int, [c_vp, c_vp, c_int, c_int, c_int, c_int, c_int, c_int, c_vp, c_vp]),
@@ -90,7 +92,7 @@
                 ("need_dx", c_int), ("dgrad_nbr", c_vp), ("wt", c_vp), ("wt_bf16", c_vp), ("dgrad_out_rows", c_vp), ("dgrad_masks", c_vp),
                 ("dplan_lidx", c_vp), ("dplan_rows", c_vp), ("dplan_cnt", c_vp), ("dplan_groups", c_int), ("dplan_cap", c_int),
                 ("addend", c_vp), ("dx", c_vp),
-                ("need_dw", c_int), ("nbr_fwd", c_vp), ("dw", c_vp), ("wgrad_ws", c_vp), ("wgrad_ws_bytes", c_sz),
+                ("need_dw", c_int), ("nbr_fwd", c_vp), ("fwd_masks", c_vp), ("dw", c_vp), ("wgrad_ws", c_vp), ("wgrad_ws_bytes", c_sz),
                 ("need_db", c_int), ("db", c_vp),
                 ("precision", c_int), ("conv_ws", c_vp), ("conv_ws_bytes", c_sz)]
 
diff --git a/toda_b200/csrc/bn.cu b/toda_b200/csrc/bn.cu
--- a/toda_b200/csrc/bn.cu
+++ b/toda_b200/csrc/bn.cu
@@ -6,6 +6,7 @@
 
 constexpr int kThreads = 256;
 constexpr int kPartials = 2 * kNumSMs;
+constexpr int kApplyPartials = 2048 / kThreads * kNumSMs;
 
 template <int MODE>
 __global__ void __launch_bounds__(kThreads) col_reduce_vec_kernel(const float *__restrict__ p0, const float *__restrict__ p1,
@@ -116,17 +117,18 @@
         col_reduce_kernel<MODE><<<kPartials, kThreads, 0, st>>>(p0, p1, p2, n, c, mean, rstd, relu, partial);
 }
 
+template <int MAX_BLOCKS = kPartials, int ROWS = 2>
 __device__ __forceinline__ void warp_sum_partials(const double *__restrict__ partial, int nblocks, int c, int ch, double &s,
                                                   double &ss) {
     const int lane = threadIdx.x & 31;
-    constexpr int kPerLane = (kPartials + 31) / 32;
+    constexpr int kPerLane = (MAX_BLOCKS + 31) / 32;
     double va[kPerLane], vb[kPerLane];
 #pragma unroll
     for (int i = 0; i < kPerLane; ++i) {
         const int j = lane + 32 * i;
         const bool ok = j < nblocks;
-        va[i] = ok ? partial[((size_t)j * 2) * c + ch] : 0.0;
-        vb[i] = ok ? partial[((size_t)j * 2 + 1) * c + ch] : 0.0;
+        va[i] = ok ? partial[((size_t)j * ROWS) * c + ch] : 0.0;
+        vb[i] = ok && ROWS == 2 ? partial[((size_t)j * ROWS + 1) * c + ch] : 0.0;
     }
     double a = 0.0, b = 0.0;
 #pragma unroll
@@ -262,17 +264,20 @@
 }
 
 template <bool VEC>
-__global__ void __launch_bounds__(kThreads) bn_bwd_apply_kernel(const float *__restrict__ da, const float *__restrict__ a,
+__global__ void __launch_bounds__(kThreads, 5) bn_bwd_apply_kernel(const float *__restrict__ da, const float *__restrict__ a,
                                                                 const float *__restrict__ y, long long total, int c, int n,
                                                                 const double *__restrict__ count, const float *__restrict__ gamma,
                                                                 const float *__restrict__ mean, const float *__restrict__ rstd,
                                                                 const double *__restrict__ sums, int relu, int training,
                                                                 float *__restrict__ dy, float *__restrict__ dres,
-                                                                __nv_bfloat16 *__restrict__ dy_bf16) {
+                                                                __nv_bfloat16 *__restrict__ dy_bf16, double *__restrict__ db_partial) {
+    extern __shared__ double s_db[];
+    double db[4] = {0.0, 0.0, 0.0, 0.0};
     if (count) n = (int)*count;
     auto sum = [&](int i) -> float { return (float)sums[i]; };
     const float inv_n = n > 0 ? 1.0f / (float)n : 0.f;
-    const long long stride = (long long)gridDim.x * blockDim.x;
+    const long long threads = (long long)gridDim.x * blockDim.x;
+    const long long stride = VEC ? threads : threads / c * c;
     long long e = blockIdx.x * (long long)blockDim.x + threadIdx.x;
     if (VEC) {
         const long long tv = total >> 2;
@@ -301,9 +306,10 @@
             o.w = fmaf(A[3], g4.w, fmaf(B[3], y4.w, C[3]));
             if (dy) ((float4 *)dy)[e] = o;
             if (dy_bf16) store_bf16x4(dy_bf16, e, o);
+            if (db_partial) { db[0] += o.x; db[1] += o.y; db[2] += o.z; db[3] += o.w; }
         }
     } else {
-        for (; e < total; e += stride) {
+        for (e = e < stride ? e : total; e < total; e += stride) {
             int ch = (int)(e % c);
             float g = __ldg(da + e);
             if (relu && !(__ldg(a + e) > 0.f)) g = 0.f;
@@ -319,19 +325,36 @@
             }
             if (dy) dy[e] = o;
             if (dy_bf16) dy_bf16[e] = __float2bfloat16_rn(o);
-        }
-    }
-}
-
+            if (db_partial) db[0] += o;
+        }
+    }
+    if (!db_partial) return;
+    constexpr int kSlots = VEC ? 4 : 1;
+#pragma unroll
+    for (int q = 0; q < kSlots; ++q) s_db[threadIdx.x * kSlots + q] = db[q];
+    __syncthreads();
+    if ((int)threadIdx.x < c) {
+        const int units = VEC ? c / 4 : c;
+        const int u = VEC ? (int)threadIdx.x >> 2 : (int)threadIdx.x, q = VEC ? (int)threadIdx.x & 3 : 0;
+        double t = 0.0;
+        for (int j = u; j < kThreads; j += units) t += s_db[j * kSlots + q];
+        const int ch = VEC ? (int)threadIdx.x : (int)(((long long)blockIdx.x * kThreads + threadIdx.x) % c);
+        db_partial[(size_t)blockIdx.x * c + ch] = t;
+    }
+}
+
+template <int MAX_BLOCKS, int ROWS>
 __global__ void col_sum_finalize_kernel(const double *__restrict__ partial, int nblocks, int c, float *out) {
     int ch = (blockIdx.x * blockDim.x + threadIdx.x) >> 5;
     if (ch >= c) return;
     double s, unused;
-    warp_sum_partials(partial, nblocks, c, ch, s, unused);
+    warp_sum_partials<MAX_BLOCKS, ROWS>(partial, nblocks, c, ch, s, unused);
     if ((threadIdx.x & 31) == 0) out[ch] = (float)s;
 }
 
-size_t partials_bytes(int c) { return (size_t)kPartials * 2 * c * sizeof(double); }
+size_t partials_bytes(int c) {
+    return (size_t)(2 * kPartials > kApplyPartials ? 2 * kPartials : kApplyPartials) * c * sizeof(double);
+}
 size_t bn_ws_bytes(int c) { return align_up(partials_bytes(c) + 2 * c * sizeof(double), 256); }
 
 template <auto Kernel> int resident_grid(int64_t items) {
@@ -431,32 +454,50 @@
 
 extern "C" int toda_bn_bwd_finish(const float *da, const float *a, const float *y, int n, int c, const float *gamma,
                                   const float *save_mean, const float *save_rstd, int relu, int training, const double *red,
-                                  const double *count, float *dy, void *dy_bf16, float *dresidual, void *stream) {
+                                  const double *count, float *dy, void *dy_bf16, float *dresidual, float *dbias, void *workspace,
+                                  size_t workspace_bytes, void *stream) {
     TODA_CHECK_ARG(n >= 0 && c > 0 && c <= 256, "bn_bwd_finish: unsupported sizes n=%d c=%d", n, c);
     TODA_CHECK_ARG(save_mean && save_rstd && (red || !training) && (n == 0 || (da && y && (dy || dy_bf16))) &&
-                   (!relu || a || n == 0), "bn_bwd_finish: null pointer");
-    if (n == 0) return TODA_OK;
+                   (!relu || a || n == 0) && (!dbias || workspace), "bn_bwd_finish: null pointer");
+    cudaStream_t st = (cudaStream_t)stream;
+    if (dbias && workspace_bytes < bn_ws_bytes(c)) { toda_set_error("bn_bwd_finish: workspace too small"); return TODA_ERR_WORKSPACE; }
+    if (n == 0) {
+        if (dbias) TODA_CUDA_OK(cudaMemsetAsync(dbias, 0, sizeof(float) * c, st));
+        return TODA_OK;
+    }
     const long long total = (long long)n * c;
-    cudaStream_t st = (cudaStream_t)stream;
-    if (vec_channels(c))
-        bn_bwd_apply_kernel<true><<<resident_grid<bn_bwd_apply_kernel<true>>(total / 4), kThreads, 0, st>>>(
-            da, a, y, total, c, n, count, gamma, save_mean, save_rstd, red, relu, training, dy, dresidual, (__nv_bfloat16 *)dy_bf16);
-    else
-        bn_bwd_apply_kernel<false><<<resident_grid<bn_bwd_apply_kernel<false>>(total), kThreads, 0, st>>>(
-            da, a, y, total, c, n, count, gamma, save_mean, save_rstd, red, relu, training, dy, dresidual, (__nv_bfloat16 *)dy_bf16);
-    TODA_LAUNCH_OK();
+    double *db_partial = dbias ? (double *)workspace : nullptr;
+    const size_t smem = dbias ? kThreads * 4 * sizeof(double) : 0;
+    int grid;
+    if (vec_channels(c)) {
+        grid = resident_grid<bn_bwd_apply_kernel<true>>(total / 4);
+        grid = grid < kApplyPartials ? grid : kApplyPartials;
+        bn_bwd_apply_kernel<true><<<grid, kThreads, smem, st>>>(da, a, y, total, c, n, count, gamma, save_mean, save_rstd, red, relu,
+                                                               training, dy, dresidual, (__nv_bfloat16 *)dy_bf16, db_partial);
+    } else {
+        grid = resident_grid<bn_bwd_apply_kernel<false>>(total);
+        grid = grid < kApplyPartials ? grid : kApplyPartials;
+        bn_bwd_apply_kernel<false><<<grid, kThreads, smem, st>>>(da, a, y, total, c, n, count, gamma, save_mean, save_rstd, red,
+                                                                relu, training, dy, dresidual, (__nv_bfloat16 *)dy_bf16, db_partial);
+    }
+    TODA_LAUNCH_OK();
+    if (dbias) {
+        col_sum_finalize_kernel<kApplyPartials, 1><<<ceil_div(c * 32, 128), 128, 0, st>>>(db_partial, grid, c, dbias);
+        TODA_LAUNCH_OK();
+    }
     return TODA_OK;
 }
 
 extern "C" int toda_bn_bwd(const float *da, const float *a, const float *y, int n, int c, const float *gamma,
                            const float *save_mean, const float *save_rstd, int relu, int training, float *dy, void *dy_bf16,
-                           float *dresidual, float *dgamma, float *dbeta, void *workspace, size_t workspace_bytes, void *stream) {
+                           float *dresidual, float *dgamma, float *dbeta, float *dbias, void *workspace, size_t workspace_bytes,
+                           void *stream) {
     TODA_CHECK_ARG(workspace, "bn_bwd: null workspace");
     double *red = bn_workspace_red(workspace, c);
     int rc = toda_bn_bwd_reduce(da, a, y, n, c, save_mean, save_rstd, relu, red, dgamma, dbeta, workspace, workspace_bytes, stream);
     if (rc) return rc;
     return toda_bn_bwd_finish(da, a, y, n, c, gamma, save_mean, save_rstd, relu, training, red, nullptr, dy, dy_bf16, dresidual,
-                              stream);
+                              dbias, workspace, workspace_bytes, stream);
 }
 
 extern "C" int toda_col_sum(const float *dy, int n, int c, float *out, void *workspace, size_t workspace_bytes, void *stream) {
@@ -466,7 +507,7 @@
     double *partial = (double *)workspace;
     launch_col_reduce<2>(dy, nullptr, nullptr, n, c, nullptr, nullptr, 0, partial, st);
     TODA_LAUNCH_OK();
-    col_sum_finalize_kernel<<<ceil_div(c * 32, 128), 128, 0, st>>>(partial, kPartials, c, out);
+    col_sum_finalize_kernel<kPartials, 2><<<ceil_div(c * 32, 128), 128, 0, st>>>(partial, kPartials, c, out);
     TODA_LAUNCH_OK();
     return TODA_OK;
 }
diff --git a/toda_b200/csrc/conv_simt.cu b/toda_b200/csrc/conv_simt.cu
--- a/toda_b200/csrc/conv_simt.cu
+++ b/toda_b200/csrc/conv_simt.cu
@@ -7,16 +7,16 @@
                 cudaStream_t st, const TilePlan *plan, const float *addend, const void *w_bf16);
 size_t conv_tc_fwd_workspace_bytes(int n_in, int cin, int cout, int kvol);
 int conv_tc_wgrad(const float *x, const void *x_bf16, int n_in, int cin, const int32_t *nbr, int n_out, int kvol,
-                  const float *dy, const void *dy_bf16, int cout, float *dw_param, void *workspace, size_t workspace_bytes,
-                  cudaStream_t st);
+                  const uint32_t *tile_masks, const float *dy, const void *dy_bf16, int cout, float *dw_param, void *workspace,
+                  size_t workspace_bytes, cudaStream_t st);
 bool conv_tc_supported(int cin, int cout, int kvol);
 size_t conv_x3_fwd_workspace_bytes(int n_in, int cin, int cout, int kvol);
 int conv_x3_fwd(const float *x, int n_in, int cin, const int32_t *nbr, int n_out, int kvol, const float *w, int cout, const float *bias,
                 float *y, const int32_t *out_rows, const uint32_t *tile_masks, double *bn_sums, void *workspace, size_t workspace_bytes,
                 cudaStream_t st, const TilePlan *plan, const float *addend);
 size_t conv_x3_wgrad_workspace_bytes(int n_in, int n_out, int kvol, int cin, int cout);
-int conv_x3_wgrad(const float *x, int n_in, int cin, const int32_t *nbr, int n_out, int kvol, const float *dy, int cout, float *dw_param,
-                  void *workspace, size_t workspace_bytes, cudaStream_t st);
+int conv_x3_wgrad(const float *x, int n_in, int cin, const int32_t *nbr, int n_out, int kvol, const uint32_t *tile_masks,
+                  const float *dy, int cout, float *dw_param, void *workspace, size_t workspace_bytes, cudaStream_t st);
 bool conv_tc_wgrad_supported(int cin, int cout, int kvol);
 size_t conv_tc_wgrad_workspace_bytes(int n_in, int n_out, int kvol, int cin, int cout);
 
@@ -328,8 +328,8 @@
 }
 
 extern "C" int toda_spconv_wgrad(const float *x, const void *x_bf16, int n_in, int cin, const int32_t *nbr, int n_out,
-                                 int kvol, const float *dy, const void *dy_bf16, int cout, float *dw_param, void *workspace,
-                                 size_t workspace_bytes, int precision, void *stream) {
+                                 int kvol, const uint32_t *tile_masks, const float *dy, const void *dy_bf16, int cout,
+                                 float *dw_param, void *workspace, size_t workspace_bytes, int precision, void *stream) {
     TODA_CHECK_ARG(n_in >= 0 && n_out >= 0 && cin > 0 && cout > 0 && kvol > 0, "spconv_wgrad: bad sizes");
     TODA_CHECK_ARG(dw_param, "spconv_wgrad: null dw");
     cudaStream_t st = (cudaStream_t)stream;
@@ -341,9 +341,10 @@
     TODA_CHECK_ARG(precision == TODA_CONV_FP32 || precision == TODA_CONV_BF16 || precision == TODA_CONV_BF16X3,
                    "spconv_wgrad: unknown precision %d", precision);
     if (precision == TODA_CONV_BF16X3 && conv_tc_wgrad_supported(cin, cout, kvol))
-        return conv_x3_wgrad(x, n_in, cin, nbr, n_out, kvol, dy, cout, dw_param, workspace, workspace_bytes, st);
+        return conv_x3_wgrad(x, n_in, cin, nbr, n_out, kvol, tile_masks, dy, cout, dw_param, workspace, workspace_bytes, st);
     if (precision == TODA_CONV_BF16 && conv_tc_wgrad_supported(cin, cout, kvol))
-        return conv_tc_wgrad(x, x_bf16, n_in, cin, nbr, n_out, kvol, dy, dy_bf16, cout, dw_param, workspace, workspace_bytes, st);
+        return conv_tc_wgrad(x, x_bf16, n_in, cin, nbr, n_out, kvol, tile_masks, dy, dy_bf16, cout, dw_param, workspace,
+                             workspace_bytes, st);
     int splits = wgrad_splits(n_out, kvol, cin, cout);
     size_t need = (size_t)splits * kvol * cin * cout * sizeof(float);
     if (workspace_bytes < need) {
diff --git a/toda_b200/csrc/conv_tc.cu b/toda_b200/csrc/conv_tc.cu
--- a/toda_b200/csrc/conv_tc.cu
+++ b/toda_b200/csrc/conv_tc.cu
@@ -571,12 +571,53 @@
     return d;
 }
 
+__device__ __forceinline__ uint32_t wgrad_live_passes(const uint32_t *__restrict__ tile_masks, int c, int rows, int k0, int npass,
+                                                      int opp) {
+    if (!tile_masks) return (1u << npass) - 1u;
+    const uint32_t om = __ldg(tile_masks + ((c * rows) >> 7)) >> k0;
+    uint32_t lm = 0;
+    for (int ps = 0; ps < npass; ++ps)
+        if ((om >> (ps * opp)) & ((1u << opp) - 1u)) lm |= 1u << ps;
+    return lm;
+}
+
+__device__ void wgrad_split_chunks(const uint32_t *__restrict__ tile_masks, int n_out, int rows, int k0, int npass, int opp,
+                                   int split, int splits, int *scratch, int &c_begin, int &c_end) {
+    const int tid = threadIdx.x, nt = blockDim.x;
+    const int nch = (n_out + rows - 1) / rows;
+    const int per = (nch + nt - 1) / nt, c0 = min(nch, tid * per), c1 = min(nch, c0 + per);
+    int local = 0;
+    for (int c = c0; c < c1; ++c) local += __popc(wgrad_live_passes(tile_masks, c, rows, k0, npass, opp));
+    if (tid == 0) scratch[nt] = scratch[nt + 1] = 0;
+    scratch[tid] = local;
+    __syncthreads();
+    for (int off = 1; off < nt; off <<= 1) {
+        const int v = tid >= off ? scratch[tid - off] : 0;
+        __syncthreads();
+        scratch[tid] += v;
+        __syncthreads();
+    }
+    const long long total = scratch[nt - 1];
+    const long long ta = (long long)split * total / splits, tb = (long long)(split + 1) * total / splits;
+    int run = scratch[tid] - local, na = 0, nb = 0;
+    for (int c = c0; c < c1; ++c) {
+        na += run < ta;
+        nb += run < tb;
+        run += __popc(wgrad_live_passes(tile_masks, c, rows, k0, npass, opp));
+    }
+    if (na) atomicAdd(scratch + nt, na);
+    if (nb) atomicAdd(scratch + nt + 1, nb);
+    __syncthreads();
+    c_begin = split == 0 ? 0 : scratch[nt];
+    c_end = split + 1 == splits ? nch : scratch[nt + 1];
+}
+
 template <int CIN, int NPAD, int ROWS>
 __global__ void __launch_bounds__(kWgradThreads, 1) conv_tc_wgrad_kernel(const __nv_bfloat16 *__restrict__ xb,
                                                                          const int *__restrict__ nbr, int n_out, int kvol,
                                                                          const __nv_bfloat16 *__restrict__ dyb, int cout,
-                                                                         int rows_per_split, int passes_per_cta,
-                                                                         float *__restrict__ partial) {
+                                                                         const uint32_t *__restrict__ tile_masks ,
+                                                                         int passes_per_cta, float *__restrict__ partial) {
     using W = WCfg<NPAD, ROWS>;
     constexpr int kOffsPerPass = 128 / CIN;
     constexpr int S = W::kStages;
@@ -601,9 +642,15 @@
     const int npass = min(passes_per_cta, total_passes - pass0);
     const int k0 = pass0 * kOffsPerPass;
     const int noffs = min(npass * kOffsPerPass, kvol - k0);
-    const int r_begin = split * rows_per_split;
-    const int r_end = min(n_out, r_begin + rows_per_split);
-    const int nchunks = r_end > r_begin ? (r_end - r_begin + kRowsW - 1) / kRowsW : 0;
+    int c_begin, c_end;
+    wgrad_split_chunks(tile_masks, n_out, kRowsW, k0, npass, kOffsPerPass, split, gridDim.x, (int *)(smem_raw + (base - raw)),
+                       c_begin, c_end);
+    const int r_begin = c_begin * kRowsW;
+    const int r_end = min(n_out, c_end * kRowsW);
+    const int nchunks = c_end - c_begin;
+    auto live_of = [&](int rc) -> uint32_t {
+        return wgrad_live_passes(tile_masks, c_begin + rc, kRowsW, k0, npass, kOffsPerPass);
+    };
 
     if (tid == 0) {
         for (int s = 0; s < S; ++s) {
@@ -639,21 +686,32 @@
         const int ci_lo = CIN >= 64 ? p * 8 : (p % (CIN / 8)) * 8;
         constexpr int kLagW = W::kLag;
         int g = 0, signalled = 0;
+        int lc = 0, bsig = 0;
+        int first1 = 0, first2 = 0;
+        uint32_t pend_first = 0;
+        auto signal_next = [&]() {
+            if (lane == 0) {
+                if (pend_first & 1u) mbar_arrive(b_full + 8 * (bsig % kBBufsW));
+                mbar_arrive(a_full + 8 * (signalled % S));
+            }
+            bsig += pend_first & 1u;
+            pend_first >>= 1;
+            ++signalled;
+        };
         for (int rc = 0; rc < nchunks; ++rc) {
-            const int ib = rc & 1, use_i = rc >> 1;
-            const int bb = rc % kBBufsW, use_b = rc / kBBufsW;
+            const uint32_t lm = live_of(rc);
+            if (!lm) continue;
+            const int ib = lc & 1, use_i = lc >> 1;
+            const int bb = lc % kBBufsW, use_b = lc / kBBufsW;
             const int row_base = r_begin + rc * kRowsW;
-            if (npass < kLagW) {
+            if (use_b > 0 && signalled < (kBBufsW == 2 ? first1 : first2)) {
                 asm volatile("cp.async.wait_group 0;" ::: "memory");
                 asm volatile("fence.proxy.async.shared::cta;" ::: "memory");
                 __syncwarp();
-                if (lane == 0)
-                    for (; signalled < g; ++signalled) {
-                        if (signalled % npass == 0) mbar_arrive(b_full + 8 * ((signalled / npass) % kBBufsW));
-                        mbar_arrive(a_full + 8 * (signalled % S));
-                    }
-                signalled = g;
+                while (signalled < g) signal_next();
             }
+            first2 = first1;
+            first1 = g;
             if (use_b > 0) mbar_wait(b_empty + 8 * bb, (use_b - 1) & 1);
             {
                 const uint32_t b_dst = b_base + bb * kBTileW + piece_off;
@@ -671,7 +729,9 @@
             }
             mbar_wait(idx_full + 8 * ib, use_i & 1);
             const uint32_t idx_tile = idx_base + ib * kIdxW + 4 * rbase;
-            for (int ps = 0; ps < npass; ++ps, ++g) {
+            for (uint32_t m = lm; m; m &= m - 1, ++g) {
+                const int ps = __ffs(m) - 1;
+                if (m == lm) pend_first |= 1u << (g - signalled);
                 const int s = g % S, use = g / S;
                 if (use > 0) mbar_wait(a_empty + 8 * s, (use - 1) & 1);
                 const uint32_t a_dst = base + s * kATileW + piece_off;
@@ -698,34 +758,29 @@
                     asm volatile("cp.async.wait_group %0;" ::"n"(kLagW) : "memory");
                     asm volatile("fence.proxy.async.shared::cta;" ::: "memory");
                     __syncwarp();
-                    const int j = signalled;
-                    if (lane == 0) {
-                        if (j % npass == 0) mbar_arrive(b_full + 8 * ((j / npass) % kBBufsW));
-                        mbar_arrive(a_full + 8 * (j % S));
-                    }
-                    ++signalled;
+                    signal_next();
                 }
             }
             mbar_arrive(idx_empty + 8 * ib);
+            ++lc;
         }
         asm volatile("cp.async.wait_group 0;" ::: "memory");
         asm volatile("fence.proxy.async.shared::cta;" ::: "memory");
         __syncwarp();
-        if (lane == 0)
-            for (int j = signalled; j < g; ++j) {
-                if (j % npass == 0) mbar_arrive(b_full + 8 * ((j / npass) % kBBufsW));
-                mbar_arrive(a_full + 8 * (j % S));
-            }
+        while (signalled < g) signal_next();
     } else if (warp == 8) {
         if (nchunks > 0) {
             constexpr uint32_t idesc = make_idesc_bf16(128, NPAD) | (1u << 15) | (1u << 16);
-            int g = 0;
-            uint32_t ready = 0;
+            int g = 0, lc = 0;
+            uint32_t ready = 0, started = 0;
             for (int rc = 0; rc < nchunks; ++rc) {
-                const int ib = rc % kBBufsW;
-                mbar_wait(b_full + 8 * ib, (rc / kBBufsW) & 1);
+                const uint32_t lm = live_of(rc);
+                if (!lm) continue;
+                const int ib = lc % kBBufsW;
+                mbar_wait(b_full + 8 * ib, (lc / kBBufsW) & 1);
                 const uint32_t b_tile = b_base + ib * kBTileW;
-                for (int ps = 0; ps < npass; ++ps, ++g) {
+                for (uint32_t m = lm; m; m &= m - 1, ++g) {
+                    const int ps = __ffs(m) - 1;
                     const int s = g % S, use = g / S;
                     if (!ready) mbar_wait(a_full + 8 * s, use & 1);
                     ready = mbar_test(a_full + 8 * ((g + 1) % S), ((g + 1) / S) & 1);
@@ -734,22 +789,28 @@
                     if (elect_one()) {
 #pragma unroll
                         const uint64_t ad0 = make_desc_mn_sw128(a_tile, kRowsW * 128), bd0 = make_desc_mn_sw128(b_tile, kRowsW * 128);
-                        umma_bf16(tmem_base + ps * NPAD, ad0, bd0, idesc, rc != 0);
+                        umma_bf16(tmem_base + ps * NPAD, ad0, bd0, idesc, (started >> ps) & 1u);
                         for (int j = 1; j < kRowsW / 16; ++j)
                             umma_bf16(tmem_base + ps * NPAD, ad0 + 128 * j, bd0 + 128 * j, idesc, 1u);
                         umma_commit(a_empty + 8 * s);
                     }
                     __syncwarp();
                 }
+                started |= lm;
                 if (elect_one()) umma_commit(b_empty + 8 * ib);
                 __syncwarp();
+                ++lc;
             }
-            if (elect_one()) umma_commit(accum_bar);
-            __syncwarp();
+            if (g > 0) {
+                if (elect_one()) umma_commit(accum_bar);
+                __syncwarp();
+            }
         }
     } else if (warp < 13) {
         const int q = warp & 3;
-        if (nchunks > 0) {
+        uint32_t used = 0;
+        for (int rc = 0; rc < nchunks; ++rc) used |= live_of(rc);
+        if (used) {
             mbar_wait(accum_bar, 0);
             asm volatile("tcgen05.fence::after_thread_sync;" ::: "memory");
         }
@@ -760,7 +821,7 @@
             const uint32_t taddr = tmem_base + ((uint32_t)(q * 32) << 16) + ps * NPAD;
             for (int n0 = 0; n0 < cout; n0 += 16) {
                 uint32_t v[16];
-                if (nchunks > 0) {
+                if ((used >> ps) & 1u) {
                     asm volatile(
                         "tcgen05.ld.sync.aligned.32x32b.x16.b32 {%0,%1,%2,%3,%4,%5,%6,%7,%8,%9,%10,%11,%12,%13,%14,%15}, [%16];"
                         : "=r"(v[0]), "=r"(v[1]), "=r"(v[2]), "=r"(v[3]), "=r"(v[4]), "=r"(v[5]), "=r"(v[6]), "=r"(v[7]),
@@ -781,8 +842,10 @@
         }
         asm volatile("tcgen05.fence::before_thread_sync;" ::: "memory");
     } else {
-        for (int rc = 0; rc < nchunks; ++rc) {
-            const int ib = rc & 1, use = rc >> 1;
+        for (int rc = 0, lc = 0; rc < nchunks; ++rc) {
+            if (!live_of(rc)) continue;
+            const int ib = lc & 1, use = lc >> 1;
+            ++lc;
             if (use > 0) mbar_wait(idx_empty + 8 * ib, (use - 1) & 1);
             const uint32_t dst0 = idx_base + ib * kIdxW;
             const int row_base = r_begin + rc * kRowsW;
@@ -824,7 +887,7 @@
 }
 
 struct WgradPlan {
-    int passes_per_cta, groups, splits, rows_per_split;
+    int passes_per_cta, groups, splits, rows;
     size_t xb_bytes, dyb_bytes, partial_bytes;
 };
 
@@ -841,15 +904,41 @@
     int max_by_rows = (n_out + 4 * kRowsW - 1) / (4 * kRowsW);
     p.splits = want < max_by_rows ? want : max_by_rows;
     if (p.splits < 1) p.splits = 1;
-    int rps = (n_out + p.splits - 1) / p.splits;
-    p.rows_per_split = (rps + kRowsW - 1) / kRowsW * kRowsW;
-    if (p.rows_per_split < kRowsW) p.rows_per_split = kRowsW;
+    p.rows = kRowsW;
     p.xb_bytes = align_up((size_t)n_in * cin * 2 + 16, 256);
     p.dyb_bytes = align_up((size_t)n_out * cout * 2 + 16, 256);
     p.partial_bytes = align_up((size_t)p.splits * kvol * cin * cout * 4, 256);
     return p;
 }
 
+__global__ void __launch_bounds__(kWgradThreads) wgrad_row_splits_kernel(const uint32_t *__restrict__ tile_masks, int n_out,
+                                                                         int kvol, int opp, int rows, int passes_per_cta,
+                                                                         int32_t *__restrict__ row_begin) {
+    __shared__ int scratch[kWgradThreads + 2];
+    const int total_passes = (kvol + opp - 1) / opp, pass0 = blockIdx.y * passes_per_cta;
+    int c_begin, c_end;
+    wgrad_split_chunks(tile_masks, n_out, rows, pass0 * opp, min(passes_per_cta, total_passes - pass0), opp, blockIdx.x, gridDim.x,
+                       scratch, c_begin, c_end);
+    if (threadIdx.x == 0) row_begin[blockIdx.y * gridDim.x + blockIdx.x] = min(n_out, c_begin * rows);
+}
+
+}
+
+bool conv_tc_wgrad_supported(int cin, int cout, int kvol);
+
+extern "C" int toda_spconv_wgrad_row_splits(const uint32_t *tile_masks, int n_out, int kvol, int cin, int cout, int *groups,
+                                            int *splits, int32_t *row_begin, void *stream) {
+    TODA_CHECK_ARG(n_out > 0 && kvol > 0 && kvol <= kMaxKvol && groups && splits && conv_tc_wgrad_supported(cin, cout, kvol),
+                   "spconv_wgrad_row_splits: bad args");
+    const int cp = pad16(cin);
+    WgradPlan p = wgrad_plan(0, n_out, kvol, cp, cout);
+    *groups = p.groups;
+    *splits = p.splits;
+    if (!row_begin) return TODA_OK;
+    wgrad_row_splits_kernel<<<dim3(p.splits, p.groups), kWgradThreads, 0, (cudaStream_t)stream>>>(tile_masks, n_out, kvol, 128 / cp,
+                                                                                                  p.rows, p.passes_per_cta, row_begin);
+    TODA_LAUNCH_OK();
+    return TODA_OK;
 }
 
 bool conv_tc_wgrad_supported(int cin, int cout, int kvol) {
@@ -862,8 +951,8 @@
 }
 
 int conv_tc_wgrad(const float *x, const void *x_bf16, int n_in, int cin, const int32_t *nbr, int n_out, int kvol,
-                  const float *dy, const void *dy_bf16, int cout, float *dw_param, void *workspace, size_t workspace_bytes,
-                  cudaStream_t st) {
+                  const uint32_t *tile_masks, const float *dy, const void *dy_bf16, int cout, float *dw_param, void *workspace,
+                  size_t workspace_bytes, cudaStream_t st) {
     const int cin_real = cin;
     cin = pad16(cin);
     WgradPlan p = wgrad_plan(n_in, n_out, kvol, cin, cout);
@@ -903,7 +992,7 @@
             TODA_CUDA_OK(cudaFuncSetAttribute(conv_tc_wgrad_kernel<CI, NP, RW>, cudaFuncAttributeMaxDynamicSharedMemorySize, smem)); \
             attr_set = true;                                                                                               \
         }                                                                                                                  \
-        conv_tc_wgrad_kernel<CI, NP, RW><<<grid, kWgradThreads, smem, st>>>(xb, nbr, n_out, kvol, dyb, cout, p.rows_per_split,  \
+        conv_tc_wgrad_kernel<CI, NP, RW><<<grid, kWgradThreads, smem, st>>>(xb, nbr, n_out, kvol, dyb, cout, tile_masks,       \
                                                                            p.passes_per_cta, partial);                      \
     } while (0)
     const bool wide = cout > 64;
diff --git a/toda_b200/csrc/conv_x3.cu b/toda_b200/csrc/conv_x3.cu
--- a/toda_b200/csrc/conv_x3.cu
+++ b/toda_b200/csrc/conv_x3.cu
@@ -9,8 +9,8 @@
                 cudaStream_t st, const TilePlan *plan, const float *addend, const void *w_bf16);
 size_t conv_tc_fwd_workspace_bytes(int n_in, int cin, int cout, int kvol);
 int conv_tc_wgrad(const float *x, const void *x_bf16, int n_in, int cin, const int32_t *nbr, int n_out, int kvol,
-                  const float *dy, const void *dy_bf16, int cout, float *dw_param, void *workspace, size_t workspace_bytes,
-                  cudaStream_t st);
+                  const uint32_t *tile_masks, const float *dy, const void *dy_bf16, int cout, float *dw_param, void *workspace,
+                  size_t workspace_bytes, cudaStream_t st);
 size_t conv_tc_wgrad_workspace_bytes(int n_in, int n_out, int kvol, int cin, int cout);
 
 namespace {
@@ -120,8 +120,8 @@
     return 2 * l.x_bytes + 2 * l.dy_bytes + 3 * l.t_bytes + l.inner + 256;
 }
 
-int conv_x3_wgrad(const float *x, int n_in, int cin, const int32_t *nbr, int n_out, int kvol, const float *dy, int cout, float *dw_param,
-                  void *workspace, size_t workspace_bytes, cudaStream_t st) {
+int conv_x3_wgrad(const float *x, int n_in, int cin, const int32_t *nbr, int n_out, int kvol, const uint32_t *tile_masks,
+                  const float *dy, int cout, float *dw_param, void *workspace, size_t workspace_bytes, cudaStream_t st) {
     const size_t need = conv_x3_wgrad_workspace_bytes(n_in, n_out, kvol, cin, cout);
     if (!workspace || workspace_bytes < need) {
         toda_set_error("spconv_wgrad(bf16x3): workspace %zu < required %zu bytes", workspace_bytes, need);
@@ -138,11 +138,11 @@
     TODA_LAUNCH_OK();
     split_rows_kernel<<<wave_grid((int64_t)n_out * cout, 256), 256, 0, st>>>(dy, n_out, cout, cout, dh, dl);
     TODA_LAUNCH_OK();
-    int rc = conv_tc_wgrad(x, xh, n_in, cp, nbr, n_out, kvol, dy, dh, cout, t1, inner, l.inner, st);
+    int rc = conv_tc_wgrad(x, xh, n_in, cp, nbr, n_out, kvol, tile_masks, dy, dh, cout, t1, inner, l.inner, st);
     if (rc) return rc;
-    rc = conv_tc_wgrad(x, xh, n_in, cp, nbr, n_out, kvol, dy, dl, cout, t2, inner, l.inner, st);
+    rc = conv_tc_wgrad(x, xh, n_in, cp, nbr, n_out, kvol, tile_masks, dy, dl, cout, t2, inner, l.inner, st);
     if (rc) return rc;
-    rc = conv_tc_wgrad(x, xl, n_in, cp, nbr, n_out, kvol, dy, dh, cout, t3, inner, l.inner, st);
+    rc = conv_tc_wgrad(x, xl, n_in, cp, nbr, n_out, kvol, tile_masks, dy, dh, cout, t3, inner, l.inner, st);
     if (rc) return rc;
     const size_t rows = (size_t)cout * kvol;
     sum3_unpad_kernel<<<wave_grid((int64_t)rows * cin, 256), 256, 0, st>>>(t1, t2, t3, rows, cp, cin, dw_param);
diff --git a/toda_b200/csrc/layer.cu b/toda_b200/csrc/layer.cu
--- a/toda_b200/csrc/layer.cu
+++ b/toda_b200/csrc/layer.cu
@@ -53,7 +53,7 @@
 
 static bool layer_bwd_reads_dy_f32(const toda_layer_bwd_args *p) {
     const int c = p->cout;
-    return p->need_db || !p->dy_bf16 || p->precision != TODA_CONV_BF16 ||
+    return !p->dy_bf16 || p->precision != TODA_CONV_BF16 ||
            (p->need_dx && !toda_spconv_uses_tensor_cores(c, p->cin, p->kvol, p->precision)) ||
            (p->need_dw && !toda_spconv_wgrad_uses_tensor_cores(p->cin, c, p->kvol, p->precision));
 }
@@ -68,12 +68,8 @@
         if (rc) return rc;
     }
     if (p->need_dw) {
-        rc = toda_spconv_wgrad(p->x, p->x_bf16, p->n_in, p->cin, p->nbr_fwd, n, p->kvol, p->dy, p->dy_bf16, c, p->dw, p->wgrad_ws,
-                               p->wgrad_ws_bytes, p->precision, stream);
-        if (rc) return rc;
-    }
-    if (p->need_db) {
-        rc = toda_col_sum(p->dy, n, c, p->db, p->bn_ws, p->bn_ws_bytes, stream);
+        rc = toda_spconv_wgrad(p->x, p->x_bf16, p->n_in, p->cin, p->nbr_fwd, n, p->kvol, p->fwd_masks, p->dy, p->dy_bf16, c, p->dw,
+                               p->wgrad_ws, p->wgrad_ws_bytes, p->precision, stream);
         if (rc) return rc;
     }
     return TODA_OK;
@@ -88,7 +84,8 @@
     const int c = p->cout, n = p->n_out;
     if (n == 0) return layer_bwd_empty(p, false, (cudaStream_t)stream);
     int rc = toda_bn_bwd_finish(p->da, p->a_mask, p->y, n, c, p->gamma, p->mean, p->rstd, p->relu, p->training, red, count,
-                                layer_bwd_reads_dy_f32(p) ? p->dy : nullptr, p->dy_bf16, p->dres, stream);
+                                layer_bwd_reads_dy_f32(p) ? p->dy : nullptr, p->dy_bf16, p->dres, p->need_db ? p->db : nullptr,
+                                p->bn_ws, p->bn_ws_bytes, stream);
     return rc ? rc : layer_bwd_conv(p, stream);
 }
 
diff --git a/toda_b200/ops.py b/toda_b200/ops.py
--- a/toda_b200/ops.py
+++ b/toda_b200/ops.py
@@ -599,8 +599,9 @@
         ws = _workspace("wgrad", ws_bytes, dy.device)
         with _timed("conv_wgrad", n_in=rb.n_in, n_out=rb.n_out, cin=cin, cout=cout, kvol=rb.kvol, precision=precision,
                     rb=id(rb)):
-            _C.check(L.toda_spconv_wgrad(_p(x), _p(xb), rb.n_in, cin, _p(rb.nbr_fwd), rb.n_out, rb.kvol, _p(dy), _p(dyb),
-                                         cout, _p(dw), _p(ws), ws.numel(), precision, _stream()), "toda_spconv_wgrad")
+            _C.check(L.toda_spconv_wgrad(_p(x), _p(xb), rb.n_in, cin, _p(rb.nbr_fwd), rb.n_out, rb.kvol, _p(rb.tile_masks),
+                                         _p(dy), _p(dyb), cout, _p(dw), _p(ws), ws.numel(), precision, _stream()),
+                     "toda_spconv_wgrad")
     if need_db:
         db = col_sum(dy)
     return dx, dw, db
@@ -737,7 +738,7 @@
     return a, ab, y, mean, rstd, a, gsums
 
 
-def _bn_backward_phases(da, y, a, gamma, mean, rstd, training, relu, has_res, want_bf16, gsums=None):
+def _bn_backward_phases(da, y, a, gamma, mean, rstd, training, relu, has_res, want_bf16, gsums=None, want_db=False):
     n, c = y.shape
     da = da.contiguous() if da is not None else torch.zeros_like(y)
     L = _C.lib()
@@ -745,19 +746,22 @@
     dyb = torch.empty(y.shape, dtype=torch.bfloat16, device=y.device) if want_bf16 else None
     dres = torch.empty_like(y) if has_res else None
     dgamma, dbeta = torch.empty((2, c), dtype=torch.float32, device=y.device).unbind(0)
+    db = torch.empty((c,), dtype=torch.float32, device=y.device) if want_db else None
     ws = _workspace("bn", L.toda_bn_workspace_bytes(c), y.device)
     if gsums is None:
         with _timed("bn_bwd", n=n, c=c, residual=has_res):
             _C.check(L.toda_bn_bwd(_p(da), _p(a), _p(y), n, c, _p(gamma), _p(mean), _p(rstd), int(relu), int(training),
-                                   _p(dy), _p(dyb), _p(dres), _p(dgamma), _p(dbeta), _p(ws), ws.numel(), _stream()), "toda_bn_bwd")
-        return dy, dyb, dres, dgamma, dbeta
+                                   _p(dy), _p(dyb), _p(dres), _p(dgamma), _p(dbeta), _p(db), _p(ws), ws.numel(), _stream()),
+                     "toda_bn_bwd")
+        return dy, dyb, dres, dgamma, dbeta, db
     red = torch.empty((2 * c,), dtype=torch.float64, device=y.device)
     _C.check(L.toda_bn_bwd_reduce(_p(da), _p(a), _p(y), n, c, _p(mean), _p(rstd), int(relu), _p(red), _p(dgamma), _p(dbeta),
                                   _p(ws), ws.numel(), _stream()), "toda_bn_bwd_reduce")
     yield red
     _C.check(L.toda_bn_bwd_finish(_p(da), _p(a), _p(y), n, c, _p(gamma), _p(mean), _p(rstd), int(relu), 1, _p(red),
-                                  gsums.data_ptr() + 16 * c, _p(dy), _p(dyb), _p(dres), _stream()), "toda_bn_bwd_finish")
-    return dy, dyb, dres, dgamma, dbeta
+                                  gsums.data_ptr() + 16 * c, _p(dy), _p(dyb), _p(dres), _p(db), _p(ws), ws.numel(), _stream()),
+             "toda_bn_bwd_finish")
+    return dy, dyb, dres, dgamma, dbeta, db
 
 
 class _BNAct(torch.autograd.Function):
@@ -780,8 +784,8 @@
             return (None,) * 13
         y, a, gamma, mean, rstd, gsums = ctx.saved_tensors
         training, relu, has_res, want_bf16 = ctx.cfg
-        dy, dyb, dres, dgamma, dbeta = _run_phases(_bn_backward_phases(da, y, a, gamma, mean, rstd, training, relu, has_res,
-                                                                       want_bf16, gsums), ctx.group)
+        dy, dyb, dres, dgamma, dbeta, _ = _run_phases(_bn_backward_phases(da, y, a, gamma, mean, rstd, training, relu, has_res,
+                                                                          want_bf16, gsums), ctx.group)
         if dyb is not None:
             dy._toda_bf16 = (dyb, dy._version)
         return dy, dgamma, dbeta, None, None, None, None, None, dres, None, None, None, None
@@ -873,9 +877,9 @@
     if da is None:
         da = torch.zeros_like(y)
     if not _fused_ok(training, True):
-        dy, dyb, dres, dgamma, dbeta = yield from _bn_backward_phases(da, y, a_mask, gamma, mean, rstd, training, relu, has_res,
-                                                                      precision == CONV_BF16, gsums)
-        dx, dw, db = _conv_backward_impl(dy, dyb, x, weight, xb, rb, precision, need_dx, need_dw, has_bias)
+        dy, dyb, dres, dgamma, dbeta, db = yield from _bn_backward_phases(da, y, a_mask, gamma, mean, rstd, training, relu,
+                                                                          has_res, precision == CONV_BF16, gsums, has_bias)
+        dx, dw, _ = _conv_backward_impl(dy, dyb, x, weight, xb, rb, precision, need_dx, need_dw, False)
         if addend is not None and dx is not None:
             dx = dx + addend
         return dx, dw, db, dgamma, dbeta, dres
@@ -940,7 +944,7 @@
         int(bool(need_dx)), _vp(nbr), _vp(wt), _vp(wtb), _vp(out_rows), _vp(masks),
         _vp(pl.lidx) if pl else None, _vp(pl.rows) if pl else None, _vp(pl.cnt) if pl else None, pl.ngroups if pl else 0,
         pl.cap if pl else 0, _vp(addend) if need_dx else None, _vp(dx),
-        int(bool(need_dw)), rb.nbr_fwd.data_ptr(), _vp(dw), _vp(wws), wws.numel() if wws is not None else 0,
+        int(bool(need_dw)), rb.nbr_fwd.data_ptr(), _vp(rb.tile_masks), _vp(dw), _vp(wws), wws.numel() if wws is not None else 0,
         int(bool(has_bias)), sp + 8 * cout, precision, _vp(ws), ws.numel() if ws is not None else 0)
     return args, dx, dw, dres, small, (da, dy, dyb, addend, wt, wtb, ws, wws, bws)
 
```
